# AshHarvey/ssa-gym

Hardware: AMD Instinct MI355X
Metric: env_steps_per_sec_at_20k_objects (higher is better)
Workload: dtype f64

## Files before the change

### include/ssa_hip.h

```cpp
#ifndef SSA_HIP_H
#define SSA_HIP_H

#include <stdint.h>

#ifdef __cplusplus
extern "C" {
#endif

#define SSA_ABI_VERSION 23
#define SSA_INLINE_ENVS 8

#define SSA_OK 0
#define SSA_E_INVALID (-1)
#define SSA_E_LAUNCH (-2)
#define SSA_E_UNSUPPORTED (-3)

#define SSA_ST_OK 0
#define SSA_ST_PREDICT_NAN 1
#define SSA_ST_PREDICT_LINALG 2
#define SSA_ST_UPDATE_NAN 3
#define SSA_ST_UPDATE_LINALG 4

#define SSA_OBS_AER 0
#define SSA_OBS_XYZ 1

#define SSA_PROP_ELEMENTS 0
#define SSA_PROP_FG 1
#define SSA_PROP_J2_RK4 2

#define SSA_PROP_HYBRID 3

#define SSA_FLAG_RESAMPLE 1u

#define SSA_FLAG_REFERENCE_COV 2u

#define SSA_UPD_STRIDE 64
#define SSA_UPD_OBS_TAKEN 0
#define SSA_UPD_Z_TRUE 1
#define SSA_UPD_Y 4
#define SSA_UPD_S 7
#define SSA_UPD_SIGMAS_H 16
#define SSA_UPD_VISIBLE 55
#define SSA_UPD_ACTION 56

#define SSA_STAT_SHARDS 128
#define SSA_STAT_SHARD_WORDS 16
#define SSA_STAT_STRIDE 8
#define SSA_STAT_MAX_DPOS 0
#define SSA_STAT_CNT_LT_1E4 1
#define SSA_STAT_CNT_LT_1E7 2
#define SSA_STAT_ARGMAX_SPOS 3
#define SSA_STAT_N_FAILED 4
#define SSA_STAT_MAX_SPOS 5

typedef struct ssa_consts {
    double Q[36];
    double R[9];
    double Wm0, Wc0, Wi;
    double sum_wm_m1;
    double sum_wc;
    double scale;
    double dt;
    double obs_limit;
    double enu[9];
    double obs_itrs[3];
    int32_t obs_type;
    int32_t propagator;
    uint32_t flags;
    int32_t update_interval;
    double j2, r_eq;
    int32_t rk4_substeps;
    int32_t reserved0;
} ssa_consts;

typedef struct ssa_step_params {
    int64_t n_obj;
    int32_t n_env;
    int32_t time_offset;
    const double *x_true_in; double *x_true_out;
    const double *x_in;      double *x_out;
    const double *P_in;      double *P_out;
    int32_t *status;
    double *obs;
    double *metrics;
    double *upd;
    const double *trans;
    const int32_t *env_time;
    const int32_t *actions;
    const double *z_noise;
    int64_t zn_stride_env, zn_stride_time, zn_stride_obj;
    int32_t n_time;
    uint32_t launch_mask;
    double *stats;
    int32_t *work;
    void *stat_ws;
    uint64_t *stat_shards;
    uint64_t *stat_shards_prev;
    double *stats_prev;
    double *aer_out;
    uint64_t *stat_shards_clear;
    int32_t aer_cols;
    int32_t action0;
    double *obs_mirror;
    int32_t inline_time[SSA_INLINE_ENVS];
    int32_t inline_action[SSA_INLINE_ENVS];
    uint64_t *spos_tiles;
    uint64_t *spos_tiles_prev;
    double *fail_log;
    uint32_t *fail_count;
    int32_t fail_cap;
    int32_t reserved1;
    const int32_t *obj_ids;
    const double *metrics_prev;
} ssa_step_params;
#define SSA_FAIL_STRIDE 8
#define SSA_FAIL_ENV 0
#define SSA_FAIL_OBJ 1
#define SSA_FAIL_STATUS 2
#define SSA_FAIL_TIME 3
#define SSA_FAIL_ERR 4

int ssa_env_step_f64(const ssa_consts *c_host, const ssa_step_params *p_host, void *stream);
#define SSA_PROFILE_SLOTS 1024
#define SSA_LAUNCH_DEFER_FOLD 8u
#define SSA_LAUNCH_INLINE_ACTION 16u
#define SSA_LAUNCH_FOLD_INSIDE 32u
#define SSA_LAUNCH_MIRROR_F32 128u
#define SSA_LAUNCH_INLINE_ENVS 64u
#define SSA_LAUNCH_STATS_FROM_METRICS 256u
int ssa_env_step_profiled_f64(const ssa_consts *c_host, const ssa_step_params *p_host, void *stream, int32_t slot);
int ssa_env_step_profile_ms(int32_t slot, float *kernel_ms);
typedef struct ssa_rollout_params {
    int32_t n_steps;
    int32_t history;
    int32_t slot_out;
    int32_t reserved;
    double *x_true_ring;
    double *x_ring;
    double *P_ring;
    double *obs_ring;
    double *metrics_ring;
    double *upd_ring;
    double *stats_ring;
    const int32_t *actions;
    uint64_t *stat_shards;
    uint64_t *spos_tiles;
} ssa_rollout_params;
int ssa_env_rollout_f64(const ssa_consts *c_host, const ssa_step_params *first, const ssa_rollout_params *r, void *stream);

int ssa_stats_fold_f64(uint64_t *stat_shards, double *stats, int32_t n_env, void *stream);
int ssa_stats_fold_spos_f64(uint64_t *stat_shards, const uint64_t *spos_tiles, double *stats, int64_t n_obj, int32_t n_env, void *stream);
int32_t ssa_stats_from_metrics_waves(int64_t n_obj, int32_t n_env);
int ssa_stats_fold_metrics_f64(const double *metrics, uint64_t *stat_shards, const uint64_t *spos_tiles, double *stats, int64_t n_obj,
                               void *stream);
int64_t ssa_env_step_work_bytes(int64_t n_obj, int32_t n_env);

int ssa_reward_stats_f64(const double *metrics, const int32_t *status, double *stats, void *workspace,
                         int64_t n_obj, int32_t n_env, void *stream);
int64_t ssa_reward_stats_workspace_bytes(int32_t n_env);

int ssa_propagate_f64(const double *x_in, double *x_out, int64_t n, double dt, int32_t propagator, void *stream);
int ssa_propagate_j2_f64(const double *x_in, double *x_out, int64_t n, double dt, double j2, double r_eq,
                         int32_t substeps, void *stream);
int ssa_kepler_elements_f64(const double *x_in, double *coe, int64_t n, double dt, void *stream);
int ssa_robust_cholesky6_f64(const double *A, double *U, int32_t *rung, int64_t n, void *stream);
int ssa_ladder_probe_f64(const double *A, double scale, int32_t *rung, int32_t *mask, double *U, int64_t n, void *stream);
int ssa_sigma_points_f64(const double *x, const double *P, double scale, double *sig, int32_t *fail,
                         int64_t n, void *stream);
int ssa_hx_aer_f64(const double *x, int64_t x_stride, const double *M, const ssa_consts *c_host, double *z,
                   int64_t n, void *stream);
int ssa_mean_z_uvw_f64(const double *sigmas, const ssa_consts *c_host, double *zp, int64_t n, void *stream);
int ssa_residual_z_aer_f64(const double *a, const double *b, double *c, int64_t n, void *stream);
int ssa_visible_mask_f64(const double *x_true, const double *M, const ssa_consts *c_host, uint8_t *mask,
                         double *el, int64_t n, void *stream);
int ssa_observe_f64(const double *x_true, const double *x, const double *P, double *obs, double *metrics,
                    int64_t n, void *stream);
int ssa_aer_obs_f64(const double *x, const double *P, const double *M, const ssa_consts *c_host, double *out,
                    int64_t n, void *stream);

int ssa_agent_scores_f64(const double *x_true, const double *x_cur, const double *P_cur, const double *P_prev,
                         const double *M, const ssa_consts *c_host, double *scores, uint8_t *mask, int64_t n,
                         void *stream);
int ssa_visible_mask_at_f64(const double *x_true, const double *trans, const int32_t *env_time, int32_t time_offset, int32_t n_time,
                            const ssa_consts *c_host, uint8_t *mask, double *el, int64_t n, void *stream);
int ssa_agent_scores_at_f64(const double *x_true, const double *x_cur, const double *P_cur, const double *P_prev, const double *trans,
                            const int32_t *env_time, int32_t time_offset, int32_t n_time, const ssa_consts *c_host, double *scores,
                            uint8_t *mask, int64_t n, void *stream);
int ssa_masked_argmax_f64(const double *score, const uint8_t *mask, int64_t n, int64_t *out, void *stream);
int ssa_masked_argmax_ws_f64(const double *score, const uint8_t *mask, int64_t n, int64_t *out, void *workspace, int64_t workspace_bytes,
                             void *stream);
int64_t ssa_masked_argmax_workspace_bytes(int64_t n);

#define SSA_AGENT_NAIVE_GREEDY 0
#define SSA_AGENT_VISIBLE_GREEDY 1
#define SSA_AGENT_SHANNON 2
#define SSA_AGENT_POS_ERROR 3
#define SSA_AGENT_VEL_ERROR 4
int ssa_agent_select_f64(const ssa_consts *c_host, int32_t kind, const double *x_true, const double *x_cur,
                         const double *P_cur, const double *P_prev, const double *trans, const int32_t *env_time,
                         int32_t time_offset, int32_t n_time, const int32_t *fallback, void *workspace,
                         int32_t *action_out, int64_t *pick_out, int64_t n_obj, int32_t n_env, void *stream);
int ssa_agent_select_ids_f64(const ssa_consts *c_host, int32_t kind, const double *x_true, const double *x_cur,
                             const double *P_cur, const double *P_prev, const double *trans, const int32_t *env_time,
                             int32_t time_offset, int32_t n_time, const int32_t *fallback, void *workspace,
                             int32_t *action_out, int64_t *pick_out, int64_t n_obj, int32_t n_env, const int32_t *obj_ids, void *stream);
int64_t ssa_agent_select_workspace_bytes(int64_t n_obj, int32_t n_env);

int ssa_nees_f64(const double *x_true, const double *x, const double *P, double *nees, int64_t n, void *stream);
int ssa_nis_f64(const double *y, const double *S, double *nis, int64_t n, void *stream);
int ssa_chi2_contained_f64(const double *v, int64_t n, double lo, double hi, int64_t *counts, void *stream);

typedef struct ssa_closed_loop_params {
    int32_t n_steps;
    int32_t history;
    int32_t slot_out;
    int32_t agent;
    double *x_true_ring, *x_ring, *P_ring, *obs_ring, *metrics_ring;
    double *upd_out;
    double *stats_out;
    int32_t *actions;
    const int32_t *fallback;
    int64_t *picks;
    int32_t *error;
    void *workspace;
    int64_t workspace_bytes;
    int64_t wait_ticks;
    uint32_t flags;
    uint32_t reserved;
    const int32_t *slot_of;
} ssa_closed_loop_params;
#define SSA_LOOP_ARGMAX_SPOS 1u
#define SSA_LOOP_DEBUG_WITHHOLD 2u
int ssa_env_closed_loop_f64(const ssa_consts *c_host, const ssa_step_params *first, const ssa_closed_loop_params *r, void *stream);
int64_t ssa_closed_loop_workspace_bytes(int64_t n_obj, int32_t n_env);

#define SSA_LOOK_NSCORE 3
#define SSA_LOOK_TRACE_GAIN 0
#define SSA_LOOK_POS_TRACE_GAIN 1
#define SSA_LOOK_INFO_GAIN 2
typedef struct ssa_lookahead_out {
    double *score;
    int32_t *status;
    uint8_t *visible;
    double *x_prior;
    double *P_prior;
    double *P_post;
} ssa_lookahead_out;
int ssa_lookahead_f64(const ssa_consts *c_host, const ssa_step_params *p_host, const ssa_lookahead_out *out, void *stream);

#define SSA_MAX_SENSORS 8
typedef struct ssa_sensor_params {
    int32_t n_sensor;
    int32_t reserved;
    int32_t action[SSA_MAX_SENSORS];
    double enu[SSA_MAX_SENSORS][9];
    double obs_itrs[SSA_MAX_SENSORS][3];
    double obs_limit[SSA_MAX_SENSORS];
    double R[SSA_MAX_SENSORS][9];
    int64_t zn_stride_sensor;
    double *upd;
} ssa_sensor_params;
int ssa_env_step_sensors_f64(const ssa_consts *c_host, const ssa_step_params *p_host, const ssa_sensor_params *s_host, void *stream);

typedef struct ssa_sensor_envs_params {
    const int32_t *actions;
    double *upd;
    int32_t inline_action[SSA_INLINE_ENVS][SSA_MAX_SENSORS];
} ssa_sensor_envs_params;
int ssa_env_step_sensors_envs_f64(const ssa_consts *c, const ssa_step_params *p, const ssa_sensor_params *sites,
                                  const ssa_sensor_envs_params *envs, void *stream);

int ssa_lookahead_sensors_f64(const ssa_consts *c_host, const ssa_step_params *p_host, const ssa_sensor_params *s_host,
                              const ssa_lookahead_out *out, void *stream);
int ssa_lookahead_sensors_envs_f64(const ssa_consts *c, const ssa_step_params *p, const ssa_sensor_params *sites,
                                   const ssa_lookahead_out *out, void *stream);

typedef struct ssa_rollout_sensors_params {
    const int32_t *actions;
    double *upd_ring;
} ssa_rollout_sensors_params;
int ssa_env_rollout_sensors_f64(const ssa_consts *c_host, const ssa_step_params *first, const ssa_rollout_params *r,
                                const ssa_sensor_params *sites, const ssa_rollout_sensors_params *rs, void *stream);
// ... 63 lines not shown
```

### profiles/pmc_counters_reduce.py

```python
import csv, glob, json, os, sys
ROOT = os.path.dirname(os.path.dirname(os.path.abspath(__file__)))
out = {"kernel": None, "workload": "20 000 objects = 5000 wavefronts, profiles/pmc_workload.py", "counters": {}}
for d in sys.argv[1:]:
    fs = glob.glob(os.path.join(ROOT, d, '*', '*counter_collection.csv'))
    if not fs:
        out["counters"][os.path.basename(d)] = "pass produced no counter file (counter not available on this build?)"
        continue
    acc = {}
    for r in csv.DictReader(open(fs[0])):
        if 'step_fast_kernel' not in r['Kernel_Name']:
            continue
        if out["kernel"] is None:
            out["kernel"] = r['Kernel_Name'].split('(')[0]
        acc.setdefault(r['Counter_Name'], []).append(float(r['Counter_Value']))
    for k, v in acc.items():
        v = v[20:] if len(v) > 40 else v
        out["counters"][k] = {"mean_per_launch": sum(v) / len(v), "per_wavefront": sum(v) / len(v) / 5000.0, "launches": len(v)}
print(json.dumps(out, indent=1))
```

### profiles/pmc_reduce.py

```python
import csv, glob, json, os, sys
ROOT = os.path.dirname(os.path.dirname(os.path.abspath(__file__)))
def per_kernel(d, counter):
    f = glob.glob(os.path.join(ROOT, d, '*', '*counter_collection.csv'))[0]
    acc = {}
    for r in csv.DictReader(open(f)):
        if r['Counter_Name'] != counter: continue
        k = r['Kernel_Name']
        key = 'step' if 'step_fast_kernel' in k else 'propagate' if 'propagate_kernel' in k else 'observe' if 'observe_kernel' in k else None
        if key: acc.setdefault(key, []).append(float(r['Counter_Value']))
    return acc
fe, wr = per_kernel(sys.argv[1], 'FETCH_SIZE'), per_kernel(sys.argv[2], 'WRITE_SIZE')
n = 1 << 20
known = {'propagate': (48 * n, 48 * n), 'observe': (384 * n, 128 * n)}
out = {}
for k in ('propagate', 'observe'):
    f = sum(fe[k][-3:]) / 3 * 1024; w = sum(wr[k][-3:]) / 3 * 1024
    out['calib_' + k] = {'fetch_counter_bytes': f, 'fetch_known_bytes': known[k][0], 'fetch_ratio': f / known[k][0],
                         'write_counter_bytes': w, 'write_known_bytes': known[k][1], 'write_ratio': w / known[k][1]}
fs = fe['step'][20:]; ws = wr['step'][20:]
f = sum(fs) / len(fs) * 1024; w = sum(ws) / len(ws) * 1024
cf = out['calib_observe']['fetch_ratio']; cw = out['calib_observe']['write_ratio']
out['step_raw'] = {'fetch_counter_bytes': f, 'write_counter_bytes': w, 'launches': len(fs)}
key = '%s_%s' % (os.environ.get('PROP', 'hybrid'), os.environ.get('M', '20000'))
out[key] = round(f / cf + w / cw)
out['algorithmic_bytes'] = 896 * int(os.environ.get('M', '20000'))
print(json.dumps(out, indent=1))
dst = os.path.join(ROOT, 'profiles', 'traffic.json')
old = json.load(open(dst)) if os.path.exists(dst) else {}
old[key] = out[key]
old.setdefault('other_configurations', {})[key] = {'step_raw': out['step_raw'], 'calib_observe': out['calib_observe'], 'calib_propagate': out['calib_propagate']}
if not isinstance(old.get('collected'), dict):
    old['collected'] = {}
old['collected'][key] = os.environ.get('TAG', 'unlabelled')
old['algorithmic_bytes_20000'] = 896 * 20000
json.dump(old, open(dst, 'w'), indent=1)
```

### ssa-gym_amd/_lib.py

```python
import ctypes as C
import os

from . import _build

c_dp = C.c_void_p


class ssa_consts(C.Structure):
    _fields_ = [
        ("Q", C.c_double * 36), ("R", C.c_double * 9),
        ("Wm0", C.c_double), ("Wc0", C.c_double), ("Wi", C.c_double),
        ("sum_wm_m1", C.c_double), ("sum_wc", C.c_double), ("scale", C.c_double),
        ("dt", C.c_double), ("obs_limit", C.c_double),
        ("enu", C.c_double * 9), ("obs_itrs", C.c_double * 3),
        ("obs_type", C.c_int32), ("propagator", C.c_int32), ("flags", C.c_uint32),
        ("update_interval", C.c_int32),
        ("j2", C.c_double), ("r_eq", C.c_double), ("rk4_substeps", C.c_int32), ("reserved0", C.c_int32),
    ]


class ssa_step_params(C.Structure):
    _fields_ = [
        ("n_obj", C.c_int64), ("n_env", C.c_int32), ("time_offset", C.c_int32),
        ("x_true_in", c_dp), ("x_true_out", c_dp), ("x_in", c_dp), ("x_out", c_dp),
        ("P_in", c_dp), ("P_out", c_dp), ("status", c_dp), ("obs", c_dp), ("metrics", c_dp),
        ("upd", c_dp), ("trans", c_dp), ("env_time", c_dp), ("actions", c_dp), ("z_noise", c_dp),
        ("zn_stride_env", C.c_int64), ("zn_stride_time", C.c_int64), ("zn_stride_obj", C.c_int64),
        ("n_time", C.c_int32), ("launch_mask", C.c_uint32), ("stats", c_dp), ("work", c_dp), ("stat_ws", c_dp),
        ("stat_shards", c_dp), ("stat_shards_prev", c_dp), ("stats_prev", c_dp), ("aer_out", c_dp),
        ("stat_shards_clear", c_dp), ("aer_cols", C.c_int32), ("action0", C.c_int32), ("obs_mirror", c_dp),
        ("inline_time", C.c_int32 * 8), ("inline_action", C.c_int32 * 8),
        ("spos_tiles", c_dp), ("spos_tiles_prev", c_dp),
        ("fail_log", c_dp), ("fail_count", c_dp), ("fail_cap", C.c_int32), ("reserved1", C.c_int32),
        ("obj_ids", c_dp), ("metrics_prev", c_dp),
    ]


class ssa_rollout_params(C.Structure):
    _fields_ = [
        ("n_steps", C.c_int32), ("history", C.c_int32), ("slot_out", C.c_int32), ("reserved", C.c_int32),
        ("x_true_ring", c_dp), ("x_ring", c_dp), ("P_ring", c_dp), ("obs_ring", c_dp), ("metrics_ring", c_dp),
        ("upd_ring", c_dp), ("stats_ring", c_dp), ("actions", c_dp), ("stat_shards", c_dp), ("spos_tiles", c_dp),
    ]


class ssa_closed_loop_params(C.Structure):
    _fields_ = [
        ("n_steps", C.c_int32), ("history", C.c_int32), ("slot_out", C.c_int32), ("agent", C.c_int32),
        ("x_true_ring", c_dp), ("x_ring", c_dp), ("P_ring", c_dp), ("obs_ring", c_dp), ("metrics_ring", c_dp),
        ("upd_out", c_dp), ("stats_out", c_dp), ("actions", c_dp), ("fallback", c_dp), ("picks", c_dp), ("error", c_dp),
        ("workspace", c_dp), ("workspace_bytes", C.c_int64),
        ("wait_ticks", C.c_int64), ("flags", C.c_uint32), ("reserved", C.c_uint32), ("slot_of", c_dp),
    ]


class ssa_lookahead_out(C.Structure):
    _fields_ = [
        ("score", c_dp), ("status", c_dp), ("visible", c_dp), ("x_prior", c_dp), ("P_prior", c_dp), ("P_post", c_dp),
    ]


class ssa_sensor_params(C.Structure):
    _fields_ = [
        ("n_sensor", C.c_int32), ("reserved", C.c_int32), ("action", C.c_int32 * 8),
        ("enu", (C.c_double * 9) * 8), ("obs_itrs", (C.c_double * 3) * 8), ("obs_limit", C.c_double * 8), ("R", (C.c_double * 9) * 8),
        ("zn_stride_sensor", C.c_int64), ("upd", c_dp),
    ]


class ssa_rollout_sensors_params(C.Structure):
    _fields_ = [("actions", c_dp), ("upd_ring", c_dp)]


class ssa_rollout_sensors_envs_params(C.Structure):
    _fields_ = [("actions", c_dp), ("stats_out", c_dp), ("upd_out", c_dp)]


class ssa_sensor_envs_params(C.Structure):
    _fields_ = [("actions", c_dp), ("upd", c_dp), ("inline_action", (C.c_int32 * 8) * 8)]


class ssa_forecast_params(C.Structure):
    _fields_ = [("n_steps", C.c_int32), ("reserved", C.c_int32), ("out", ssa_lookahead_out)]


class ssa_screen_params(C.Structure):
    _fields_ = [
        ("n", C.c_int64), ("n_time", C.c_int32), ("n_site", C.c_int32), ("step", C.c_double), ("min_alt", C.c_double),
        ("first", C.c_int32), ("max_gap", C.c_int32), ("elements", c_dp), ("trans", c_dp), ("sites", c_dp),
        ("accept", c_dp), ("worst_gap", c_dp), ("flags", c_dp),
    ]


E_INVALID, E_LAUNCH, E_UNSUPPORTED = -1, -2, -3
ABI_VERSION = 23
ST_OK, ST_PREDICT_NAN, ST_PREDICT_LINALG, ST_UPDATE_NAN, ST_UPDATE_LINALG = range(5)
OBS_AER, OBS_XYZ = 0, 1
PROP_ELEMENTS, PROP_FG, PROP_J2_RK4, PROP_HYBRID = 0, 1, 2, 3
FLAG_RESAMPLE = 1
FLAG_REFERENCE_COV = 2
UPD_STRIDE, UPD_OBS_TAKEN, UPD_Z_TRUE, UPD_Y, UPD_S, UPD_SIGMAS_H, UPD_VISIBLE, UPD_ACTION = 64, 0, 1, 4, 7, 16, 55, 56
STAT_SHARDS = 128
STAT_SHARD_WORDS = 16
PROFILE_SLOTS = 1024
LAUNCH_DEFER_FOLD = 8
LAUNCH_INLINE_ACTION = 16
LAUNCH_FOLD_INSIDE = 32
LAUNCH_INLINE_ENVS = 64
LAUNCH_MIRROR_F32 = 128
LAUNCH_STATS_FROM_METRICS = 256
INLINE_ENVS = 8
LOOP_ARGMAX_SPOS, LOOP_DEBUG_WITHHOLD = 1, 2
FAIL_STRIDE, FAIL_ENV, FAIL_OBJ, FAIL_STATUS, FAIL_TIME, FAIL_ERR = 8, 0, 1, 2, 3, 4
AGENT_NAIVE_GREEDY, AGENT_VISIBLE_GREEDY, AGENT_SHANNON, AGENT_POS_ERROR, AGENT_VEL_ERROR = range(5)
MAX_SENSORS = 8
LOOK_NSCORE, LOOK_TRACE_GAIN, LOOK_POS_TRACE_GAIN, LOOK_INFO_GAIN = 3, 0, 1, 2
STAT_STRIDE, STAT_MAX_DPOS, STAT_CNT_LT_1E4, STAT_CNT_LT_1E7, STAT_ARGMAX_SPOS, STAT_N_FAILED, STAT_MAX_SPOS = 8, 0, 1, 2, 3, 4, 5

SIGNATURES = {
    "ssa_abi_version": (C.c_int, []),
    "ssa_build_info": (C.c_char_p, []),
    "ssa_env_step_f64": (C.c_int, [C.POINTER(ssa_consts), C.POINTER(ssa_step_params), c_dp]),
    "ssa_env_step_profiled_f64": (C.c_int, [C.POINTER(ssa_consts), C.POINTER(ssa_step_params), c_dp, C.c_int32]),
    "ssa_env_step_profile_ms": (C.c_int, [C.c_int32, C.POINTER(C.c_float)]),
    "ssa_stats_fold_f64": (C.c_int, [c_dp, c_dp, C.c_int32, c_dp]),
    "ssa_stats_fold_spos_f64": (C.c_int, [c_dp, c_dp, c_dp, C.c_int64, C.c_int32, c_dp]),
    "ssa_stats_from_metrics_waves": (C.c_int32, [C.c_int64, C.c_int32]),
    "ssa_stats_fold_metrics_f64": (C.c_int, [c_dp, c_dp, c_dp, c_dp, C.c_int64, c_dp]),
    "ssa_ladder_probe_f64": (C.c_int, [c_dp, C.c_double, c_dp, c_dp, c_dp, C.c_int64, c_dp]),
    "ssa_env_rollout_f64": (C.c_int, [C.POINTER(ssa_consts), C.POINTER(ssa_step_params), C.POINTER(ssa_rollout_params), c_dp]),
    "ssa_env_closed_loop_f64": (C.c_int, [C.POINTER(ssa_consts), C.POINTER(ssa_step_params), C.POINTER(ssa_closed_loop_params), c_dp]),
    "ssa_lookahead_f64": (C.c_int, [C.POINTER(ssa_consts), C.POINTER(ssa_step_params), C.POINTER(ssa_lookahead_out), c_dp]),
    "ssa_env_step_sensors_f64": (C.c_int, [C.POINTER(ssa_consts), C.POINTER(ssa_step_params), C.POINTER(ssa_sensor_params), c_dp]),
    "ssa_env_step_sensors_envs_f64": (C.c_int, [C.POINTER(ssa_consts), C.POINTER(ssa_step_params), C.POINTER(ssa_sensor_params),
                                                C.POINTER(ssa_sensor_envs_params), c_dp]),
    "ssa_lookahead_sensors_f64": (C.c_int, [C.POINTER(ssa_consts), C.POINTER(ssa_step_params), C.POINTER(ssa_sensor_params),
                                            C.POINTER(ssa_lookahead_out), c_dp]),
    "ssa_lookahead_sensors_envs_f64": (C.c_int, [C.POINTER(ssa_consts), C.POINTER(ssa_step_params), C.POINTER(ssa_sensor_params),
                                                 C.POINTER(ssa_lookahead_out), c_dp]),
    "ssa_forecast_sensors_f64": (C.c_int, [C.POINTER(ssa_consts), C.POINTER(ssa_step_params), C.POINTER(ssa_sensor_params),
                                           C.POINTER(ssa_forecast_params), c_dp]),
    "ssa_forecast_sensors_envs_f64": (C.c_int, [C.POINTER(ssa_consts), C.POINTER(ssa_step_params), C.POINTER(ssa_sensor_params),
                                                C.POINTER(ssa_forecast_params), c_dp]),
    "ssa_env_rollout_sensors_f64": (C.c_int, [C.POINTER(ssa_consts), C.POINTER(ssa_step_params), C.POINTER(ssa_rollout_params),
                                              C.POINTER(ssa_sensor_params), C.POINTER(ssa_rollout_sensors_params), c_dp]),
    "ssa_env_rollout_sensors_envs_f64": (C.c_int, [C.POINTER(ssa_consts), C.POINTER(ssa_step_params), C.POINTER(ssa_rollout_params),
                                                   C.POINTER(ssa_sensor_params), C.POINTER(ssa_rollout_sensors_envs_params), c_dp]),
    "ssa_closed_loop_workspace_bytes": (C.c_int64, [C.c_int64, C.c_int32]),
    "ssa_env_step_work_bytes": (C.c_int64, [C.c_int64, C.c_int32]),
    "ssa_reward_stats_f64": (C.c_int, [c_dp, c_dp, c_dp, c_dp, C.c_int64, C.c_int32, c_dp]),
    "ssa_reward_stats_workspace_bytes": (C.c_int64, [C.c_int32]),
    "ssa_propagate_f64": (C.c_int, [c_dp, c_dp, C.c_int64, C.c_double, C.c_int32, c_dp]),
    "ssa_propagate_j2_f64": (C.c_int, [c_dp, c_dp, C.c_int64, C.c_double, C.c_double, C.c_double, C.c_int32, c_dp]),
    "ssa_kepler_elements_f64": (C.c_int, [c_dp, c_dp, C.c_int64, C.c_double, c_dp]),
    "ssa_robust_cholesky6_f64": (C.c_int, [c_dp, c_dp, c_dp, C.c_int64, c_dp]),
    "ssa_sigma_points_f64": (C.c_int, [c_dp, c_dp, C.c_double, c_dp, c_dp, C.c_int64, c_dp]),
    "ssa_hx_aer_f64": (C.c_int, [c_dp, C.c_int64, c_dp, C.POINTER(ssa_consts), c_dp, C.c_int64, c_dp]),
    "ssa_mean_z_uvw_f64": (C.c_int, [c_dp, C.POINTER(ssa_consts), c_dp, C.c_int64, c_dp]),
    "ssa_residual_z_aer_f64": (C.c_int, [c_dp, c_dp, c_dp, C.c_int64, c_dp]),
    "ssa_visible_mask_f64": (C.c_int, [c_dp, c_dp, C.POINTER(ssa_consts), c_dp, c_dp, C.c_int64, c_dp]),
    "ssa_observe_f64": (C.c_int, [c_dp, c_dp, c_dp, c_dp, c_dp, C.c_int64, c_dp]),
    "ssa_agent_scores_f64": (C.c_int, [c_dp, c_dp, c_dp, c_dp, c_dp, C.POINTER(ssa_consts), c_dp, c_dp, C.c_int64, c_dp]),
    "ssa_visible_mask_at_f64": (C.c_int, [c_dp, c_dp, c_dp, C.c_int32, C.c_int32, C.POINTER(ssa_consts), c_dp, c_dp, C.c_int64, c_dp]),
    "ssa_agent_scores_at_f64": (C.c_int, [c_dp, c_dp, c_dp, c_dp, c_dp, c_dp, C.c_int32, C.c_int32, C.POINTER(ssa_consts), c_dp, c_dp, C.c_int64, c_dp]),
    "ssa_masked_argmax_f64": (C.c_int, [c_dp, c_dp, C.c_int64, c_dp, c_dp]),
    "ssa_masked_argmax_ws_f64": (C.c_int, [c_dp, c_dp, C.c_int64, c_dp, c_dp, C.c_int64, c_dp]),
    "ssa_masked_argmax_workspace_bytes": (C.c_int64, [C.c_int64]),
    "ssa_assign_sensors_f64": (C.c_int, [c_dp, C.c_int64, C.c_int32, C.c_int32, c_dp, c_dp, c_dp, c_dp, C.c_int64, c_dp]),
    "ssa_assign_sensors_workspace_bytes": (C.c_int64, [C.c_int64, C.c_int32]),
    "ssa_assign_sensors_envs_f64": (C.c_int, [c_dp, C.c_int64, C.c_int32, C.c_int32, C.c_int32, c_dp, c_dp, c_dp, c_dp, C.c_int64, c_dp]),
    "ssa_assign_sensors_envs_workspace_bytes": (C.c_int64, [C.c_int64, C.c_int32, C.c_int32]),
    "ssa_match_sensors_f64": (C.c_int, [c_dp, C.c_int64, C.c_int32, C.c_int32, c_dp, c_dp, c_dp, c_dp, C.c_int64, c_dp]),
    "ssa_match_sensors_envs_f64": (C.c_int, [c_dp, C.c_int64, C.c_int32, C.c_int32, C.c_int32, c_dp, c_dp, c_dp, c_dp, C.c_int64, c_dp]),
    "ssa_peer_push_f64": (C.c_int, [c_dp, C.c_int64, c_dp, c_dp, C.c_int32, c_dp, C.c_uint64, c_dp, C.c_int64, c_dp, c_dp, c_dp]),
    "ssa_peer_wait": (C.c_int, [c_dp, C.c_int32, c_dp, C.c_uint64, C.c_int64, c_dp, c_dp]),
    "ssa_aer_obs_f64": (C.c_int, [c_dp, c_dp, c_dp, C.POINTER(ssa_consts), c_dp, C.c_int64, c_dp]),
    "ssa_agent_select_f64": (C.c_int, [C.POINTER(ssa_consts), C.c_int32, c_dp, c_dp, c_dp, c_dp, c_dp, c_dp, C.c_int32, C.c_int32,
                                       c_dp, c_dp, c_dp, c_dp, C.c_int64, C.c_int32, c_dp]),
    "ssa_agent_select_ids_f64": (C.c_int, [C.POINTER(ssa_consts), C.c_int32, c_dp, c_dp, c_dp, c_dp, c_dp, c_dp, C.c_int32, C.c_int32,
                                           c_dp, c_dp, c_dp, c_dp, C.c_int64, C.c_int32, c_dp, c_dp]),
    "ssa_agent_select_workspace_bytes": (C.c_int64, [C.c_int64, C.c_int32]),
    "ssa_nees_f64": (C.c_int, [c_dp, c_dp, c_dp, c_dp, C.c_int64, c_dp]),
    "ssa_nis_f64": (C.c_int, [c_dp, c_dp, c_dp, C.c_int64, c_dp]),
    "ssa_chi2_contained_f64": (C.c_int, [c_dp, C.c_int64, C.c_double, C.c_double, c_dp, c_dp]),
    "ssa_catalogue_screen_f64": (C.c_int, [C.POINTER(ssa_screen_params), c_dp]),
}

_lib = None


class SsaHipError(RuntimeError):
    pass


def library_path():
    return _build.LIB


def load():
    global _lib
    if _lib is not None:
        return _lib
    path = library_path()
    if not os.path.exists(path):
        raise SsaHipError(
            "libssa_hip.so is not built (%s). The ssa-gym hot path has no CPU fallback: run "
            "`python -c 'import __graft_entry__ as g; g.build()'` (needs hipcc)." % path)
    import torch
    lib = C.CDLL(path)
    for name, (res, args) in SIGNATURES.items():
        fn = getattr(lib, name)
        fn.restype = res
        fn.argtypes = args
    if lib.ssa_abi_version() != ABI_VERSION:
        raise SsaHipError("libssa_hip.so ABI %d != binding %d: rebuild" % (lib.ssa_abi_version(), ABI_VERSION))
    _lib = lib
    return lib


def check(rc, what):
    if rc != 0:
        raise SsaHipError("%s failed with code %d" % (what, rc))
```

### ssa-gym_amd/csrc/ssa_kernels.hip

```cpp
#include <hip/hip_runtime.h>
#include <cstdio>
#include <cstddef>
#include <cstdlib>
#include <hip/hip_ext.h>
#include <stdint.h>
#include <type_traits>

#include "../../include/ssa_hip.h"
#include "ssa_math.hpp"
#include "ssa_conics.hpp"
#include "ssa_screen.hpp"

namespace ssa {

__device__ __noinline__ Vec6 kepler_general_v(Vec6 x, double tof)
{
    Vec6 o;
    kepler_general_impl(x.v, tof, o.v, nullptr);
    return o;
}
template <int TAG>
__device__ __noinline__ Vec6 kepler_general_tagged(Vec6 x, double tof)
{
    Vec6 o;
    kepler_general_impl(x.v, tof, o.v, nullptr);
    return o;
}
template <int TAG>
__device__ __noinline__ Vec6 kepler_general_fast_tagged(Vec6 x, double tof) { return kepler_general_fast_impl<TAG>(x, tof); }
template <int TAG>
__device__ __noinline__ Vec6 kepler_beyond_series_tagged(Vec6 x, double tof)
{
    Vec6 o;
    const bool ok = kepler_conic_lean<TAG, false>(x.v, tof, o.v);
    if (__any(!ok)) {
        if (!ok) o = kepler_general_fast_tagged<TAG>(x, tof);
    }
    return o;
}
SSA_DEV bool kepler_hybrid_fast(const double* s, double tof, double* o)
{
    const double rr = dot3(s, s), vv = dot3(s + 3, s + 3), rv = dot3(s, s + 3);
    const double c1 = vv - MU * rsqrt_nr(rr);
    const double ex = c1 * s[0] - rv * s[3], ey = c1 * s[1] - rv * s[4], ez = c1 * s[2] - rv * s[5];
    const double e2 = (ex * ex + ey * ey + ez * ez) * (1.0 / (MU * MU));
    bool handled;
    const bool ok = kepler_uv_fast(s, tof, o, handled);
    return ok && (e2 < (1.0 - 1e-2) * (1.0 - 1e-2));
}

__device__ __noinline__ Vec8 kepler_general_diag_v(Vec6 x, double tof, Vec6* out)
{
    Vec8 d;
    Vec6 o;
    kepler_general_impl(x.v, tof, o.v, d.v);
    *out = o;
    return d;
}

struct StepK {
    ssa_consts c;
    ssa_step_params p;
};

constexpr int OBJ_PER_WAVE = 4;
constexpr double X_FAILED_POS = 1e20, X_FAILED_VEL = 1e12;

struct alignas(16) Tiles {
    double P[OBJ_PER_WAVE * 36];
    double Q[36];
    double Z[8];
    int St[OBJ_PER_WAVE];
    int Oid[OBJ_PER_WAVE];
    double X[OBJ_PER_WAVE * 6];
    double pad1[8];
    double T[OBJ_PER_WAVE * 6];
    double UA[OBJ_PER_WAVE * 36];
    double D[408];
    double M[OBJ_PER_WAVE * 12];
    double Obs[OBJ_PER_WAVE * 12];
    double Met[OBJ_PER_WAVE * 4];
};
static_assert(offsetof(Tiles, P) == 0 && offsetof(Tiles, X) == 1536 && offsetof(Tiles, T) == 1792, "LDS-DMA image of the tile (tile_dma_issue)");
SSA_DEV int dbase(int g) { return g * 96 + (g & 1) * 4 + (g >> 1) * 16; }
static_assert(sizeof(Tiles) <= 7680, "Tiles must fit 20 wavefronts per CU (see above)");

struct TileRegs { double2 main, aux; int st; bool dma; };
SSA_DEV double2 load16(const double* src) { return *reinterpret_cast<const double2*>(src); }
SSA_DEV void tile_issue_from(TileRegs& r, const double* P_in, const double* x_in, const double* x_true_in, const int32_t* status,
                            int lane, int64_t base, int cnt)
{
    const double2 zero = make_double2(0.0, 0.0);
    r.main = zero;
    r.aux = zero;
    r.st = SSA_ST_PREDICT_NAN;
    r.dma = false;
    if (cnt <= 0) return;
    const double* Pin = P_in + base * 36;
    if (lane < cnt * 18) r.main = load16(Pin + 2 * lane);
    const bool sX = lane >= 32, sT = lane >= 48;
    const int i = lane - (sT ? 48 : sX ? 32 : 0);
    const int lim = sX ? cnt * 3 : cnt * 18 - 64;
    const double* src = sT ? x_true_in + base * 6 : sX ? x_in + base * 6 : Pin + 128;
    if (i < lim) r.aux = load16(src + 2 * i);
    if (lane >= 60 && lane - 60 < cnt) r.st = status[base + (lane - 60)];
}
SSA_DEV void tile_issue(TileRegs& r, const ssa_step_params& p, int lane, int64_t base, int cnt)
{
    tile_issue_from(r, p.P_in, p.x_in, p.x_true_in, p.status, lane, base, cnt);
}
SSA_DEV void tile_commit(Tiles& t, const TileRegs& r, int lane)
{
    reinterpret_cast<double2*>(t.P)[lane] = r.main;
    const bool sX = lane >= 32, sT = lane >= 48;
    const int i = lane - (sT ? 48 : sX ? 32 : 0);
    double* dst = sT ? t.T : sX ? t.X : t.P + 128;
    if (i < (sX ? 12 : 8)) reinterpret_cast<double2*>(dst)[i] = r.aux;
    if (lane >= 60) t.St[lane - 60] = r.st;
}
SSA_DEV int64_t tile_total(const ssa_step_params& p, bool one_env) { return one_env ? p.n_obj : (int64_t)p.n_env * p.n_obj; }
typedef const __attribute__((address_space(1))) void* GlobalVoidPtr;
typedef __attribute__((address_space(3))) void* LdsVoidPtr;
SSA_DEV void glds16(const double* src, double* lds_base)
{
    __builtin_amdgcn_global_load_lds((GlobalVoidPtr)src, (LdsVoidPtr)lds_base, 16, 0, 0);
}
SSA_DEV void tile_dma_issue(Tiles& t, TileRegs& r, const double* P_in, const double* x_in, const double* x_true_in, const int32_t* status,
                            int lane, int64_t base, bool whole, const ssa_step_params& p, bool one_env)
{
    r.dma = whole;
    if (!whole) {
        tile_issue_from(r, P_in, x_in, x_true_in, status, lane, base, (int)(tile_total(p, one_env) - base));
        return;
    }
    r.st = SSA_ST_PREDICT_NAN;
    const double* Pin = P_in + base * 36;
    glds16(Pin + 2 * lane, t.P);
    if (lane < 8) glds16(Pin + 128 + 2 * lane, t.P + 128);
    if (lane >= 32 && lane < 44) glds16(x_in + base * 6 - 64 + 2 * lane, t.P + 128);
    if (lane >= 48 && lane < 60) glds16(x_true_in + base * 6 - 96 + 2 * lane, t.P + 128);
    if (lane >= 60) r.st = status[base + (lane - 60)];
}
SSA_DEV void tile_dma_wait(Tiles& t, const TileRegs& r, int lane)
{
    asm volatile("s_waitcnt vmcnt(0)" ::: "memory");
    if (lane >= 60) t.St[lane - 60] = r.st;
}
typedef double v2d __attribute__((ext_vector_type(2)));
template <bool NT>
SSA_DEV void store16(double* dst, const double* src)
{
    if (NT) __builtin_nontemporal_store(*reinterpret_cast<const v2d*>(src), reinterpret_cast<v2d*>(dst));
    else *reinterpret_cast<v2d*>(dst) = *reinterpret_cast<const v2d*>(src);
}
SSA_DEV int64_t env_row0(const ssa_step_params& p, int64_t base)
{
    return p.n_env > 1 ? (int64_t)((uint32_t)base / (uint32_t)p.n_obj) * p.n_obj : 0;
}
template <bool NT>
SSA_DEV void store_tile(const Tiles& t, const ssa_step_params& p, int lane, int64_t base, int cnt)
{
#define SSA_SKIP(b) 0
    if (cnt == OBJ_PER_WAVE) {
        if (!SSA_SKIP(1)) {
            store16<NT>(p.P_out + base * 36 + 2 * lane, t.P + 2 * lane);
            if (lane < 8) store16<NT>(p.P_out + base * 36 + 128 + 2 * lane, t.P + 128 + 2 * lane);
        }
        if (!SSA_SKIP(4)) {
            if ((unsigned)(lane - 8) < 12u) store16<NT>(p.x_out + base * 6 - 16 + 2 * lane, t.X - 16 + 2 * lane);
            if ((unsigned)(lane - 20) < 12u) store16<NT>(p.x_true_out + base * 6 - 40 + 2 * lane, t.T - 40 + 2 * lane);
        }
        if (!SSA_SKIP(2) && lane >= 32 && lane < 56) {
            const int i = lane - 32;
            const int jj = (i * 43) >> 8;
            const int r = 2 * i - 12 * jj;
            double* dst = p.obs + base * 12 - 64 + 2 * lane;
            v2d pair;
            if (r < 6) pair = *reinterpret_cast<const v2d*>(t.X + jj * 6 + r);
            else {
                const double* d = t.P + jj * 36 + 7 * (r - 6);
                pair = v2d{d[0], d[7]};
            }
            if (NT) __builtin_nontemporal_store(pair, reinterpret_cast<v2d*>(dst));
            else *reinterpret_cast<v2d*>(dst) = pair;
            if (p.obs_mirror) {
                const int64_t at = p.obj_ids ? (env_row0(p, base) + t.Oid[jj]) * 12 + r : base * 12 - 64 + 2 * lane;
                if (p.launch_mask & SSA_LAUNCH_MIRROR_F32)
                    *reinterpret_cast<float2*>(reinterpret_cast<float*>(p.obs_mirror) + at) = make_float2((float)pair.x, (float)pair.y);
                else *reinterpret_cast<v2d*>(p.obs_mirror + at) = pair;
            }
        }
        if (!SSA_SKIP(16) && lane >= 56 && lane < 60) p.status[base - 56 + lane] = t.St[lane - 56];
        if (!SSA_SKIP(8) && lane < 16) {
            const int kk = lane >> 2, jj = lane & 3;
            const int64_t obj = base + jj;
            if (p.n_env == 1) {
                p.metrics[(int64_t)kk * p.n_obj + obj] = t.Met[jj * 4 + kk];
            } else {
                const int64_t e = (int64_t)((uint32_t)obj / (uint32_t)p.n_obj), j = obj - e * p.n_obj;
                p.metrics[(e * 4 + kk) * p.n_obj + j] = t.Met[jj * 4 + kk];
            }
        }
        return;
    }
    if (!SSA_SKIP(1) && lane < cnt * 18) store16<NT>(p.P_out + base * 36 + 2 * lane, t.P + 2 * lane);
    {
        const bool sT = lane >= 16, sP = lane >= 32, sO = lane >= 40;
        const int i = lane - (sO ? 40 : sP ? 32 : sT ? 16 : 0);
        const int lim = sO ? cnt * 6 : sP ? cnt * 18 - 64 : cnt * 3;
        double* dst = sO ? p.obs + base * 12 : sP ? p.P_out + base * 36 + 128 : sT ? p.x_true_out + base * 6 : p.x_out + base * 6;
        const double* src = sO ? t.Obs : sP ? t.P + 128 : sT ? t.T : t.X;
        const bool skip = sO ? SSA_SKIP(2) : sP ? SSA_SKIP(1) : SSA_SKIP(4);
        if (!skip && i < lim) store16<NT>(dst + 2 * i, src + 2 * i);
        if (sO && p.obs_mirror && i < lim) {
            const int jj = (i * 43) >> 8;
            const int64_t at = p.obj_ids ? (env_row0(p, base) + t.Oid[jj]) * 12 + (2 * i - 12 * jj) : base * 12 + 2 * i;
            if (p.launch_mask & SSA_LAUNCH_MIRROR_F32)
                *reinterpret_cast<float2*>(reinterpret_cast<float*>(p.obs_mirror) + at) = make_float2((float)src[2 * i], (float)src[2 * i + 1]);
            else store16<false>(p.obs_mirror + at, src + 2 * i);
        }
    }
    if (!SSA_SKIP(16) && lane >= 12 && lane < 16) {
        const int i = lane - 12;
        if (i < cnt) p.status[base + i] = t.St[i];
    }
    if (!SSA_SKIP(8) && lane < 16) {
        const int kk = lane >> 2, jj = lane & 3;
        if (jj < cnt) {
            const int64_t obj = base + jj;
            if (p.n_env == 1) {
                p.metrics[(int64_t)kk * p.n_obj + obj] = t.Met[jj * 4 + kk];
            } else {
                const int64_t e = (int64_t)((uint32_t)obj / (uint32_t)p.n_obj), j = obj - e * p.n_obj;
                p.metrics[(e * 4 + kk) * p.n_obj + j] = t.Met[jj * 4 + kk];
            }
        }
    }
}

SSA_DEV void observe_rows(Tiles& t, int g, int l, bool stage_obs)
{
    if (stage_obs && l < 12) t.Obs[g * 12 + l] = (l < 6) ? t.X[g * 6 + l] : t.P[g * 36 + 7 * (l - 6)];
    if (l < 4) {
        const int off = (l & 1) * 3;
        double v;
        if (l < 2) {
            double a0 = t.X[g * 6 + off] - t.T[g * 6 + off];
            double a1 = t.X[g * 6 + off + 1] - t.T[g * 6 + off + 1];
            double a2 = t.X[g * 6 + off + 2] - t.T[g * 6 + off + 2];
            v = sqrt_fast(a0 * a0 + a1 * a1 + a2 * a2);
        } else {
            v = sqrt_fast(t.P[g * 36 + 7 * off] + t.P[g * 36 + 7 * (off + 1)] + t.P[g * 36 + 7 * (off + 2)]);
        }
        t.Met[g * 4 + l] = v;
    }
}

struct Moments { double c00, c01, c11; };
template <bool SUMS_ONLY = false>
SSA_DEV Moments moment_sums_mfma(Tiles& t, int lane)
{
    const int hi = lane >> 4, mid = (lane >> 2) & 3, lo = lane & 3;
    const double* src = &t.D[dbase(mid) + hi * 8 + lo];
    double a0[3], a1[3];
#pragma unroll
    for (int kc = 0; kc < 3; ++kc) {
        a0[kc] = src[kc * 32];
        a1[kc] = src[kc * 32 + 4];
    }
    Moments mo = {0.0, 0.0, 0.0};
#pragma unroll
    for (int kc = 0; kc < 3; ++kc) {
        if (!SUMS_ONLY) mo.c00 = __builtin_amdgcn_mfma_f64_4x4x4f64(a0[kc], a0[kc], mo.c00, 0, 0, 0);
        mo.c01 = __builtin_amdgcn_mfma_f64_4x4x4f64(a0[kc], a1[kc], mo.c01, 0, 0, 0);
        mo.c11 = __builtin_amdgcn_mfma_f64_4x4x4f64(a1[kc], a1[kc], mo.c11, 0, 0, 0);
    }
    if (lo == 2) {
        t.M[mid * 12 + hi] = mo.c01;
        if (hi < 2) t.M[mid * 12 + 4 + hi] = mo.c11;
    }
    return mo;
}

SSA_DEV double covariance_entry(const ssa_consts& C, double acc, double sa_, double ma, double sb_, double mb, double q)
{
    return C.Wi * acc - ma * sb_ - sa_ * mb + C.sum_wc * ma * mb + q;
}
SSA_DEV void covariance_finish(Tiles& t, const ssa_consts& C, int lane, const Moments& mo)
{
    const int hi = lane >> 4, mid = (lane >> 2) & 3, lo = lane & 3;
    const int hi1 = hi & 1, lo1 = lo & 1;
    const double* M = &t.M[mid * 12];
    double* P = &t.P[mid * 36];
    const double s_a = M[hi], m_a = M[6 + hi], s_b = M[lo], m_b = M[6 + lo];
    const double s_a4 = M[4 + hi1], m_a4 = M[10 + hi1], s_b4 = M[4 + lo1], m_b4 = M[10 + lo1];
    const double p00 = covariance_entry(C, mo.c00, s_a, m_a, s_b, m_b, t.Q[hi * 6 + lo]);
    const double p01 = covariance_entry(C, mo.c01, s_a, m_a, s_b4, m_b4, t.Q[hi * 6 + 4 + lo1]);
    const double p11 = covariance_entry(C, mo.c11, s_a4, m_a4, s_b4, m_b4, t.Q[(4 + hi1) * 6 + 4 + lo1]);
    if (hi <= lo) {
        P[hi * 6 + lo] = p00;
        P[lo * 6 + hi] = p00;
    }
    if (lo < 2) {
        P[hi * 6 + 4 + lo] = p01;
        P[(4 + lo) * 6 + hi] = p01;
        if (hi <= lo) {
            P[(4 + hi) * 6 + 4 + lo] = p11;
            P[(4 + lo) * 6 + 4 + hi] = p11;
        }
    }
}

struct StatAcc {
    double mx, sm;
    long long arg;
    unsigned c4, c7, nf;
    int mx_nan, sm_nan;
};
SSA_DEV void stat_merge(StatAcc& a, const StatAcc& b)
{
    a.mx = fmax(a.mx, b.mx);
    a.mx_nan |= b.mx_nan;
    a.c4 += b.c4; a.c7 += b.c7; a.nf += b.nf;
    bool take_b;
    if (a.sm_nan || b.sm_nan) take_b = b.sm_nan && (!a.sm_nan || b.arg < a.arg);
    else take_b = (b.sm > a.sm) || (b.sm == a.sm && b.arg < a.arg);
    if (take_b) { a.sm = b.sm; a.arg = b.arg; a.sm_nan = b.sm_nan; }
}
SSA_DEV StatAcc stat_shfl_down(const StatAcc& a, int off)
{
    StatAcc b;
    b.mx = __shfl_down(a.mx, off, 64);
    b.sm = __shfl_down(a.sm, off, 64);
    b.arg = __shfl_down(a.arg, off, 64);
    b.c4 = __shfl_down(a.c4, off, 64);
    b.c7 = __shfl_down(a.c7, off, 64);
    b.nf = __shfl_down(a.nf, off, 64);
    b.mx_nan = __shfl_down(a.mx_nan, off, 64);
    b.sm_nan = __shfl_down(a.sm_nan, off, 64);
    return b;
}
SSA_DEV StatAcc stat_identity()
{
    StatAcc a;
    a.mx = -1.0; a.sm = -1.0; a.arg = 0x7fffffffffffffffLL; a.c4 = a.c7 = a.nf = 0; a.mx_nan = a.sm_nan = 0;
    return a;
}
SSA_DEV StatAcc stat_wave_reduce(StatAcc a)
{
#pragma unroll
    for (int off = 32; off > 0; off >>= 1) {
        StatAcc b = stat_shfl_down(a, off);
        stat_merge(a, b);
    }
    return a;
}

SSA_DEV void wave_lds_sync()
{
    __builtin_amdgcn_fence(__ATOMIC_ACQ_REL, "wavefront");
    __builtin_amdgcn_wave_barrier();
    asm volatile("" ::: "memory");
}

SSA_DEV int ybase(int g) { return g * 104 + (g & 1) * 28 + (g >> 1) * 32; }
SSA_DEV void covariance_reference(Tiles& t, const ssa_consts& C, int lane, const double (&o)[6], double xb_l)
{
    static_assert(372 + 16 * 8 <= OBJ_PER_WAVE * 36 + 408, "y rows fit the factor tile + D");
    typedef double v2d_t __attribute__((ext_vector_type(2)));
    double* const Y = t.UA;
    {
        const int g = lane >> 4, l = lane & 15;
        const double x0 = row_bcast<0>(xb_l), x1 = row_bcast<1>(xb_l), x2 = row_bcast<2>(xb_l), x3 = row_bcast<3>(xb_l),
                     x4 = row_bcast<4>(xb_l), x5 = row_bcast<5>(xb_l);
        if (l <= 12) {
            v2d_t* dst = reinterpret_cast<v2d_t*>(&Y[ybase(g) + l * 8]);
            dst[0] = v2d_t{o[0] - x0, o[1] - x1};
            dst[1] = v2d_t{o[2] - x2, o[3] - x3};
            dst[2] = v2d_t{o[4] - x4, o[5] - x5};
            dst[3] = v2d_t{0.0, 0.0};
        }
    }
    wave_lds_sync();
// ... 281 lines not shown
    idx = ids ? (unsigned long long)t.Oid[0] : (unsigned long long)j0;
#pragma unroll
    for (int g = 1; g < OBJ_PER_WAVE; ++g) {
        const unsigned long long k = spos_key(t.Met[g * 4 + 2]);
        const unsigned long long ig = ids ? (unsigned long long)t.Oid[g] : (unsigned long long)(j0 + g);
        if (g < cnt && (k > key || (ids && k == key && ig < idx))) { key = k; idx = ig; }
    }
}
template <int CTRL>
SSA_DEV unsigned long long dpp_u64(unsigned long long v)
{
    return (unsigned long long)__builtin_amdgcn_update_dpp((long long)v, (long long)v, CTRL, 0xF, 0xF, true);
}
SSA_DEV unsigned long long lane_u64(unsigned long long v, int l)
{
    return ((unsigned long long)(unsigned)__builtin_amdgcn_readlane((int)(v >> 32), l) << 32) | (unsigned)__builtin_amdgcn_readlane((int)v, l);
}
struct OpMax { SSA_DEV unsigned long long operator()(unsigned long long a, unsigned long long b) const { return a > b ? a : b; } };
struct OpMin { SSA_DEV unsigned long long operator()(unsigned long long a, unsigned long long b) const { return a < b ? a : b; } };
struct OpAdd { SSA_DEV unsigned long long operator()(unsigned long long a, unsigned long long b) const { return a + b; } };
template <class OP>
SSA_DEV unsigned long long wave_fold_u64(unsigned long long v, OP op)
{
    v = op(v, dpp_u64<0x128>(v));
    v = op(v, dpp_u64<0x124>(v));
    v = op(v, dpp_u64<0x122>(v));
    v = op(v, dpp_u64<0x121>(v));
    return op(op(lane_u64(v, 0), lane_u64(v, 16)), op(lane_u64(v, 32), lane_u64(v, 48)));
}
template <bool COHERENT>
SSA_DEV void fold_spos_tiles(const unsigned long long* __restrict__ slots, int t_lo, int t_hi, double* __restrict__ stats, int lane)
{
    unsigned long long key = 0ull, idx = ~0ull;
    bool any = false;
    for (int tb = t_lo + lane; tb <= t_hi; tb += 64) {
        unsigned long long k, i;
        if (COHERENT) {
            k = __hip_atomic_load(slots + 2 * (int64_t)tb, __ATOMIC_RELAXED, __HIP_MEMORY_SCOPE_AGENT);
            i = __hip_atomic_load(slots + 2 * (int64_t)tb + 1, __ATOMIC_RELAXED, __HIP_MEMORY_SCOPE_AGENT);
        } else {
            const ulonglong2 v = *reinterpret_cast<const ulonglong2*>(slots + 2 * (int64_t)tb);
            k = v.x; i = v.y;
        }
        if (!any || k > key || (k == key && i < idx)) { key = k; idx = i; any = true; }
    }
    const unsigned long long top = wave_fold_u64(any ? key : 0ull, OpMax());
    const unsigned long long who = wave_fold_u64((any && key == top) ? idx : ~0ull, OpMin());
    if (lane == 0) {
        stats[SSA_STAT_ARGMAX_SPOS] = (double)(long long)who;
        stats[SSA_STAT_MAX_SPOS] = spos_of_key(top);
    }
}
SSA_DEV void env_tile_range(int64_t n_obj, int e, int& t_lo, int& t_hi)
{
    const int64_t first = (int64_t)e * n_obj;
    t_lo = (int)(first / OBJ_PER_WAVE);
    t_hi = (int)((first + n_obj - 1) / OBJ_PER_WAVE);
}
SSA_DEV void fold_stat_shards_inside(unsigned long long* __restrict__ shards, double* __restrict__ stats, int lane)
{
    unsigned long long* sh = shards + (int64_t)lane * SSA_STAT_SHARD_WORDS;
    unsigned long long* sh2 = sh + 64 * SSA_STAT_SHARD_WORDS;
    unsigned long long mx = __hip_atomic_load(sh, __ATOMIC_RELAXED, __HIP_MEMORY_SCOPE_AGENT);
    unsigned long long cn = __hip_atomic_load(sh + 1, __ATOMIC_RELAXED, __HIP_MEMORY_SCOPE_AGENT);
    unsigned long long nf = __hip_atomic_load(sh + 2, __ATOMIC_RELAXED, __HIP_MEMORY_SCOPE_AGENT);
    const unsigned long long mb = __hip_atomic_load(sh2, __ATOMIC_RELAXED, __HIP_MEMORY_SCOPE_AGENT);
    const unsigned long long cb = __hip_atomic_load(sh2 + 1, __ATOMIC_RELAXED, __HIP_MEMORY_SCOPE_AGENT);
    const unsigned long long nb = __hip_atomic_load(sh2 + 2, __ATOMIC_RELAXED, __HIP_MEMORY_SCOPE_AGENT);
#pragma unroll
    for (int q = 0; q < 3; ++q) {
        __hip_atomic_store(sh + q, 0ull, __ATOMIC_RELAXED, __HIP_MEMORY_SCOPE_AGENT);
        __hip_atomic_store(sh2 + q, 0ull, __ATOMIC_RELAXED, __HIP_MEMORY_SCOPE_AGENT);
    }
    mx = mb > mx ? mb : mx;
    cn += cb;
    nf += nb;
#pragma unroll
    for (int off = 32; off > 0; off >>= 1) {
        unsigned long long m2 = __shfl_down(mx, off, 64), c2 = __shfl_down(cn, off, 64), n2 = __shfl_down(nf, off, 64);
        mx = m2 > mx ? m2 : mx;
        cn += c2;
        nf += n2;
    }
    if (lane == 0) {
        stats[SSA_STAT_MAX_DPOS] = __longlong_as_double((long long)mx);
        stats[SSA_STAT_CNT_LT_1E4] = (double)(cn & 0xffffffffull);
        stats[SSA_STAT_CNT_LT_1E7] = (double)(cn >> 32);
        stats[SSA_STAT_ARGMAX_SPOS] = -1.0;
        stats[SSA_STAT_N_FAILED] = (double)nf;
        stats[SSA_STAT_MAX_SPOS] = __builtin_nan("");
        stats[6] = 0.0; stats[7] = 0.0;
    }
}

constexpr int STAT_SERVICE_WAVES = 32, STAT_SERVICE_ILP = 10;
static_assert(STAT_SERVICE_WAVES <= SSA_STAT_SHARDS, "one shard line per service wavefront");
SSA_DEV void stats_service_wave(const double* __restrict__ dpos, unsigned long long* __restrict__ shards, double* __restrict__ stats,
                                const unsigned long long* __restrict__ spos, int64_t n_obj, int w, int nserv, int lane)
{
    const uint32_t n = (uint32_t)n_obj;
    const uint32_t per = (n + (uint32_t)nserv - 1u) / (uint32_t)nserv;
    const uint32_t lo = (uint32_t)w * per < n ? (uint32_t)w * per : n;
    const uint32_t hi = n - lo < per ? n : lo + per;
    unsigned long long mx = 0ull, cn = 0ull;
    for (uint32_t b = lo; b < hi; b += 64u * STAT_SERVICE_ILP) {
        double v[STAT_SERVICE_ILP];
#pragma unroll
        for (int q = 0; q < STAT_SERVICE_ILP; ++q) {
            const uint32_t i = b + (uint32_t)(q * 64 + lane);
            v[q] = i < hi ? dpos[i] : 0.0;
        }
#pragma unroll
        for (int q = 0; q < STAT_SERVICE_ILP; ++q) {
            const uint32_t i = b + (uint32_t)(q * 64 + lane);
            if (i < hi) {
                const unsigned long long bits = (unsigned long long)__double_as_longlong(v[q]) & 0x7fffffffffffffffull;
                mx = bits > mx ? bits : mx;
                cn += (unsigned long long)(v[q] < 1e4) + ((unsigned long long)(v[q] < 1e7) << 32);
            }
        }
    }
    mx = wave_fold_u64(mx, OpMax());
    cn = wave_fold_u64(cn, OpAdd());
    bool last = false;
    if (lane == 0) {
        unsigned long long* sh = shards + (int64_t)w * SSA_STAT_SHARD_WORDS;
        __hip_atomic_store(sh, mx, __ATOMIC_RELAXED, __HIP_MEMORY_SCOPE_AGENT);
        __hip_atomic_store(sh + 1, cn, __ATOMIC_RELAXED, __HIP_MEMORY_SCOPE_AGENT);
        asm volatile("s_waitcnt vmcnt(0)" ::: "memory");
        const unsigned old = (unsigned)__hip_atomic_fetch_add(shards + 4, 1ull, __ATOMIC_RELAXED, __HIP_MEMORY_SCOPE_AGENT);
        if (old == (unsigned)nserv - 1u) {
            __hip_atomic_store(shards + 4, 0ull, __ATOMIC_RELAXED, __HIP_MEMORY_SCOPE_AGENT);
            last = true;
        }
    }
    if (__any(last)) {
        fold_stat_shards_inside(shards, stats, lane);
        if (spos) {
            int t_lo, t_hi;
            env_tile_range(n_obj, 0, t_lo, t_hi);
            fold_spos_tiles<false>(spos, t_lo, t_hi, stats, lane);
        }
    }
}

struct ActBase {
    static constexpr bool late = false;
    static constexpr bool all = false;
    static constexpr bool sensors = false;
    static constexpr bool look_sensors = false;
    static constexpr bool forecast = false;
    static constexpr bool envs = false;
    static constexpr bool look_envs = false;
    SSA_DEV int get() { return -1; }
    SSA_DEV void before_wait(Tiles&, int, int) {}
    SSA_DEV void mid_step(Tiles&, int) {}
    SSA_DEV const ssa_sensor_params* sites() const { return nullptr; }
};
struct ActEarly : ActBase {};
struct ActLate;
struct LoopK;
SSA_DEV void closed_loop_prescore(ActLate& a, Tiles& t, int lane, int cnt);
SSA_DEV void closed_loop_store(const LoopK* lk, Tiles& t, int lane, int kk, int64_t base, int cnt);
constexpr unsigned CL_ABORT_GEN = 0xFFFFFFFFu;
constexpr unsigned long long CL_TIMEOUT_TICKS = 200000000ull;
struct ActLate : ActBase {
    static constexpr bool late = true;
    unsigned long long* flag;
    unsigned long long* all_flags;
    int* err;
    int nflags;
    unsigned long long timeout;
    unsigned want;
    int first;
    int last;
    bool aborted;
    int agent;
    const ssa_consts* C;
    const double* M;
    int* vis;
    SSA_DEV void before_wait(Tiles& t, int lane, int cnt) { closed_loop_prescore(*this, t, lane, cnt); }
    const LoopK* lk;
    int pend;
    int64_t base;
    int cnt;
    SSA_DEV void mid_step(Tiles& t, int lane)
    {
        if (pend < 0) return;
        closed_loop_store(lk, t, lane, pend, base, cnt);
        pend = -1;
    }
    SSA_DEV void abort_all()
    {
        const int lane = threadIdx.x;
        for (int i = lane; i < nflags; i += 64)
            __hip_atomic_store(all_flags + (int64_t)i * 16, (unsigned long long)CL_ABORT_GEN << 32, __ATOMIC_RELAXED, __HIP_MEMORY_SCOPE_AGENT);
        if (lane == 0 && err) __hip_atomic_store(err, 1, __ATOMIC_RELAXED, __HIP_MEMORY_SCOPE_SYSTEM);
    }
    SSA_DEV int get()
    {
        if (want == 0u) { last = first; return first; }
        const unsigned long long t0 = wall_clock64();
        unsigned lo, hi;
        for (;;) {
            const unsigned long long v = __hip_atomic_load(flag, __ATOMIC_RELAXED, __HIP_MEMORY_SCOPE_AGENT);
            lo = __builtin_amdgcn_readfirstlane((unsigned)v);
            hi = __builtin_amdgcn_readfirstlane((unsigned)(v >> 32));
            if (hi >= want) break;
            if (wall_clock64() - t0 > timeout) {
                abort_all();
                hi = CL_ABORT_GEN;
                break;
            }
            __builtin_amdgcn_s_sleep(2);
        }
        if (hi == CL_ABORT_GEN) {
            aborted = true;
            return -2;
        }
        last = (int)lo;
        return (int)lo;
    }
};
struct ActAll : ActBase {
    static constexpr bool all = true;
    const ssa_lookahead_out* o;
};
struct ActSensors : ActBase {
    static constexpr bool sensors = true;
    const ssa_sensor_params* s;
    SSA_DEV const ssa_sensor_params* sites() const { return s; }
    SSA_DEV const int32_t* actions(const ssa_sensor_params* sp) const { return sp->action; }
    SSA_DEV int action(const ssa_sensor_params* sp, int k) const { return sp->action[k]; }
    SSA_DEV double* records(const ssa_sensor_params* sp) const { return sp->upd; }
};
struct ActSchedule : ActBase {
    static constexpr bool sensors = true;
    const ssa_sensor_params* s;
    const int32_t* row;
    double* upd;
    SSA_DEV const ssa_sensor_params* sites() const { return s; }
    typedef int row_t __attribute__((ext_vector_type(SSA_MAX_SENSORS)));
    typedef const __attribute__((address_space(4))) int32_t* WordPtr;
    SSA_DEV row_t actions(const ssa_sensor_params*) const
    {
        typedef const __attribute__((address_space(4))) row_t* RowPtr;
        return *(RowPtr)__builtin_assume_aligned(row, sizeof(row_t));
    }
    SSA_DEV int action(const ssa_sensor_params*, int k) const { return ((WordPtr)row)[k]; }
    SSA_DEV double* records(const ssa_sensor_params*) const { return upd; }
};
SSA_DEV ConstPtr<int32_t> vector_sensors_inline_rows();
struct ActSensorEnvs : ActBase {
    static constexpr bool sensors = true, envs = true;
    const ssa_sensor_params* s;
    const ssa_sensor_envs_params* v;
    int env;
    ConstPtr<int32_t> row;
    double* upd;
    SSA_DEV const ssa_sensor_params* sites() const { return s; }
    SSA_DEV void enter(uint32_t mask, int n_env, int64_t n_obj, int64_t base)
    {
        env = (n_env > 1) ? __builtin_amdgcn_readfirstlane((int)((uint32_t)base / (uint32_t)n_obj)) : 0;
        const ConstPtr<int32_t> rows = (mask & SSA_LAUNCH_INLINE_ENVS) ? vector_sensors_inline_rows() : (ConstPtr<int32_t>)v->actions;
        row = rows + (int64_t)env * SSA_MAX_SENSORS;
        upd = v->upd ? v->upd + (int64_t)env * s->n_sensor * SSA_UPD_STRIDE : nullptr;
    }
    typedef int row_t __attribute__((ext_vector_type(SSA_MAX_SENSORS)));
    SSA_DEV row_t actions(const ssa_sensor_params*) const { return *(ConstPtr<row_t>)__builtin_assume_aligned(row, sizeof(row_t)); }
    SSA_DEV int action(const ssa_sensor_params*, int k) const { return row[k]; }
    SSA_DEV double* records(const ssa_sensor_params*) const { return upd; }
};
struct ActScheduleEnvs : ActBase {
    static constexpr bool sensors = true, envs = true;
    const ssa_sensor_params* s;
    const ssa_rollout_sensors_envs_params* v;
    int kk;
    int env;
    ConstPtr<int32_t> row;
    double* upd;
    SSA_DEV const ssa_sensor_params* sites() const { return s; }
    SSA_DEV void enter(uint32_t, int n_env, int64_t n_obj, int64_t base)
    {
        env = (n_env > 1) ? __builtin_amdgcn_readfirstlane((int)((uint32_t)base / (uint32_t)n_obj)) : 0;
        const int64_t ke = (int64_t)kk * n_env + env;
        row = (ConstPtr<int32_t>)v->actions + ke * SSA_MAX_SENSORS;
        upd = v->upd_out ? v->upd_out + ke * s->n_sensor * SSA_UPD_STRIDE : nullptr;
    }
    typedef int row_t __attribute__((ext_vector_type(SSA_MAX_SENSORS)));
    SSA_DEV row_t actions(const ssa_sensor_params*) const { return *(ConstPtr<row_t>)__builtin_assume_aligned(row, sizeof(row_t)); }
    SSA_DEV int action(const ssa_sensor_params*, int k) const { return row[k]; }
    SSA_DEV double* records(const ssa_sensor_params*) const { return upd; }
};
template <class ACT>
SSA_DEV int sensor_index(const ACT& a, const ssa_sensor_params* s, int64_t jid)
{
    int sid = -1;
    const auto act = a.actions(s);
#pragma unroll
    for (int k = SSA_MAX_SENSORS - 1; k >= 0; --k)
        if (k < s->n_sensor && act[k] >= 0 && (int64_t)act[k] == jid) sid = k;
    return sid;
}
struct ActLookSensors : ActBase {
    static constexpr bool all = true, look_sensors = true;
    const ssa_lookahead_out* o;
    const ssa_sensor_params* s;
    SSA_DEV const ssa_sensor_params* sites() const { return s; }
};
struct ActForecastSensors : ActBase {
    static constexpr bool all = true, look_sensors = true, forecast = true;
    const ssa_lookahead_out* o;
    const ssa_sensor_params* s;
    int h;
    SSA_DEV const ssa_sensor_params* sites() const { return s; }
    SSA_DEV void slab(ssa_lookahead_out& os, int64_t m, int S) const
    {
        const int64_t rs = (int64_t)h * S * m, rp = (int64_t)h * m;
        os.score += rs * SSA_LOOK_NSCORE;
        os.status += rs;
        os.visible += rs;
        if (os.P_post) os.P_post += rs * 36;
        if (os.x_prior) os.x_prior += rp * 6;
        if (os.P_prior) os.P_prior += rp * 36;
    }
};
struct ActLookSensorEnvs : ActBase {
    static constexpr bool all = true, look_sensors = true, look_envs = true;
    const ssa_lookahead_out* o;
    const ssa_sensor_params* s;
    int env;
    SSA_DEV const ssa_sensor_params* sites() const { return s; }
    SSA_DEV void enter(int n_env, int64_t n_obj, int64_t base)
    {
        env = (n_env > 1) ? __builtin_amdgcn_readfirstlane((int)((uint32_t)base / (uint32_t)n_obj)) : 0;
    }
    SSA_DEV void slab(ssa_lookahead_out& os, int64_t m, int S) const
    {
        const int64_t rs = (int64_t)env * S * m, rp = (int64_t)env * m;
        os.score += rs * SSA_LOOK_NSCORE;
        os.status += rs;
        os.visible += rs;
        if (os.P_post) os.P_post += rs * 36;
        if (os.x_prior) os.x_prior += rp * 6;
        if (os.P_prior) os.P_prior += rp * 36;
    }
};
SSA_DEV ConstPtr<int32_t> forecast_envs_inline_time();
struct ActForecastSensorEnvs : ActBase {
    static constexpr bool all = true, look_sensors = true, forecast = true, look_envs = true;
    const ssa_lookahead_out* o;
    const ssa_sensor_params* s;
    int h;
    int n_env;
    int env;
    SSA_DEV const ssa_sensor_params* sites() const { return s; }
    SSA_DEV void enter(int n_env_, int64_t n_obj, int64_t base)
    {
        env = (n_env_ > 1) ? __builtin_amdgcn_readfirstlane((int)((uint32_t)base / (uint32_t)n_obj)) : 0;
    }
    SSA_DEV int time_word(uint32_t mask, const int32_t* mem) const
    {
        const ConstPtr<int32_t> src = (mask & SSA_LAUNCH_INLINE_ENVS) ? forecast_envs_inline_time() : (ConstPtr<int32_t>)mem;
        return src[env];
    }
    SSA_DEV void slab(ssa_lookahead_out& os, int64_t m, int S) const
    {
        const int64_t he = (int64_t)h * n_env + env;
        const int64_t rs = he * S * m, rp = he * m;
        os.score += rs * SSA_LOOK_NSCORE;
        os.status += rs;
        os.visible += rs;
        if (os.P_post) os.P_post += rs * 36;
        if (os.x_prior) os.x_prior += rp * 6;
        if (os.P_prior) os.P_prior += rp * 36;
    }
};
template <class T> SSA_DEV const T* kernarg_opaque(const T* q)
{
    typedef const __attribute__((address_space(4))) T* KP;
    KP k = (KP)q;
    asm volatile("" : "+s"(k));
    return (const T*)k;
}
SSA_DEV double logdet_chol(const double (&A)[21]);
template <int PPL> SSA_DEV int pp_at(int idx) { return PPL == 0 ? idx : (idx / 3) * 9 + 6 + idx % 3; }
template <int PPL = 0>
SSA_DEV void lookahead_store(const Tiles& t, const ssa_lookahead_out& o, int g, int l, int64_t orow, int st, bool vis, bool taken)
{
    const double* Pm = &t.P[g * 36];
    const double* Pp = &t.UA[g * 117];
    const bool lin = st == SSA_ST_UPDATE_LINALG;
    for (int idx = l; idx < 36; idx += 16) {
        const int a = idx / 6, b = idx - 6 * a;
        const double pm = Pm[idx];
        const double pp = taken ? Pp[pp_at<PPL>(idx)] : (lin ? ((a == b) ? (a < 3 ? X_FAILED_POS : X_FAILED_VEL) : 0.0) : pm);
        if (o.P_prior) o.P_prior[orow * 36 + idx] = pm;
        if (o.P_post) o.P_post[orow * 36 + idx] = pp;
    }
    if (o.x_prior && l < 6) o.x_prior[orow * 6 + l] = t.X[g * 6 + l];
    double ld = 0.0;
    if (taken && l < 2) {
        const double* src = (l == 0) ? Pm : Pp;
        double A[21];
#pragma unroll
        for (int r = 0; r < 6; ++r)
#pragma unroll
            for (int c = r; c < 6; ++c) A[tri(r, c)] = (PPL == 0 || l == 0) ? src[r * 6 + c] : src[pp_at<PPL>(r * 6 + c)];
        ld = logdet_chol(A);
    }
    const double ld_post = __shfl_down(ld, 1, 64);
    if (l == 0) {
        const double nan = __builtin_nan("");
        double sc[SSA_LOOK_NSCORE] = {nan, nan, nan};
        if (taken) {
            double trm = 0.0, trp = 0.0, pos_m = 0.0, pos_p = 0.0;
#pragma unroll
            for (int r = 0; r < 6; ++r) {
                trm += Pm[7 * r];
                trp += Pp[pp_at<PPL>(7 * r)];
                if (r == 2) { pos_m = trm; pos_p = trp; }
            }
            sc[SSA_LOOK_TRACE_GAIN] = trm - trp;
            sc[SSA_LOOK_POS_TRACE_GAIN] = pos_m - pos_p;
            sc[SSA_LOOK_INFO_GAIN] = 0.5 * (ld - ld_post);
        }
#pragma unroll
        for (int k = 0; k < SSA_LOOK_NSCORE; ++k) o.score[orow * SSA_LOOK_NSCORE + k] = sc[k];
        o.status[orow] = st;
        o.visible[orow] = vis ? 1 : 0;
    }
}

template <int PROP, int TILE, class ACT>
SSA_DEV void process_wave(Tiles& t, const ssa_consts& C, const ssa_step_params& p, int lane, int64_t obj_in, bool valid,
                          int64_t base, int cnt, TileRegs& pf, int64_t next_base, int next_cnt, int tile, ACT& asrc)
{
    constexpr bool INL = (TILE != 2) && !ACT::late;
    constexpr bool SEG = (TILE == 0);
    constexpr bool FOLD_OK = (TILE == 0);
    constexpr bool FROM_METRICS = (TILE == 0) && !ACT::late && !ACT::all && !ACT::sensors && !ACT::look_sensors;
    constexpr bool ALL = ACT::all;
    constexpr bool SENS = ACT::sensors;
    constexpr bool LSENS = ACT::look_sensors;
    constexpr bool FCAST = ACT::forecast;
    constexpr bool ENVS = ACT::envs;
    constexpr bool LENVS = ACT::look_envs;
    constexpr bool ISSUE_LAST = LSENS && PROP != 0;
    constexpr bool PASS_ARGS = LSENS && !(TILE == 1 && PROP == 0);
    int g = lane >> 4, l = lane & 15;
    int64_t obj = obj_in;
    double q_in = 0.0;
    if (TILE == 0 && lane < 36) q_in = C.Q[lane];
    struct { uint32_t mask; const int32_t *actions, *env_time, *obj_ids; int n_env, time_offset, update_interval; } hw =
        {p.launch_mask, p.actions, p.env_time, p.obj_ids, p.n_env, p.time_offset, C.update_interval};
    if (TILE == 0 && !ALL) {
        asm volatile("" : "+s"(hw.mask), "+s"(hw.actions), "+s"(hw.env_time), "+s"(hw.obj_ids), "+s"(hw.n_env), "+s"(hw.time_offset),
                          "+s"(hw.update_interval)
                     : "s"(p.P_out), "s"(p.x_out), "s"(p.x_true_out), "s"(p.obs), "s"(p.metrics), "s"(p.stat_shards), "s"(p.upd), "s"(p.aer_out),
                       "s"(p.n_obj));
    } else if (TILE == 0) {
        asm volatile("" : "+s"(hw.mask), "+s"(hw.env_time), "+s"(hw.obj_ids), "+s"(hw.n_env), "+s"(hw.time_offset), "+s"(hw.update_interval));
    }

    if constexpr (ENVS) asrc.enter(hw.mask, hw.n_env, p.n_obj, base);
    int e = (valid && hw.n_env > 1) ? (int)((uint32_t)obj / (uint32_t)p.n_obj) : 0;
    if constexpr (ENVS) e = asrc.env;
    if constexpr (LENVS) {
        asrc.enter(hw.n_env, p.n_obj, base);
        e = asrc.env;
    }
    const int64_t j = valid ? obj - (int64_t)e * p.n_obj : 0;
    int act, tix;
    int id0 = 0, id1 = 0, id2 = 0, id3 = 0;
    if (ACT::late) {
        act = -1;
        tix = valid ? p.env_time[0] + p.time_offset : 0;
    } else if (SEG) {
        const ConstPtr<int32_t> t_src = segment_word_src<true>(hw.mask, hw.env_time), a_src = segment_word_src<false>(hw.mask, hw.actions);
        int t0 = *t_src, a0 = -1;
        if constexpr (ENVS) t0 = t_src[asrc.env];
        if constexpr (LENVS) t0 = t_src[asrc.env];
        if (!ALL && !SENS) a0 = *a_src;
        if (hw.obj_ids) {
            const v4i w = *(ConstPtr<v4i>)(hw.obj_ids + base);
            id0 = w.x; id1 = w.y; id2 = w.z; id3 = w.w;
        }
        asm volatile("" : "+s"(t0), "+s"(a0), "+s"(id0), "+s"(id1), "+s"(id2), "+s"(id3));
        if (!ENVS && !LENVS && hw.n_env > 1) {
            t0 = segment_lane_word(t_src, e);
            if (!ALL && !SENS) a0 = segment_lane_word(a_src, e);
        }
        act = valid ? a0 : -1;
        tix = valid ? t0 + hw.time_offset : 0;
    } else if (ALL) {
        act = -1;
        if constexpr (FCAST && LENVS) tix = valid ? asrc.time_word(hw.mask, hw.env_time) + p.time_offset : 0;
        else tix = valid ? env_time_of<INL>(p, e) + p.time_offset : 0;
    } else if (SENS) {
        act = -1;
        if constexpr (ENVS) tix = valid ? env_time_of<INL>(p, asrc.env) + p.time_offset : 0;
        else tix = valid ? env_time_of<INL>(p, 0) + p.time_offset : 0;
    } else if (p.n_env > 1) {
        act = valid ? env_action<INL>(p, e) : -1;
        tix = valid ? env_time_of<INL>(p, e) + p.time_offset : 0;
    } else {
        const int a0 = env_action<INL>(p, 0), t0 = env_time_of<INL>(p, 0);
        act = valid ? a0 : -1;
        tix = valid ? t0 + p.time_offset : 0;
    }
    const bool interval_ok = (hw.update_interval <= 1) || (tix % hw.update_interval == 0);
    int64_t jid = j;
    if (hw.obj_ids) {
        int4 ids;
        if (TILE == 0) ids = make_int4(id0, id1, id2, id3);
        else ids = *reinterpret_cast<const int4*>(hw.obj_ids + base);
        const int mine = (g == 0) ? ids.x : (g == 1) ? ids.y : (g == 2) ? ids.z : ids.w;
        jid = valid ? (int64_t)mine : 0;
        if (l == 0) t.Oid[g] = mine;
    }
    int sid = -1;
    if constexpr (SENS) {
        sid = valid ? sensor_index(asrc, asrc.sites(), jid) : -1;
        act = (sid >= 0) ? (int)jid : -1;
    }
    bool my_update = ALL ? (valid && interval_ok) : SENS ? (sid >= 0 && interval_ok)
                                                         : (!ACT::late && valid && act >= 0 && (int64_t)act == jid && interval_ok);
    const bool may_update = ACT::late ? (valid && interval_ok) : my_update;
    if (!ACT::late && !ALL && __any(my_update)) __builtin_amdgcn_s_setprio(3);
    int tmod = 0;
    double upd_in = 0.0;
    if (may_update && l < (ALL ? 9 : 12)) {
        tmod = time_row(tix, p.n_time);
        const int64_t aobj = ACT::late ? jid : (int64_t)act;
        const double* src = (l < 9) ? p.trans + (int64_t)tmod * 9 + l
                                    : p.z_noise + (int64_t)e * p.zn_stride_env + (int64_t)tmod * p.zn_stride_time + aobj * p.zn_stride_obj + (l - 9);
        if constexpr (SENS) {
            if (l >= 9) src += (int64_t)sid * asrc.sites()->zn_stride_sensor;
        }
        upd_in = *src;
    }

    if (TILE == 0 && pf.dma) tile_dma_wait(t, pf, lane);
    else if (TILE != 2) tile_commit(t, pf, lane);
    if (lane < 8) t.Z[lane] = 0.0;
    if (TILE == 0) {
        if (lane < 36) t.Q[lane] = q_in;
    } else if (TILE != 2 && lane < 36) t.Q[lane] = C.Q[lane];
    wave_lds_sync();

    const int st_in = t.St[g];
    const bool active = valid && st_in == SSA_ST_OK;

    const int rung = robust_chol_row_lds(t, C.scale, g, l);
    asrc.mid_step(t, lane);
    if (may_update && l < 12) t.Obs[g * 12 + l] = upd_in;
    wave_lds_sync();
    const bool chol_fail = (rung == 16);
    const bool is_sigma = (l <= 12);
    const bool is_pm = (l >= 1 && l <= 12);
    double s[6];
    {
        const int krow = (l >= 7) ? l - 7 : l - 1;
        const double sgn = (l >= 7) ? -1.0 : 1.0;
        const bool use_filter = active && !chol_fail && l != 13;
        const double* base = use_filter ? &t.X[g * 6] : &t.T[g * 6];
        const double* urow = (use_filter && is_pm) ? &t.UA[g * 36 + krow * 6] : &t.Z[0];
#pragma unroll
        for (int c = 0; c < 6; ++c) s[c] = fma(sgn, urow[c], base[c]);
    }
    double o[6];
    {
        bool kep_ok;
        if (PROP == 2) {
            const J2Params jq = {C.j2, C.r_eq, C.rk4_substeps};
            kep_ok = propagate_j2_rk4(s, C.dt, jq, o);
        } else {
            if (PROP == 3) kep_ok = kepler_hybrid_fast(s, C.dt, o);
            else kep_ok = kepler_step_fast<PROP == 2 ? 1 : PROP, 1>(s, C.dt, o);
        }
        if (PROP == 3) {
            if (__any(!kep_ok)) {
                bool served = kep_ok;
                if (!ACT::late) {
                    if (!kep_ok) served = kepler_conic_lean<1, true>(s, C.dt, o);
                }
                if (__any(!served)) {
                    __builtin_amdgcn_s_setprio(3);
                    if (!served) {
                        Vec6 si;
#pragma unroll
                        for (int c = 0; c < 6; ++c) si.v[c] = s[c];
                        Vec6 oo = kepler_beyond_series_tagged<1>(si, C.dt);
#pragma unroll
                        for (int c = 0; c < 6; ++c) o[c] = oo.v[c];
                    }
                }
            }
        } else if (PROP != 0) {
            if (__any(!kep_ok)) {
                asm volatile("");
                if (!kep_ok) {
#pragma unroll
                    for (int c = 0; c < 6; ++c) o[c] = __builtin_nan("");
                }
            }
        } else if (__any(!kep_ok)) {
            bool served = kep_ok;
            if (!ACT::late) {
                if (!kep_ok) served = kepler_conic_lean<2, true>(s, C.dt, o);
            }
            if (__any(!served)) {
                if (!served) {
                    Vec6 si;
#pragma unroll
                    for (int c = 0; c < 6; ++c) si.v[c] = s[c];
                    Vec6 oo = kepler_beyond_series_tagged<2>(si, C.dt);
#pragma unroll
                    for (int c = 0; c < 6; ++c) o[c] = oo.v[c];
                }
            }
        }
    }
    wave_lds_sync();
    asm volatile("" : "+v"(lane));
    g = lane >> 4;
    l = lane & 15;
    obj = base + g;
    e = (valid && p.n_env > 1) ? (int)((uint32_t)obj / (uint32_t)p.n_obj) : 0;
    if constexpr (ENVS) e = asrc.env;
    if constexpr (FCAST && LENVS) e = asrc.env;
    if (TILE == 1 && !ISSUE_LAST) tile_issue(pf, p, lane, next_base, next_cnt);

    {
        typedef double v2d_t __attribute__((ext_vector_type(2)));
        double d[6];
#pragma unroll
        for (int c = 0; c < 6; ++c) d[c] = o[c] - row_bcast<0>(o[c]);
        if (is_pm) {
            v2d_t* dst = reinterpret_cast<v2d_t*>(&t.D[dbase(g) + (l - 1) * 8]);
            dst[0] = v2d_t{d[0], d[1]};
            dst[1] = v2d_t{d[2], d[3]};
            dst[2] = v2d_t{d[4], d[5]};
            dst[3] = v2d_t{1.0, 0.0};
        } else if (l == 0 || l == 13) {
            v2d_t* dst = reinterpret_cast<v2d_t*>(l == 0 ? &t.X[g * 6] : &t.T[g * 6]);
            dst[0] = v2d_t{o[0], o[1]};
            dst[1] = v2d_t{o[2], o[3]};
            dst[2] = v2d_t{o[4], o[5]};
        }
    }
    wave_lds_sync();
    Moments mo = {0.0, 0.0, 0.0};
    if (C.flags & SSA_FLAG_REFERENCE_COV) mo = moment_sums_mfma<true>(t, lane);
    else mo = moment_sums_mfma(t, lane);
    wave_lds_sync();
    double xb_l = 0.0;
    if (l < 6) {
        const double s0 = t.X[g * 6 + l];
        const double ssum = C.Wi * t.M[g * 12 + l];
        const double mp = C.sum_wm_m1 * s0 + ssum;
        xb_l = s0 + mp;
        t.M[g * 12 + l] = ssum;
        t.M[g * 12 + 6 + l] = mp;
        t.X[g * 6 + l] = xb_l;
    }
    const bool nan_x = ((__ballot(l < 6 && xb_l != xb_l) >> (g * 16)) & 0xFFFFull) != 0;
    wave_lds_sync();
    if (C.flags & SSA_FLAG_REFERENCE_COV) covariance_reference(t, C, lane, o, xb_l);
    else covariance_finish(t, C, lane, mo);
    wave_lds_sync();

    int st_new = st_in;
    if (active) {
        if (chol_fail) st_new = SSA_ST_PREDICT_LINALG;
        else if (nan_x) st_new = SSA_ST_PREDICT_NAN;
    }
    if (C.flags & SSA_FLAG_RESAMPLE) {
        const int rg = robust_chol_row_lds(t, C.scale, g, l);
        wave_lds_sync();
        if (active && st_new == SSA_ST_OK && rg == 16) st_new = SSA_ST_PREDICT_LINALG;
    }
    const int st_pred = st_new;

    if (ACT::late) {
        asrc.before_wait(t, lane, cnt);
        act = asrc.get();
        my_update = valid && act >= 0 && (int64_t)act == (p.obj_ids ? (int64_t)t.Oid[g] : obj) && interval_ok;
        if (__any(my_update)) __builtin_amdgcn_s_setprio(3);
    }
    int look_s = 0;
look_pass:
    if constexpr (LSENS) st_new = st_pred;
    bool look_vis = false, look_taken = false;
    const ssa_sensor_params* SP = PASS_ARGS ? kernarg_opaque(asrc.sites()) : asrc.sites();
    if constexpr (ENVS) sid = valid ? sensor_index(asrc, SP, p.obj_ids ? (int64_t)t.Oid[g] : obj - (int64_t)asrc.env * p.n_obj) : -1;
    else if constexpr (SENS) sid = valid ? sensor_index(asrc, SP, p.obj_ids ? (int64_t)t.Oid[g] : obj) : -1;
    if (__any(my_update)) {
    bool upd_go = false, taken = false, visible = false, attempted = false;
    double z[3] = {0.0, 0.0, 0.0}, y_row[3] = {0.0, 0.0, 0.0};
    double* rec = nullptr;
    double* const STG = &t.UA[g * 117];
    double* const W = &t.D[330];
    static_assert(offsetof(Tiles, D) == offsetof(Tiles, UA) + sizeof(double) * OBJ_PER_WAVE * 36, "UA and D contiguous");
    static_assert(4 * 117 <= OBJ_PER_WAVE * 36 + 330 && 330 + 57 <= 408, "update staging fits");
    if (my_update) {
        if constexpr (SENS) rec = asrc.records(SP) ? asrc.records(SP) + (int64_t)sid * SSA_UPD_STRIDE : nullptr;
        else rec = (!ALL && p.upd) ? p.upd + (int64_t)e * SSA_UPD_STRIDE : nullptr;
        attempted = (st_new == SSA_ST_OK);
        if (attempted) {
            const double* M = &t.Obs[g * 12];
            double sf[6], xb[6];
#pragma unroll
            for (int c = 0; c < 6; ++c) {
                sf[c] = o[c];
                xb[c] = t.X[g * 6 + c];
            }
            if ((C.flags & SSA_FLAG_RESAMPLE) && (!LSENS || look_s == 0)) {
                const int krow = is_pm ? (l - 1) % 6 : 0;
                const double sgn = (l >= 1 && l <= 6) ? 1.0 : ((l >= 7 && l <= 12) ? -1.0 : 0.0);
#pragma unroll
                for (int c = 0; c < 6; ++c)
                    if (l != 13) sf[c] = xb[c] + sgn * t.UA[g * 36 + krow * 6 + c];
            }
            if constexpr (LSENS) {
                if (look_s == 0) {
                    if (l <= 12) {
#pragma unroll
                        for (int c = 0; c < 6; ++c) STG[l * 9 + c] = sf[c];
                    }
                } else {
#pragma unroll
                    for (int c = 0; c < 6; ++c) sf[c] = (l <= 12) ? STG[l * 9 + c] : t.T[g * 6 + c];
                }
            } else if (l <= 12) {
#pragma unroll
                for (int c = 0; c < 6; ++c) STG[l * 9 + c] = sf[c] - xb[c];
            }
            double enu_vec[3];
            double el_mine;
            double lim = 0.0;
            {
                double Mm[9], aer[3];
#pragma unroll
                for (int i = 0; i < 9; ++i) Mm[i] = M[i];
                if constexpr (SENS) {
                    for (;;) {
                        const int su = __builtin_amdgcn_readfirstlane(sid);
                        if (sid == su) {
                            hx_aer_enu(sf, Mm, SP->enu[su], SP->obs_itrs[su], aer, enu_vec);
                            lim = SP->obs_limit[su];
                            break;
                        }
                    }
                } else if constexpr (LSENS) {
                    hx_aer_enu(sf, Mm, SP->enu[look_s], SP->obs_itrs[look_s], aer, enu_vec);
                    lim = SP->obs_limit[look_s];
                } else hx_aer_enu(sf, Mm, C.enu, C.obs_itrs, aer, enu_vec);
                el_mine = aer[1];
                if (C.obs_type == SSA_OBS_AER) { z[0] = aer[0]; z[1] = aer[1]; z[2] = aer[2]; }
                else { z[0] = sf[0]; z[1] = sf[1]; z[2] = sf[2]; }
            }
            if constexpr (SENS || LSENS) visible = row_bcast<13>(el_mine) >= lim;
            else visible = row_bcast<13>(el_mine) >= C.obs_limit;
            if (rec && l == 13) {
#pragma unroll
                for (int c = 0; c < 3; ++c) rec[SSA_UPD_Z_TRUE + c] = z[c];
            }
            if (visible) {
                double zp[3];
                const double wl = (l == 0) ? C.Wc0 : (is_pm ? C.Wi : 0.0);
                if (C.obs_type == SSA_OBS_AER) {
                    double um[3];
#pragma unroll
                    for (int c = 0; c < 3; ++c) {
                        double u0 = row_bcast<0>(enu_vec[c]);
                        double du = is_pm ? (enu_vec[c] - u0) : 0.0;
                        um[c] = u0 + (C.sum_wm_m1 * u0 + C.Wi * row_allsum(du));
                    }
                    uvw2aer(um, zp);
                } else {
#pragma unroll
                    for (int c = 0; c < 3; ++c) {
                        double u0 = row_bcast<0>(z[c]);
                        double du = is_pm ? (z[c] - u0) : 0.0;
                        zp[c] = u0 + (C.sum_wm_m1 * u0 + C.Wi * row_allsum(du));
                    }
                }
                double rz[3];
                {
                    double zin[3];
                    if (l == 13) {
                        const double* zn = &t.Obs[g * 12 + 9];
#pragma unroll
                        for (int c = 0; c < 3; ++c) zin[c] = z[c] + zn[c];
                    } else {
#pragma unroll
                        for (int c = 0; c < 3; ++c) zin[c] = z[c];
                    }
                    if (C.obs_type == SSA_OBS_AER) residual_z_aer_wrapped(zin, zp, rz);
                    else {
#pragma unroll
                        for (int c = 0; c < 3; ++c) rz[c] = zin[c] - zp[c];
                    }
                }
                upd_go = true;
                if (l <= 12) {
#pragma unroll
                    for (int c = 0; c < 3; ++c) STG[l * 9 + 6 + c] = rz[c];
                }
                if (l == 13) {
#pragma unroll
                    for (int c = 0; c < 3; ++c) y_row[c] = rz[c];
                }
            }
        }
    }
    {
        unsigned long long pend = __ballot(upd_go);
        while (pend) {
            const int gu = (__ffsll((long long)pend) - 1) >> 4;
            pend &= ~(0xFFFFull << (gu * 16));
            const double* Rm = C.R;
            if constexpr (SENS) Rm = SP->R[__builtin_amdgcn_readlane(sid, gu * 16)];
            if constexpr (LSENS) Rm = SP->R[look_s];
            if (g == gu && l == 13) {
#pragma unroll
                for (int c = 0; c < 3; ++c) W[54 + c] = y_row[c];
            }
            wave_lds_sync();
            {
                const int kk = lane >> 4, blk = (lane >> 2) & 3, ij = lane & 3;
                const double* SG = &t.UA[gu * 117];
                const int acol = (blk < 2) ? 4 * blk + ij : 8;
                double acc = 0.0;
#pragma unroll
                for (int cch = 0; cch < 4; ++cch) {
                    const int k = (cch < 3) ? 4 * cch + kk : 12;
                    const double* row = &SG[k * 9];
                    double av = row[acol];
                    if constexpr (LSENS) {
                        if (acol < 6) av = av - t.X[gu * 6 + acol];
                    }
                    double bv = row[6 + (ij < 3 ? ij : 2)] * ((cch == 0 && kk == 0) ? C.Wc0 : C.Wi);
                    if (cch == 3 && kk != 0) { av = 0.0; bv = 0.0; }
                    acc = __builtin_amdgcn_mfma_f64_4x4x4f64(av, bv, acc, 0, 0, 0);
                }
                const int ri = 4 * blk + kk;
                if (ij < 3 && ri < 6) W[9 + ri * 3 + ij] = acc;
                if (ij < 3 && ri >= 6 && ri < 9 && ri - 6 <= ij) {
                    const int a = ri - 6;
                    W[a * 3 + ij] = acc + Rm[a * 3 + ij];
                    W[ij * 3 + a] = acc + Rm[ij * 3 + a];
                }
            }
            wave_lds_sync();
            bool inv_ok;
            double SI[9];
            {
                double S[9];
#pragma unroll
                for (int c = 0; c < 9; ++c) S[c] = W[c];
                inv_ok = inv3(S, SI);
            }
            bool nan_u = false;
            if (inv_ok) {
                if (lane < 18) {
                    const int a = lane / 3, b = lane - 3 * a;
                    W[36 + lane] = W[9 + a * 3] * SI[b] + W[9 + a * 3 + 1] * SI[3 + b] + W[9 + a * 3 + 2] * SI[6 + b];
                }
                wave_lds_sync();
                if constexpr (ALL) {
                    if (lane < 36) {
                        const int a = lane / 6, b = lane - 6 * a;
                        double corr = 0.0;
#pragma unroll
                        for (int u = 0; u < 3; ++u) {
                            const double sk = W[u * 3] * W[36 + b * 3] + W[u * 3 + 1] * W[36 + b * 3 + 1] + W[u * 3 + 2] * W[36 + b * 3 + 2];
                            corr = fma(W[36 + a * 3 + u], sk, corr);
                        }
                        t.UA[gu * 117 + (LSENS ? pp_at<1>(lane) : lane)] = t.P[gu * 36 + lane] - corr;
                    }
                } else {
                double xn = 0.0;
                if (lane < 6) xn = t.X[gu * 6 + lane] + (W[36 + lane * 3] * W[54] + W[36 + lane * 3 + 1] * W[55] + W[36 + lane * 3 + 2] * W[56]);
                nan_u = __ballot(lane < 6 && xn != xn) != 0;
                if (lane < 36) {
                    const int a = lane / 6, b = lane - 6 * a;
                    double corr = 0.0;
#pragma unroll
                    for (int u = 0; u < 3; ++u) {
                        const double sk = W[u * 3] * W[36 + b * 3] + W[u * 3 + 1] * W[36 + b * 3 + 1] + W[u * 3 + 2] * W[36 + b * 3 + 2];
                        corr = fma(W[36 + a * 3 + u], sk, corr);
                    }
                    t.P[gu * 36 + lane] = t.P[gu * 36 + lane] - corr;
                }
                if (lane < 6) t.X[gu * 6 + lane] = xn;
                }
            }
            if (g == gu) {
                if (!inv_ok) st_new = SSA_ST_UPDATE_LINALG;
                else {
                    taken = true;
                    if (nan_u) st_new = SSA_ST_UPDATE_NAN;
                    if (rec) {
                        if (l < 3) rec[SSA_UPD_Y + l] = W[54 + l];
                        if (l < 9) rec[SSA_UPD_S + l] = W[l];
                        if (is_sigma) {
#pragma unroll
                            for (int c = 0; c < 3; ++c) rec[SSA_UPD_SIGMAS_H + l * 3 + c] = z[c];
                        }
                    }
                }
            }
            wave_lds_sync();
        }
    }
    if (my_update && rec && l == 0) {
        rec[SSA_UPD_OBS_TAKEN] = taken ? 1.0 : 0.0;
        rec[SSA_UPD_VISIBLE] = visible ? 1.0 : 0.0;
        if constexpr (ENVS) rec[SSA_UPD_ACTION] = attempted ? (double)(p.obj_ids ? (int64_t)t.Oid[g] : obj - (int64_t)asrc.env * p.n_obj) : -1.0;
        else if constexpr (SENS) rec[SSA_UPD_ACTION] = attempted ? (double)(p.obj_ids ? (int64_t)t.Oid[g] : obj) : -1.0;
        else rec[SSA_UPD_ACTION] = attempted ? (double)(ACT::late ? act : env_action<INL, SEG>(p, e)) : -1.0;
    }
    if constexpr (ALL) {
        look_vis = visible;
        look_taken = taken;
    }
    asm volatile("" : "+v"(lane));
    g = lane >> 4;
    l = lane & 15;
    obj = base + g;
    e = (valid && p.n_env > 1) ? (int)((uint32_t)obj / (uint32_t)p.n_obj) : 0;
    if constexpr (ENVS) e = asrc.env;
    if constexpr (FCAST && LENVS) e = asrc.env;
    if (TILE == 1 && !ISSUE_LAST) tile_issue(pf, p, lane, next_base, next_cnt);
    }
    if (!ALL && valid && p.upd && obj == (int64_t)e * p.n_obj && l == 0) {
      const int a_env = ACT::late ? act : env_action<INL, SEG>(p, e);
      if (!(a_env >= 0 && interval_ok && (int64_t)a_env < p.n_obj)) {
        double* rec = p.upd + (int64_t)e * SSA_UPD_STRIDE;
        rec[SSA_UPD_OBS_TAKEN] = 0.0;
        rec[SSA_UPD_VISIBLE] = 0.0;
        rec[SSA_UPD_ACTION] = -1.0;
      }
    }
    if constexpr (ENVS) {
        if (asrc.records(SP) && valid && obj == (int64_t)asrc.env * p.n_obj && l == 0) {
            for (int k = 0; k < SP->n_sensor; ++k) {
                const int a = asrc.action(SP, k);
                bool owns = a >= 0 && (int64_t)a < p.n_obj && interval_ok;
                for (int q = 0; q < k; ++q)
                    if (asrc.action(SP, q) == a) owns = false;
                if (!owns) {
                    double* rec = asrc.records(SP) + (int64_t)k * SSA_UPD_STRIDE;
                    rec[SSA_UPD_OBS_TAKEN] = 0.0;
                    rec[SSA_UPD_VISIBLE] = 0.0;
                    rec[SSA_UPD_ACTION] = -1.0;
                }
            }
        }
    } else if constexpr (SENS) {
        if (asrc.records(SP) && valid && obj == 0 && l == 0) {
            for (int k = 0; k < SP->n_sensor; ++k) {
                const int a = asrc.action(SP, k);
                bool owns = a >= 0 && (int64_t)a < p.n_obj && interval_ok;
                for (int q = 0; q < k; ++q)
                    if (asrc.action(SP, q) == a) owns = false;
                if (!owns) {
                    double* rec = asrc.records(SP) + (int64_t)k * SSA_UPD_STRIDE;
                    rec[SSA_UPD_OBS_TAKEN] = 0.0;
                    rec[SSA_UPD_VISIBLE] = 0.0;
                    rec[SSA_UPD_ACTION] = -1.0;
                }
            }
        }
    }

    wave_lds_sync();
    if (valid && (ALL ? st_pred : st_new) != SSA_ST_OK && st_in == SSA_ST_OK) {
        for (int idx = l; idx < 36; idx += 16) {
            int a = idx / 6, b = idx - a * 6;
            t.P[g * 36 + idx] = (a == b) ? (a < 3 ? X_FAILED_POS : X_FAILED_VEL) : 0.0;
        }
        if (l < 6) t.X[g * 6 + l] = (l < 3) ? X_FAILED_POS : X_FAILED_VEL;
        if (!ALL && p.fail_log && l == 0) {
            if (ACT::late) asm volatile("s_waitcnt vmcnt(0)" ::: "memory");
            const double* xt = p.x_true_in + obj * 6;
            const double* xf = p.x_in + obj * 6;
            const double* Pd = p.P_in + obj * 36;
            const double a0 = xf[0] - xt[0], a1 = xf[1] - xt[1], a2 = xf[2] - xt[2];
            const double b0 = xf[3] - xt[3], b1 = xf[4] - xt[4], b2 = xf[5] - xt[5];
            const unsigned at = atomicAdd(p.fail_count, 1u);
            if ((int)at < p.fail_cap) {
                double* rec = p.fail_log + (int64_t)at * SSA_FAIL_STRIDE;
                rec[SSA_FAIL_ENV] = (double)e;
                rec[SSA_FAIL_OBJ] = p.obj_ids ? (double)t.Oid[g] : (double)(obj - (int64_t)e * p.n_obj);
                rec[SSA_FAIL_STATUS] = (double)st_new;
                rec[SSA_FAIL_TIME] = (double)((ACT::late ? p.env_time[0] : env_time_of<INL, SEG>(p, e)) + p.time_offset);
                rec[SSA_FAIL_ERR + 0] = sqrt(a0 * a0 + a1 * a1 + a2 * a2);
                rec[SSA_FAIL_ERR + 1] = sqrt(b0 * b0 + b1 * b1 + b2 * b2);
                rec[SSA_FAIL_ERR + 2] = sqrt(Pd[0] + Pd[7] + Pd[14]);
                rec[SSA_FAIL_ERR + 3] = sqrt(Pd[21] + Pd[28] + Pd[35]);
            }
        }
    }
    if constexpr (FCAST) {
        if (valid && st_in != SSA_ST_OK) {
            const bool at_entry = p.status[obj] != SSA_ST_OK;
            for (int idx = l; idx < 36; idx += 16) {
                const int a = idx / 6, b = idx - a * 6;
                t.P[g * 36 + idx] = at_entry ? p.P_in[obj * 36 + idx] : ((a == b) ? (a < 3 ? X_FAILED_POS : X_FAILED_VEL) : 0.0);
            }
            if (l < 6) t.X[g * 6 + l] = at_entry ? p.x_in[obj * 6 + l] : ((l < 3) ? X_FAILED_POS : X_FAILED_VEL);
        }
        if (l == 0) t.St[g] = st_pred;
    } else {
    if (valid && st_in != SSA_ST_OK) {
        if (ACT::late) asm volatile("s_waitcnt vmcnt(0)" ::: "memory");
        for (int idx = l; idx < 36; idx += 16) t.P[g * 36 + idx] = p.P_in[obj * 36 + idx];
        if (l < 6) t.X[g * 6 + l] = p.x_in[obj * 6 + l];
    }
    if (l == 0) t.St[g] = st_new;
    }
    wave_lds_sync();
    if constexpr (LSENS) {
        const bool last = look_s + 1 >= SP->n_sensor;
        if (TILE == 1 && ISSUE_LAST && last) tile_issue(pf, p, lane, next_base, next_cnt);
        ssa_lookahead_out os = PASS_ARGS ? *kernarg_opaque(asrc.o) : *asrc.o;
        if constexpr (FCAST) asrc.slab(os, p.n_obj, SP->n_sensor);
        if constexpr (LENVS && !FCAST) asrc.slab(os, p.n_obj, SP->n_sensor);
        if (look_s > 0) os.x_prior = os.P_prior = nullptr;
        if constexpr (LENVS) {
            if (valid) lookahead_store<1>(t, os, g, l, (int64_t)look_s * p.n_obj + (p.obj_ids ? (int64_t)t.Oid[g] : obj - (int64_t)asrc.env * p.n_obj),
                                          st_new, look_vis, look_taken);
        } else {
        if (valid) lookahead_store<1>(t, os, g, l, (int64_t)look_s * p.n_obj + (p.obj_ids ? (int64_t)t.Oid[g] : obj), st_new, look_vis, look_taken);
        }
        if (!last) {
            ++look_s;
            wave_lds_sync();
            goto look_pass;
        }
        return;
    } else if constexpr (ALL) {
        if (valid) lookahead_store(t, *asrc.o, g, l, (int64_t)e * p.n_obj + (p.obj_ids ? (int64_t)t.Oid[g] : obj - (int64_t)e * p.n_obj),
                                   st_new, look_vis, look_taken);
        return;
    }
    observe_rows(t, g, l, cnt != OBJ_PER_WAVE);
    if (p.aer_out && p.stat_shards) {
        if (l < 4 && valid) aer_obs_tile<INL, SEG>(t, p, C, g, l, e, p.obj_ids ? (int64_t)e * p.n_obj + t.Oid[g] : obj);
    }
    wave_lds_sync();
    if (!ACT::late) {
        if (p.spos_tiles && p.stat_shards && lane == 0) {
            unsigned long long key, idx;
            spos_tile_best(t, cnt, obj - (int64_t)e * p.n_obj, key, idx, p.obj_ids != nullptr);
            unsigned long long* slot = (unsigned long long*)p.spos_tiles + 2 * (int64_t)tile;
            __hip_atomic_store(slot, key, __ATOMIC_RELAXED, __HIP_MEMORY_SCOPE_AGENT);
            __hip_atomic_store(slot + 1, idx, __ATOMIC_RELAXED, __HIP_MEMORY_SCOPE_AGENT);
        }
        store_tile<TILE != 1>(t, p, lane, base, cnt);
        const bool one_env = p.n_env == 1 || ((uint32_t)base / (uint32_t)p.n_obj == (uint32_t)(base + cnt - 1) / (uint32_t)p.n_obj);
        if (FROM_METRICS && (p.launch_mask & SSA_LAUNCH_STATS_FROM_METRICS)) {
            const unsigned long long failed = __ballot(valid && st_new != 0) & 0x0001000100010001ull;
            if (failed && lane == 63) {
                unsigned long long* sh = (unsigned long long*)p.stat_shards + (int64_t)(tile & (SSA_STAT_SHARDS - 1)) * SSA_STAT_SHARD_WORDS;
                atomicAdd(sh + 2, (unsigned long long)__popcll(failed));
            }
        } else if (p.stat_shards && one_env) {
            const double dp = t.Met[g * 4 + 0];
            const bool rv = g < cnt;
            const unsigned long long rowbit = 0x0001000100010001ull;
            const unsigned c4 = (unsigned)__popcll(__ballot(rv && dp < 1e4) & rowbit);
            const unsigned c7 = (unsigned)__popcll(__ballot(rv && dp < 1e7) & rowbit);
            const unsigned nfl = (unsigned)__popcll(__ballot(rv && t.St[g] != 0) & rowbit);
            unsigned long long mx = rv ? ((unsigned long long)__double_as_longlong(dp) & 0x7fffffffffffffffull) : 0ull;
#define SSA_XROW(CTRL, ROWMASK)                                                                                          \
            {                                                                                                            \
                const unsigned long long m2 = ((unsigned long long)(unsigned)__builtin_amdgcn_update_dpp(0, (int)(mx >> 32), CTRL, ROWMASK, 0xF, false) << 32) | \
                                              (unsigned)__builtin_amdgcn_update_dpp(0, (int)(mx & 0xffffffffull), CTRL, ROWMASK, 0xF, false);                 \
                mx = m2 > mx ? m2 : mx;                                                                                  \
            }
            SSA_XROW(0x142, 0xA)
            SSA_XROW(0x143, 0xC)
#undef SSA_XROW
            bool i_fold = false;
            if (lane == 63) {
                const int64_t e_tile = (p.n_env > 1) ? (int64_t)((uint32_t)base / (uint32_t)p.n_obj) : 0;
                unsigned long long* sh = (unsigned long long*)p.stat_shards + ((e_tile * SSA_STAT_SHARDS) + (tile & (SSA_STAT_SHARDS - 1))) * SSA_STAT_SHARD_WORDS;
                atomicMax(sh, mx);
                atomicAdd(sh + 1, (unsigned long long)c4 | ((unsigned long long)c7 << 32));
                if (nfl) atomicAdd(sh + 2, (unsigned long long)nfl);
                if (FOLD_OK && (p.launch_mask & SSA_LAUNCH_FOLD_INSIDE)) {
                    asm volatile("s_waitcnt vmcnt(0)" ::: "memory");
                    i_fold = stat_tile_counted(p, e_tile, tile);
                }
            }
            if (FOLD_OK && (p.launch_mask & SSA_LAUNCH_FOLD_INSIDE) && __any(i_fold)) {
                const int64_t e_tile = (p.n_env > 1) ? (int64_t)((uint32_t)base / (uint32_t)p.n_obj) : 0;
                fold_stat_shards_inside((unsigned long long*)p.stat_shards + e_tile * SSA_STAT_SHARDS * SSA_STAT_SHARD_WORDS,
                                        p.stats + e_tile * SSA_STAT_STRIDE, lane);
                if (p.spos_tiles) {
                    int t_lo, t_hi;
                    env_tile_range(p.n_obj, (int)e_tile, t_lo, t_hi);
                    fold_spos_tiles<true>((const unsigned long long*)p.spos_tiles, t_lo, t_hi, p.stats + e_tile * SSA_STAT_STRIDE, lane);
                }
            }
        } else if (p.stat_shards) {
          unsigned fold_envs = 0u;
          const int64_t e_first = (p.n_env > 1) ? (int64_t)((uint32_t)base / (uint32_t)p.n_obj) : 0;
          if (lane == 0) {
            int64_t e_cur = -1;
            unsigned long long mx = 0ull, cnts = 0ull, nf = 0ull;
            int64_t j_run = base - e_first * p.n_obj, e_run = e_first;
            for (int gg = 0; gg <= cnt; ++gg) {
                while (j_run >= p.n_obj) { j_run -= p.n_obj; ++e_run; }
                const int64_t eg = (gg < cnt) ? e_run : -2;
                ++j_run;
                if (eg != e_cur) {
                    if (e_cur >= 0) {
                        unsigned long long* sh = (unsigned long long*)p.stat_shards + ((e_cur * SSA_STAT_SHARDS) + (tile & (SSA_STAT_SHARDS - 1))) * SSA_STAT_SHARD_WORDS;
                        atomicMax(sh, mx);
                        atomicAdd(sh + 1, cnts);
                        if (nf) atomicAdd(sh + 2, nf);
                        if (FOLD_OK && (p.launch_mask & SSA_LAUNCH_FOLD_INSIDE)) {
                            asm volatile("s_waitcnt vmcnt(0)" ::: "memory");
                            if (stat_tile_counted(p, e_cur, tile)) fold_envs |= 1u << (unsigned)(e_cur - e_first);
                        }
                    }
                    e_cur = eg; mx = 0ull; cnts = 0ull; nf = 0ull;
                }
                if (gg < cnt) {
                    const double dp = t.Met[gg * 4 + 0];
                    unsigned long long bits = (unsigned long long)__double_as_longlong(dp) & 0x7fffffffffffffffull;
                    mx = bits > mx ? bits : mx;
                    cnts += (unsigned long long)(dp < 1e4) + ((unsigned long long)(dp < 1e7) << 32);
                    nf += t.St[gg] != 0;
                }
            }
          }
          if (FOLD_OK && (p.launch_mask & SSA_LAUNCH_FOLD_INSIDE)) {
              fold_envs = (unsigned)__builtin_amdgcn_readfirstlane((int)fold_envs);
              for (int i = 0; i < OBJ_PER_WAVE; ++i)
                  if (fold_envs & (1u << i))
                      fold_stat_shards_inside((unsigned long long*)p.stat_shards + (e_first + i) * SSA_STAT_SHARDS * SSA_STAT_SHARD_WORDS,
                                              p.stats + (e_first + i) * SSA_STAT_STRIDE, lane);
          }
        }
        if (tile == 0) {
            if (p.stat_shards_clear) {
                unsigned long long* z = (unsigned long long*)p.stat_shards_clear;
                for (int i = lane; i < p.n_env * SSA_STAT_SHARDS * 4; i += 64) z[(i >> 2) * SSA_STAT_SHARD_WORDS + (i & 3)] = 0ull;
            }
        }
    }
}

SSA_DEV void fold_stat_shards(unsigned long long* __restrict__ shards, double* __restrict__ stats, int e, int lane,
                              const unsigned long long* __restrict__ spos = nullptr, int64_t n_obj = 0)
{
    static_assert(SSA_STAT_SHARDS == 128, "two shards per lane");
    unsigned long long* sh = shards + ((int64_t)e * SSA_STAT_SHARDS + lane) * SSA_STAT_SHARD_WORDS;
    unsigned long long* sh2 = sh + 64 * SSA_STAT_SHARD_WORDS;
    unsigned long long mx = sh[0], cn = sh[1], nf = sh[2];
    const unsigned long long mb = sh2[0], cb = sh2[1], nb = sh2[2];
    sh[0] = 0ull; sh[1] = 0ull; sh[2] = 0ull;
    sh2[0] = 0ull; sh2[1] = 0ull; sh2[2] = 0ull;
    mx = mb > mx ? mb : mx;
    cn += cb;
    nf += nb;
#pragma unroll
    for (int off = 32; off > 0; off >>= 1) {
        unsigned long long m2 = __shfl_down(mx, off, 64), c2 = __shfl_down(cn, off, 64), n2 = __shfl_down(nf, off, 64);
        mx = m2 > mx ? m2 : mx;
        cn += c2;
        nf += n2;
    }
    if (lane == 0 && stats) {
        double* o = stats + (int64_t)e * SSA_STAT_STRIDE;
        o[SSA_STAT_MAX_DPOS] = __longlong_as_double((long long)mx);
        o[SSA_STAT_CNT_LT_1E4] = (double)(cn & 0xffffffffull);
        o[SSA_STAT_CNT_LT_1E7] = (double)(cn >> 32);
        o[SSA_STAT_ARGMAX_SPOS] = -1.0;
        o[SSA_STAT_N_FAILED] = (double)nf;
        o[SSA_STAT_MAX_SPOS] = __builtin_nan("");
        o[6] = 0.0; o[7] = 0.0;
    }
    if (spos && stats) {
        int t_lo, t_hi;
        env_tile_range(n_obj, e, t_lo, t_hi);
        fold_spos_tiles<false>(spos, t_lo, t_hi, stats + (int64_t)e * SSA_STAT_STRIDE, lane);
    }
}
__global__ void __launch_bounds__(64) reward_fold_kernel(unsigned long long* __restrict__ shards, double* __restrict__ stats,
                                                         const unsigned long long* __restrict__ spos, int64_t n_obj)
{
    fold_stat_shards(shards, stats, blockIdx.x, threadIdx.x, spos, n_obj);
}

__global__ void __launch_bounds__(64) reward_service_kernel(const double* __restrict__ dpos, unsigned long long* __restrict__ shards,
                                                            double* __restrict__ stats, const unsigned long long* __restrict__ spos, int64_t n_obj)
{
    stats_service_wave(dpos, shards, stats, spos, n_obj, blockIdx.x, gridDim.x, threadIdx.x);
}

SSA_DEV int xcd_tile(int b, int n)
{
    const int x = b & 7, i = b >> 3, q = n >> 3, r = n & 7;
    return x * q + (x < r ? x : r) + i;
}

SSA_DEV void rotate_issue_priority(unsigned wave_slot, unsigned turn)
{
    switch ((wave_slot + turn) & 3u) {
        case 0: __builtin_amdgcn_s_setprio(0); break;
        case 1: __builtin_amdgcn_s_setprio(1); break;
        case 2: __builtin_amdgcn_s_setprio(2); break;
        default: __builtin_amdgcn_s_setprio(3); break;
    }
}

template <class K> struct TileArgs {
    int ntiles, nwork;
    const double *pre_P_in, *pre_x_in, *pre_x_true_in;
    const int32_t* pre_status;
    K k;
};
template <class K> using KernargPtr = ConstPtr<K>;
static_assert(offsetof(TileArgs<StepK>, k) == 40 && offsetof(StepK, p) == sizeof(ssa_consts), "the step's parameter block in the argument segment");
SSA_DEV ConstPtr<ssa_step_params> tile_kernel_params()
{
    return (ConstPtr<ssa_step_params>)((const char*)__builtin_amdgcn_kernarg_segment_ptr() + offsetof(TileArgs<StepK>, k) + offsetof(StepK, p));
}
struct LookK {
    StepK k;
    ssa_lookahead_out o;
};
struct SensK {
    StepK k;
    ssa_sensor_params s;
};
struct LookSensK {
    LookK k;
    ssa_sensor_params s;
};
struct VecLookSensK {
    LookK k;
    ssa_sensor_params s;
};
struct VecSensK {
    StepK k;
    ssa_sensor_params s;
    ssa_sensor_envs_params v;
};
SSA_DEV const StepK& step_of(const StepK& k) { return k; }
SSA_DEV const StepK& step_of(const LookK& k) { return k.k; }
SSA_DEV const StepK& step_of(const SensK& k) { return k.k; }
SSA_DEV const StepK& step_of(const LookSensK& k) { return k.k.k; }
SSA_DEV const StepK& step_of(const VecLookSensK& k) { return k.k.k; }
SSA_DEV ConstPtr<int32_t> vector_sensors_inline_rows()
{
    return (ConstPtr<int32_t>)((const char*)__builtin_amdgcn_kernarg_segment_ptr() + offsetof(TileArgs<VecSensK>, k) + offsetof(VecSensK, v) +
                               offsetof(ssa_sensor_envs_params, inline_action));
}
SSA_DEV const StepK& step_of(const VecSensK& k) { return k.k; }
SSA_DEV ActEarly act_of(const StepK&) { return ActEarly(); }
SSA_DEV ActAll act_of(const LookK& k) { return ActAll{{}, &k.o}; }
SSA_DEV ActSensors act_of(const SensK& k) { return ActSensors{{}, &k.s}; }
SSA_DEV ActLookSensors act_of(const LookSensK& k) { return ActLookSensors{{}, &k.k.o, &k.s}; }
SSA_DEV ActLookSensorEnvs act_of(const VecLookSensK& k) { return ActLookSensorEnvs{{}, &k.k.o, &k.s, 0}; }
SSA_DEV ActSensorEnvs act_of(const VecSensK& k) { return ActSensorEnvs{{}, &k.s, &k.v, 0, nullptr, nullptr}; }
enum : unsigned {
    WALK_STEP = 1,
    WALK_ONE_ENV = 2,
    WALK_ACT_SEGMENT = 4,
    WALK_BASE_PER_TILE = 8
};
#define SSA_TILE_KERNEL(NAME, K, WALK)                                                                                                        \
    template <int PROP, bool MULTI>                                                                                                           \
    __global__ void __launch_bounds__(64, SSA_STEP_WAVES) NAME(int ntiles, int nwork, const double* pre_P_in, const double* pre_x_in,         \
                                                               const double* pre_x_true_in, const int32_t* pre_status, const K k_arg)         \
    {                                                                                                                                         \
        __shared__ Tiles t;                                                                                                                   \
        int lane = threadIdx.x;                                                                                                               \
        const int unit = (int)blockIdx.x;                                                                                                     \
        if (((WALK) & WALK_STEP) && unit >= nwork) {                                                                                          \
            const ssa_step_params& p = step_of(k_arg).p;                                                                                      \
            if (!MULTI && !((WALK) & WALK_ONE_ENV) && (p.launch_mask & SSA_LAUNCH_STATS_FROM_METRICS))                                        \
                stats_service_wave(p.metrics_prev, (unsigned long long*)p.stat_shards_prev, p.stats_prev,                                     \
                                   (const unsigned long long*)p.spos_tiles_prev, p.n_obj, unit - nwork, (int)gridDim.x - nwork, lane);        \
            else                                                                                                                              \
                fold_stat_shards((unsigned long long*)p.stat_shards_prev, p.stats_prev, unit - nwork, lane,                                   \
                                 (const unsigned long long*)p.spos_tiles_prev, p.n_obj);                                                      \
            return;                                                                                                                           \
        }                                                                                                                                     \
        const int64_t total = ((WALK) & WALK_ONE_ENV) ? step_of(k_arg).p.n_obj : (int64_t)step_of(k_arg).p.n_env * step_of(k_arg).p.n_obj;    \
        TileRegs pf;                                                                                                                          \
        int tile = xcd_tile(unit, nwork);                                                                                                     \
        if (!MULTI) {                                                                                                                         \
            const int64_t base = (int64_t)tile * OBJ_PER_WAVE;                                                                                \
            const bool whole = tile < ntiles;                                  \
                   \
            tile_dma_issue(t, pf, pre_P_in, pre_x_in, pre_x_true_in, pre_status, lane, base, whole, step_of(k_arg).p,                         \
                           ((WALK) & WALK_ONE_ENV) != 0);                                                                                     \
            int cnt = OBJ_PER_WAVE;                                                                                                           \
            asm volatile("" : "+s"(cnt));                                                                                                     \
            if (!whole) cnt = (int)(tile_total(step_of(k_arg).p, ((WALK) & WALK_ONE_ENV) != 0) - base);                                       \
            const K& ka = ((WALK) & WALK_ACT_SEGMENT)                                                                                         \
                              ? *(const K*)(KernargPtr<K>)((const char*)__builtin_amdgcn_kernarg_segment_ptr() + offsetof(TileArgs<K>, k))    \
                              : k_arg;                                                                                                        \
            auto act = act_of(ka);                                                                                                            \
            process_wave<PROP, 0>(t, step_of(k_arg).c, step_of(k_arg).p, lane, base + (lane >> 4), (lane >> 4) < cnt, base, cnt, pf, 0, 0,    \
                                  tile, act);                                                                                                 \
            return;                                                                                                                           \
        }                                                                                                                                     \
        {                                                                                                                                     \
            const int64_t b0 = (int64_t)tile * OBJ_PER_WAVE;                                                                                  \
            tile_issue(pf, step_of(k_arg).p, lane, b0, tile < ntiles ? (int)((total - b0) < OBJ_PER_WAVE ? (total - b0) : OBJ_PER_WAVE) : 0); \
        }                                                                                                                                     \
        constexpr size_t pre_off = ((WALK) & WALK_BASE_PER_TILE) ? 0 : offsetof(TileArgs<K>, k);                                              \
        KernargPtr<K> kp = (KernargPtr<K>)((const char*)__builtin_amdgcn_kernarg_segment_ptr() + pre_off);                                    \
        unsigned wave_slot, turn = 0;                                                                                                         \
        if ((WALK) & WALK_STEP) asm volatile("s_getreg_b32 %0, hwreg(HW_REG_HW_ID, 0, 4)" : "=s"(wave_slot));                                 \
        for (; tile < ntiles; tile += nwork) {                                                                                                \
            if ((WALK) & WALK_STEP) rotate_issue_priority(wave_slot, turn++);                                                                 \
            asm volatile("" : "+s"(kp));                                                                                                      \
            asm volatile("" : "+v"(lane));                                                                                                    \
            const K& k = *(const K*)((const char*)kp + (offsetof(TileArgs<K>, k) - pre_off));                                                 \
            const int64_t base = (int64_t)tile * OBJ_PER_WAVE;                                                                                \
            const int cnt = (int)((total - base) < OBJ_PER_WAVE ? (total - base) : OBJ_PER_WAVE);                                             \
            const int nt = tile + nwork;                                                                                                      \
            const int64_t nbase = (int64_t)nt * OBJ_PER_WAVE;                                                                                 \
            const int ncnt = nt < ntiles ? (int)((total - nbase) < OBJ_PER_WAVE ? (total - nbase) : OBJ_PER_WAVE) : 0;                        \
            auto act = act_of(k);                                                                                                             \
            process_wave<PROP, 1>(t, step_of(k).c, step_of(k).p, lane, base + (lane >> 4), (lane >> 4) < cnt, base, cnt, pf, nbase, ncnt,     \
                                  tile, act);                                                                                                 \
            wave_lds_sync();                                                                                                                  \
        }                                                                                                                                     \
    }

SSA_TILE_KERNEL(step_fast_kernel, StepK, WALK_STEP | WALK_BASE_PER_TILE)
SSA_TILE_KERNEL(lookahead_kernel, LookK, 0)
SSA_TILE_KERNEL(lookahead_sensors_kernel, LookSensK, WALK_ONE_ENV | WALK_ACT_SEGMENT)
SSA_TILE_KERNEL(step_sensors_kernel, SensK, WALK_STEP | WALK_ONE_ENV)
SSA_TILE_KERNEL(vector_sensors_kernel, VecSensK, WALK_STEP)
SSA_TILE_KERNEL(lookahead_sensor_envs_kernel, VecLookSensK, WALK_ACT_SEGMENT)
#undef SSA_TILE_KERNEL

struct RollK {
    StepK k;
    ssa_rollout_params r;
};
struct RollSensK {
    RollK k;
    ssa_sensor_params s;
    ssa_rollout_sensors_params rs;
};
SSA_DEV const RollK& roll_of(const RollK& a) { return a; }
SSA_DEV const RollK& roll_of(const RollSensK& a) { return a.k; }
SSA_DEV const StepK& step_of(const RollK& a) { return a.k; }
SSA_DEV const StepK& step_of(const RollSensK& a) { return a.k.k; }
SSA_DEV int roll_envs(const RollK& a) { return a.k.p.n_env; }
SSA_DEV int roll_envs(const RollSensK&) { return 1; }
struct Ring {
    int E, H, K_steps;
    int64_t total, sx, sP, so_, sm, su;
};
SSA_DEV Ring ring_of(const RollK& a, int E)
{
    const int H = a.r.history, K_steps = a.r.n_steps;
    const int64_t total = (int64_t)E * a.k.p.n_obj;
    return Ring{E, H, K_steps, total, total * 6, total * 36, total * 12, (int64_t)E * 4 * a.k.p.n_obj, (int64_t)E * SSA_UPD_STRIDE};
}
SSA_DEV Ring roll_plan(const RollK& a) { return ring_of(a, roll_envs(a)); }
SSA_DEV Ring roll_plan(const RollSensK& a) { return ring_of(a.k, roll_envs(a)); }
SSA_DEV ssa_step_params roll_source(const RollK& a, const Ring& g)
{
    const int si0 = (a.r.slot_out + g.H - 1) % g.H;
    ssa_step_params p0 = a.k.p;
    p0.x_true_in = a.r.x_true_ring + si0 * g.sx;
    p0.x_in = a.r.x_ring + si0 * g.sx;
    p0.P_in = a.r.P_ring + si0 * g.sP;
    return p0;
}
SSA_DEV ssa_step_params roll_source(const RollSensK& a, const Ring& g) { return roll_source(a.k, g); }
SSA_DEV ActEarly ring_act(const RollK&, ssa_step_params&, int, int, bool) { return ActEarly(); }
SSA_DEV ActSchedule ring_act(const RollSensK& a, ssa_step_params& pk, int kk, int so, bool owns)
{
    pk.upd = nullptr;
    pk.actions = nullptr;
    return ActSchedule{{}, &a.s, a.rs.actions + (int64_t)kk * SSA_MAX_SENSORS,
                       (a.rs.upd_ring && owns) ? a.rs.upd_ring + (int64_t)so * a.s.n_sensor * SSA_UPD_STRIDE : nullptr};
}
template <class K>
SSA_DEV auto roll_act(const Ring& g, const K& ka, ssa_step_params& pk, int kk, int ntiles)
{
    const int E = g.E, H = g.H, K_steps = g.K_steps;
    const int64_t sx = g.sx, sP = g.sP, so_ = g.so_, sm = g.sm, su = g.su;
    const StepK& k = roll_of(ka).k;
    const ssa_rollout_params& r = roll_of(ka).r;
    const int so = (r.slot_out + kk) % H, si = (so + H - 1) % H;
    pk = k.p;
    pk.time_offset = k.p.time_offset + kk;
    pk.x_true_in = r.x_true_ring + si * sx;  pk.x_true_out = r.x_true_ring + so * sx;
    pk.x_in = r.x_ring + si * sx;            pk.x_out = r.x_ring + so * sx;
    pk.P_in = r.P_ring + si * sP;            pk.P_out = r.P_ring + so * sP;
    pk.obs = r.obs_ring + so * so_;
    pk.metrics = r.metrics_ring + so * sm;
    pk.upd = (r.upd_ring && kk >= K_steps - H) ? r.upd_ring + so * su : nullptr;
    pk.actions = r.actions + (int64_t)kk * E;
    pk.stat_shards = r.stat_shards + (int64_t)kk * E * SSA_STAT_SHARDS * SSA_STAT_SHARD_WORDS;
    pk.spos_tiles = r.spos_tiles ? r.spos_tiles + (int64_t)kk * ntiles * 2 : nullptr;
    pk.aer_out = nullptr;
    return ring_act(ka, pk, kk, so, kk >= K_steps - H);
}
#define SSA_RESIDENT_KERNEL(NAME, K)                                                                                                          \
    template <int PROP>                                                                                                                       \
    __global__ void __launch_bounds__(64, SSA_STEP_WAVES) NAME(const K a, int ntiles, int nwork)                                              \
    {                                                                                                                                         \
        __shared__ Tiles t;                                                                                                                   \
        int lane = threadIdx.x;                                                                                                               \
        const auto plan = roll_plan(a);                                                                                                       \
        const int K_steps = plan.K_steps;                                                                                                     \
        const int64_t total = plan.total;                                                                                                     \
        TileRegs pf;                                                                                                                          \
        typedef const __attribute__((address_space(4))) K* RollArgPtr;                                                                        \
        RollArgPtr kp = (RollArgPtr)__builtin_amdgcn_kernarg_segment_ptr();                                                                   \
        for (int tile = xcd_tile((int)blockIdx.x, nwork); tile < ntiles; tile += nwork) {                                                     \
            const int64_t base = (int64_t)tile * OBJ_PER_WAVE;                                                                                \
            const int cnt = (int)((total - base) < OBJ_PER_WAVE ? (total - base) : OBJ_PER_WAVE);                                             \
            {                                                                                                                                 \
                const ssa_step_params p0 = roll_source(a, plan);                                                                              \
                wave_lds_sync();                                                     \
                tile_issue(pf, p0, lane, base, cnt);                                                                                          \
                tile_commit(t, pf, lane);                                                                                                     \
                if (lane < 36) t.Q[lane] = step_of(a).c.Q[lane];                  \
            }                                                                                                                                 \
            unsigned wave_slot;                                                        \
            asm volatile("s_getreg_b32 %0, hwreg(HW_REG_HW_ID, 0, 4)" : "=s"(wave_slot));                                                     \
            for (int kk = 0; kk < K_steps; ++kk) {                                                                                            \
                rotate_issue_priority(wave_slot, (unsigned)kk);                                                                               \
                asm volatile("" : "+s"(kp));                  \
                asm volatile("" : "+v"(lane));                                                                                                \
                const K& ka = *(const K*)kp;                                                                                                  \
                ssa_step_params pk;                                                                                                           \
                auto act = roll_act(plan, ka, pk, kk, ntiles);                                                                                \
                process_wave<PROP, 2>(t, step_of(ka).c, pk, lane, base + (lane >> 4), (lane >> 4) < cnt, base, cnt, pf, 0, 0, tile, act);     \
                wave_lds_sync();                                                                                                              \
            }                                                                                                                                 \
        }                                                                                                                                     \
    }
SSA_RESIDENT_KERNEL(rollout_kernel, RollK)
SSA_RESIDENT_KERNEL(rollout_sensors_kernel, RollSensK)

struct ForeSensK {
    StepK k;
    ssa_sensor_params s;
    ssa_forecast_params f;
};
SSA_DEV const StepK& step_of(const ForeSensK& a) { return a.k; }
struct ForePlan {
    int K_steps;
    int64_t total;
};
SSA_DEV ForePlan roll_plan(const ForeSensK& a) { return ForePlan{a.f.n_steps, a.k.p.n_obj}; }
SSA_DEV ssa_step_params roll_source(const ForeSensK& a, ForePlan) { return a.k.p; }
SSA_DEV ActForecastSensors roll_act(ForePlan, const ForeSensK& ka, ssa_step_params& pk, int h, int)
{
    pk = ka.k.p;
    pk.time_offset = ka.k.p.time_offset + h;
    return ActForecastSensors{{}, &ka.f.out, &ka.s, h};
}
SSA_RESIDENT_KERNEL(forecast_sensors_kernel, ForeSensK)
struct VecForeSensK {
    StepK k;
    ssa_sensor_params s;
    ssa_forecast_params f;
};
SSA_DEV ConstPtr<int32_t> forecast_envs_inline_time()
{
    return (ConstPtr<int32_t>)((const char*)__builtin_amdgcn_kernarg_segment_ptr() + offsetof(VecForeSensK, k) + offsetof(StepK, p) +
                               offsetof(ssa_step_params, inline_time));
}
SSA_DEV const StepK& step_of(const VecForeSensK& a) { return a.k; }
SSA_DEV ForePlan roll_plan(const VecForeSensK& a) { return ForePlan{a.f.n_steps, (int64_t)a.k.p.n_env * a.k.p.n_obj}; }
SSA_DEV ssa_step_params roll_source(const VecForeSensK& a, ForePlan) { return a.k.p; }
SSA_DEV ActForecastSensorEnvs roll_act(ForePlan, const VecForeSensK& ka, ssa_step_params& pk, int h, int)
{
    pk = ka.k.p;
    pk.time_offset = ka.k.p.time_offset + h;
    return ActForecastSensorEnvs{{}, &ka.f.out, &ka.s, h, ka.k.p.n_env, 0};
}
SSA_RESIDENT_KERNEL(forecast_sensor_envs_kernel, VecForeSensK)
struct VecRollSensK {
// ... 1403 lines not shown
static inline unsigned nblk(int64_t n, int bs) { return (unsigned)((n + bs - 1) / bs); }


constexpr int PEER_SPLIT = 8;
__global__ void __launch_bounds__(256) peer_push_kernel(const double* __restrict__ src, int64_t n_words, double* const* __restrict__ dst,
                                                        unsigned long long* const* __restrict__ flag,
                                                        const unsigned long long* __restrict__ seq_base, unsigned long long seq_off,
                                                        const unsigned long long* __restrict__ prev_flags, long long timeout_ticks,
                                                        int32_t* __restrict__ error, unsigned int* __restrict__ tickets)
{
    const int r = blockIdx.x, sl = blockIdx.y, t = threadIdx.x;
    const unsigned long long seq = seq_base[0] + seq_off;
    if (prev_flags && seq >= 2ull) {
        if (t == 0) {
            const long long t0 = (long long)wall_clock64();
            while (__hip_atomic_load(&prev_flags[r], __ATOMIC_ACQUIRE, __HIP_MEMORY_SCOPE_SYSTEM) < seq - 1ull) {
                if ((long long)wall_clock64() - t0 > timeout_ticks) {
                    if (error) atomicMax(error, 1 + r);
                    break;
                }
                __builtin_amdgcn_s_sleep(8);
            }
        }
        __syncthreads();
    }
    double* __restrict__ d = dst[r];
    int64_t chunk = (n_words + gridDim.y - 1) / gridDim.y;
    chunk += chunk & 1;
    const int64_t lo = (int64_t)sl * chunk, hi = (lo + chunk < n_words) ? lo + chunk : n_words;
    if (lo < hi) {
        const bool wide = ((reinterpret_cast<uintptr_t>(d) | reinterpret_cast<uintptr_t>(src)) & 15) == 0;
        if (wide) {
            const double2* __restrict__ s2 = reinterpret_cast<const double2*>(src + lo);
            double2* __restrict__ d2 = reinterpret_cast<double2*>(d + lo);
            const int64_t n2 = (hi - lo) >> 1;
            for (int64_t i = t; i < n2; i += blockDim.x) d2[i] = s2[i];
            if (((hi - lo) & 1) && t == 0) d[hi - 1] = src[hi - 1];
        } else {
            for (int64_t i = lo + t; i < hi; i += blockDim.x) d[i] = src[i];
        }
    }
    __threadfence_system();
    __syncthreads();
    if (t == 0 && atomicInc(&tickets[r], gridDim.y - 1) == gridDim.y - 1) {
        __threadfence_system();
        __hip_atomic_store(flag[r], seq, __ATOMIC_RELEASE, __HIP_MEMORY_SCOPE_SYSTEM);
    }
}
__global__ void __launch_bounds__(64) peer_wait_kernel(const unsigned long long* __restrict__ flags, int32_t n_src,
                                                       const unsigned long long* __restrict__ seq_base, unsigned long long seq_off,
                                                       long long timeout_ticks, int32_t* __restrict__ error)
{
    const unsigned long long want = seq_base[0] + seq_off;
    const long long t0 = (long long)wall_clock64();
    for (int r = threadIdx.x; r < n_src; r += 64) {
        while (__hip_atomic_load(&flags[r], __ATOMIC_ACQUIRE, __HIP_MEMORY_SCOPE_SYSTEM) < want) {
            if ((long long)wall_clock64() - t0 > timeout_ticks) {
                if (error) atomicMax(error, 1 + r);
                break;
            }
            __builtin_amdgcn_s_sleep(8);
        }
    }
}

}

using namespace ssa;

template <class F> static void with_prop(int prop, F&& f)
{
    if (prop == SSA_PROP_FG) f(std::integral_constant<int, SSA_PROP_FG>());
    else if (prop == SSA_PROP_ELEMENTS) f(std::integral_constant<int, SSA_PROP_ELEMENTS>());
    else if (prop == SSA_PROP_HYBRID) f(std::integral_constant<int, SSA_PROP_HYBRID>());
    else f(std::integral_constant<int, SSA_PROP_J2_RK4>());
}
template <class F> static void with_prop(int prop, bool multi, F&& f)
{
    with_prop(prop, [&](auto P) {
        if (multi) f(P, std::true_type());
        else f(P, std::false_type());
    });
}

extern "C" {

int ssa_abi_version(void) { return SSA_ABI_VERSION; }
const char* ssa_build_info(void) { return "libssa_hip gfx950 fp64 (" __DATE__ " " __TIME__ ")"; }

static int device_cu_count()
{
    static int cached = 0;
    if (cached <= 0) {
        int dev = 0, n = 0;
        if (hipGetDevice(&dev) != hipSuccess || hipDeviceGetAttribute(&n, hipDeviceAttributeMultiprocessorCount, dev) != hipSuccess || n <= 0) n = 256;
        cached = n;
    }
    return cached;
}
static int post_parts(int64_t n_obj, int32_t n_env)
{
    (void)n_env;
    int64_t want = (n_obj + POST_T - 1) / POST_T;
    if (want < 1) want = 1;
    if (want > 256) want = 256;
    return (int)want;
}
static bool consts_ok(const ssa_consts* c)
{
    if (c->obs_type != SSA_OBS_AER && c->obs_type != SSA_OBS_XYZ) return false;
    if (c->propagator != SSA_PROP_FG && c->propagator != SSA_PROP_ELEMENTS && c->propagator != SSA_PROP_J2_RK4 && c->propagator != SSA_PROP_HYBRID) return false;
    return c->propagator != SSA_PROP_J2_RK4 || (c->rk4_substeps >= 1 && c->rk4_substeps <= 4096);
}
struct TileGrid {
    int64_t ntiles, per_wave;
    int nwork, arg;
};
static TileGrid tile_grid(int64_t total)
{
    TileGrid g;
    g.ntiles = (total + OBJ_PER_WAVE - 1) / OBJ_PER_WAVE;
    const int64_t slots = (int64_t)device_cu_count() * 4 * SSA_STEP_WAVES;
    g.per_wave = (g.ntiles + slots - 1) / slots;
    g.nwork = (int)((g.ntiles + g.per_wave - 1) / g.per_wave);
    g.arg = g.per_wave != 1 ? (int)g.ntiles : (int)(total / OBJ_PER_WAVE);
    return g;
}
static bool ragged_envs(int64_t n_obj, int32_t n_env) { return n_env > 1 && (n_obj % OBJ_PER_WAVE) != 0; }
static bool ragged_envs(const ssa_step_params* p) { return ragged_envs(p->n_obj, p->n_env); }
static bool rows_fit(int64_t a, int64_t b, int64_t c = 1) { return a * b * c < ((int64_t)1 << 31); }
static bool row_aligned(const int32_t* row) { return row && ((uintptr_t)row % (SSA_MAX_SENSORS * sizeof(int32_t))) == 0; }
static bool inline_envs_fit(const ssa_step_params* p) { return !(p->launch_mask & SSA_LAUNCH_INLINE_ENVS) || p->n_env <= SSA_INLINE_ENVS; }
static int sites_ok(const ssa_sensor_params* sp, int between = SSA_OK)
{
    if (sp->n_sensor < 1 || sp->n_sensor > SSA_MAX_SENSORS) return SSA_E_INVALID;
    if (between != SSA_OK) return between;
    for (int k = 0; k < sp->n_sensor; ++k)
        if (!(sp->obs_limit[k] == sp->obs_limit[k])) return SSA_E_INVALID;
    return SSA_OK;
}
static int sensors_ok(const ssa_sensor_params* sp, const ssa_step_params* p) { return sites_ok(sp, p->n_env != 1 ? SSA_E_UNSUPPORTED : SSA_OK); }
static bool noise_stride_ok(const ssa_sensor_params* sp)
{
    return sp->zn_stride_sensor >= 0 && (sp->n_sensor <= 1 || sp->zn_stride_sensor != 0);
}
static ssa_sensor_params idle_sites(const ssa_sensor_params* sp)
{
    ssa_sensor_params s = *sp;
    s.upd = nullptr;
    for (int q = 0; q < SSA_MAX_SENSORS; ++q) s.action[q] = -1;
    return s;
}

static int step_launch(const ssa_consts* c, const ssa_step_params* p, void* stream, hipEvent_t ev0, hipEvent_t ev1,
                       const ssa_sensor_params* sens = nullptr, const ssa_sensor_envs_params* envs = nullptr)
{
    if (!c || !p || p->n_obj <= 0 || p->n_env <= 0) return SSA_E_INVALID;
    if (!p->x_true_in || !p->x_true_out || !p->x_in || !p->x_out || !p->P_in || !p->P_out || !p->status ||
        !p->obs || !p->metrics || !p->trans || !p->env_time || !p->z_noise || !p->stat_ws)
        return SSA_E_INVALID;
    if (sens) {
    } else if (p->launch_mask & SSA_LAUNCH_INLINE_ENVS) {
        if (!inline_envs_fit(p) || (p->launch_mask & SSA_LAUNCH_INLINE_ACTION)) return SSA_E_INVALID;
    } else if (p->launch_mask & SSA_LAUNCH_INLINE_ACTION) {
        if (p->n_env != 1) return SSA_E_INVALID;
    } else if (!p->actions) return SSA_E_INVALID;
    if ((p->launch_mask & SSA_LAUNCH_FOLD_INSIDE) &&
        (!p->stat_shards || !p->stats || (p->launch_mask & SSA_LAUNCH_DEFER_FOLD))) return SSA_E_INVALID;
    if (p->spos_tiles && !p->stat_shards) return SSA_E_INVALID;
    if (p->fail_log && (!p->fail_count || p->fail_cap <= 0)) return SSA_E_INVALID;
    if ((p->launch_mask & SSA_LAUNCH_MIRROR_F32) && !p->stat_shards) return SSA_E_UNSUPPORTED;
    if (p->obj_ids && (!p->stat_shards || ragged_envs(p))) return SSA_E_UNSUPPORTED;
    if ((p->spos_tiles || p->spos_tiles_prev) && ragged_envs(p)) return SSA_E_UNSUPPORTED;
    if (!consts_ok(c)) return SSA_E_INVALID;
    if (p->aer_cols != 0 && p->aer_cols != 1 && p->aer_cols != 4) return SSA_E_INVALID;
    StepK k;
    k.c = *c;
    k.p = *p;
    if (!rows_fit(p->n_env, p->n_obj)) return SSA_E_INVALID;
    const TileGrid g = tile_grid((int64_t)p->n_env * p->n_obj);
    const bool fast_stats = p->stat_shards != nullptr;
    const bool defer = fast_stats && (p->launch_mask & SSA_LAUNCH_DEFER_FOLD);
    if (defer && p->stat_shards_prev && (!p->stats_prev || p->stat_shards_prev == p->stat_shards)) return SSA_E_INVALID;
    const bool from_metrics = (p->launch_mask & SSA_LAUNCH_STATS_FROM_METRICS) != 0;
    if (from_metrics) {
        if (!defer || sens || p->n_env != 1 || g.per_wave != 1 || (p->launch_mask & SSA_LAUNCH_FOLD_INSIDE) || p->stat_shards_clear)
            return SSA_E_UNSUPPORTED;
        if (p->stat_shards_prev && !p->metrics_prev) return SSA_E_INVALID;
    }
    const int nfold = (defer && p->stat_shards_prev) ? (from_metrics ? STAT_SERVICE_WAVES : p->n_env) : 0;
    dim3 grid((unsigned)(g.nwork + nfold)), block(64);
    const int nparts = post_parts(p->n_obj, p->n_env);
    StatAcc* parts = (StatAcc*)p->stat_ws;
    hipStream_t s = (hipStream_t)stream;
    const unsigned mask = (p->launch_mask & 7u) ? (p->launch_mask & 7u) : 7u;
    const int prop = c->propagator;
    if ((mask & 1u) && envs) {
        VecSensK kv;
        kv.k = k;
        kv.k.p.upd = nullptr;
        kv.k.p.actions = nullptr;
        kv.s = idle_sites(sens);
        kv.v = *envs;
        with_prop(prop, g.per_wave != 1, [&](auto P, auto M) {
            hipExtLaunchKernelGGL((vector_sensors_kernel<P, M>), grid, block, 0, s, ev0, ev1, 0, g.arg, g.nwork, p->P_in, p->x_in, p->x_true_in, p->status, kv);
        });
    } else if ((mask & 1u) && sens) {
        SensK ks;
        ks.k = k;
        ks.k.p.upd = nullptr;
        ks.k.p.actions = nullptr;
        ks.k.p.launch_mask &= ~SSA_LAUNCH_INLINE_ACTION;
        ks.s = *sens;
        with_prop(prop, g.per_wave != 1, [&](auto P, auto M) {
            hipExtLaunchKernelGGL((step_sensors_kernel<P, M>), grid, block, 0, s, ev0, ev1, 0, g.arg, g.nwork, p->P_in, p->x_in, p->x_true_in, p->status, ks);
        });
    } else if (mask & 1u) {
        with_prop(prop, g.per_wave != 1, [&](auto P, auto M) {
            hipExtLaunchKernelGGL((step_fast_kernel<P, M>), grid, block, 0, s, ev0, ev1, 0, g.arg, g.nwork, p->P_in, p->x_in, p->x_true_in, p->status, k);
        });
    }
    if (fast_stats) {
        if ((p->launch_mask & SSA_LAUNCH_FOLD_INSIDE) && g.per_wave == 1) return launch_status();
        if ((mask & 6u) && !defer && p->stats)
            hipLaunchKernelGGL(reward_fold_kernel, dim3(p->n_env), dim3(64), 0, s, (unsigned long long*)p->stat_shards, p->stats,
                               (const unsigned long long*)p->spos_tiles, p->n_obj);
        return launch_status();
    }
    if (mask & 2u)
        with_prop(prop, [&](auto P) { hipLaunchKernelGGL(step_post_kernel<P>, dim3(nparts, p->n_env), dim3(POST_T), 0, s, k, parts, nparts); });
    if ((mask & 4u) && p->stats)
        hipLaunchKernelGGL(reward_final_kernel, dim3(p->n_env), dim3(64), 0, s, (const StatAcc*)parts, p->stats, nparts);
    return launch_status();
}
int32_t ssa_stats_from_metrics_waves(int64_t n_obj, int32_t n_env)
{
    if (n_obj <= 0 || n_env != 1) return 0;
    return tile_grid(n_obj).per_wave == 1 ? STAT_SERVICE_WAVES : 0;
}
int ssa_stats_fold_metrics_f64(const double* metrics, uint64_t* stat_shards, const uint64_t* spos_tiles, double* stats, int64_t n_obj,
                               void* stream)
{
    if (!metrics || !stat_shards || !stats || n_obj <= 0 || n_obj >= ((int64_t)1 << 31)) return SSA_E_INVALID;
    hipLaunchKernelGGL(reward_service_kernel, dim3(STAT_SERVICE_WAVES), dim3(64), 0, (hipStream_t)stream, metrics,
                       (unsigned long long*)stat_shards, stats, (const unsigned long long*)spos_tiles, n_obj);
    return launch_status();
}
int ssa_env_step_f64(const ssa_consts* c, const ssa_step_params* p, void* stream)
{
    return step_launch(c, p, stream, nullptr, nullptr);
}
int ssa_env_step_sensors_f64(const ssa_consts* c, const ssa_step_params* p, const ssa_sensor_params* sp, void* stream)
{
    if (!c || !p || !sp) return SSA_E_INVALID;
    const int rc = sensors_ok(sp, p);
    if (rc != SSA_OK) return rc;
    if (!noise_stride_ok(sp)) return SSA_E_INVALID;
    return step_launch(c, p, stream, nullptr, nullptr, sp);
}
int ssa_env_step_sensors_envs_f64(const ssa_consts* c, const ssa_step_params* p, const ssa_sensor_params* sp,
                                  const ssa_sensor_envs_params* envs, void* stream)
{
    if (!c || !p || !sp || !envs) return SSA_E_INVALID;
    if (sites_ok(sp) != SSA_OK || !noise_stride_ok(sp)) return SSA_E_INVALID;
    if ((p->launch_mask & SSA_LAUNCH_INLINE_ACTION) || !inline_envs_fit(p)) return SSA_E_INVALID;
    if (!(p->launch_mask & SSA_LAUNCH_INLINE_ENVS) && !row_aligned(envs->actions)) return SSA_E_INVALID;
    if (ragged_envs(p) || (p->launch_mask & SSA_LAUNCH_STATS_FROM_METRICS)) return SSA_E_UNSUPPORTED;
    return step_launch(c, p, stream, nullptr, nullptr, sp, envs);
}
static hipEvent_t g_prof_ev[SSA_PROFILE_SLOTS][2];
static bool g_prof_made[SSA_PROFILE_SLOTS];
int ssa_env_step_profiled_f64(const ssa_consts* c, const ssa_step_params* p, void* stream, int32_t slot)
{
    if (slot < 0 || slot >= SSA_PROFILE_SLOTS) return SSA_E_INVALID;
    if (!g_prof_made[slot]) {
        if (hipEventCreate(&g_prof_ev[slot][0]) != hipSuccess || hipEventCreate(&g_prof_ev[slot][1]) != hipSuccess) return SSA_E_LAUNCH;
        g_prof_made[slot] = true;
    }
    return step_launch(c, p, stream, g_prof_ev[slot][0], g_prof_ev[slot][1]);
}
int ssa_env_step_profile_ms(int32_t slot, float* kernel_ms)
{
    if (slot < 0 || slot >= SSA_PROFILE_SLOTS || !kernel_ms || !g_prof_made[slot]) return SSA_E_INVALID;
    if (hipEventSynchronize(g_prof_ev[slot][1]) != hipSuccess ||
        hipEventElapsedTime(kernel_ms, g_prof_ev[slot][0], g_prof_ev[slot][1]) != hipSuccess) return SSA_E_LAUNCH;
    return SSA_OK;
}
static int lookahead_args(const ssa_consts* c, const ssa_step_params* p, const ssa_lookahead_out* o, LookK& k)
{
    if (!c || !p || !o || p->n_obj <= 0 || p->n_env <= 0) return SSA_E_INVALID;
    if (!p->x_true_in || !p->x_in || !p->P_in || !p->status || !p->trans || !p->env_time) return SSA_E_INVALID;
    if (!o->score || !o->status || !o->visible) return SSA_E_INVALID;
    if (!inline_envs_fit(p)) return SSA_E_INVALID;
    if (p->obj_ids && ragged_envs(p)) return SSA_E_UNSUPPORTED;
    if (!consts_ok(c) || !rows_fit(p->n_env, p->n_obj)) return SSA_E_INVALID;
    k.k.c = *c;
    k.k.p = *p;
    k.o = *o;
    ssa_step_params& q = k.k.p;
    q.x_true_out = nullptr; q.x_out = nullptr; q.P_out = nullptr; q.obs = nullptr; q.metrics = nullptr; q.upd = nullptr;
    q.actions = nullptr; q.z_noise = nullptr; q.stats = nullptr; q.work = nullptr; q.stat_ws = nullptr;
    q.stat_shards = nullptr; q.stat_shards_prev = nullptr; q.stats_prev = nullptr; q.aer_out = nullptr; q.stat_shards_clear = nullptr;
    q.metrics_prev = nullptr;
    q.obs_mirror = nullptr; q.spos_tiles = nullptr; q.spos_tiles_prev = nullptr; q.fail_log = nullptr; q.fail_count = nullptr;
    q.fail_cap = 0;
    q.launch_mask = p->launch_mask & SSA_LAUNCH_INLINE_ENVS;
    return SSA_OK;
}
int ssa_lookahead_f64(const ssa_consts* c, const ssa_step_params* p, const ssa_lookahead_out* o, void* stream)
{
    LookK k;
    const int rc = lookahead_args(c, p, o, k);
    if (rc != SSA_OK) return rc;
    const TileGrid g = tile_grid((int64_t)p->n_env * p->n_obj);
    dim3 grid((unsigned)g.nwork), block(64);
    hipStream_t s = (hipStream_t)stream;
    with_prop(c->propagator, g.per_wave != 1, [&](auto P, auto M) {
        hipLaunchKernelGGL((lookahead_kernel<P, M>), grid, block, 0, s, g.arg, g.nwork, p->P_in, p->x_in, p->x_true_in, p->status, k);
    });
    return launch_status();
}
static int lookahead_sensors_args(const ssa_consts* c, const ssa_step_params* p, const ssa_sensor_params* sp, const ssa_lookahead_out* o,
                                  bool envs, LookK& k, ssa_sensor_params& sites)
{
    if (!c || !p || !sp || !o) return SSA_E_INVALID;
    int rc = envs ? sites_ok(sp) : sensors_ok(sp, p);
    if (rc != SSA_OK) return rc;
    rc = lookahead_args(c, p, o, k);
    if (rc != SSA_OK) return rc;
    if (!rows_fit(p->n_env, sp->n_sensor, p->n_obj)) return SSA_E_INVALID;
    if (ragged_envs(p)) return SSA_E_UNSUPPORTED;
    sites = idle_sites(sp);
    return SSA_OK;
}
int ssa_lookahead_sensors_f64(const ssa_consts* c, const ssa_step_params* p, const ssa_sensor_params* sp, const ssa_lookahead_out* o,
                              void* stream)
{
    LookSensK k;
    const int rc = lookahead_sensors_args(c, p, sp, o, false, k.k, k.s);
    if (rc != SSA_OK) return rc;
    const TileGrid g = tile_grid(p->n_obj);
    dim3 grid((unsigned)g.nwork), block(64);
    hipStream_t s = (hipStream_t)stream;
    with_prop(c->propagator, g.per_wave != 1, [&](auto P, auto M) {
        hipLaunchKernelGGL((lookahead_sensors_kernel<P, M>), grid, block, 0, s, g.arg, g.nwork, p->P_in, p->x_in, p->x_true_in, p->status, k);
    });
    return launch_status();
}
int ssa_lookahead_sensors_envs_f64(const ssa_consts* c, const ssa_step_params* p, const ssa_sensor_params* sp, const ssa_lookahead_out* o,
                                   void* stream)
{
    VecLookSensK k;
    const int rc = lookahead_sensors_args(c, p, sp, o, true, k.k, k.s);
    if (rc != SSA_OK) return rc;
    const TileGrid g = tile_grid((int64_t)p->n_env * p->n_obj);
    dim3 grid((unsigned)g.nwork), block(64);
    hipStream_t s = (hipStream_t)stream;
    with_prop(c->propagator, g.per_wave != 1, [&](auto P, auto M) {
        hipLaunchKernelGGL((lookahead_sensor_envs_kernel<P, M>), grid, block, 0, s, g.arg, g.nwork, p->P_in, p->x_in, p->x_true_in, p->status, k);
    });
    return launch_status();
}
int ssa_forecast_sensors_f64(const ssa_consts* c, const ssa_step_params* p, const ssa_sensor_params* sp, const ssa_forecast_params* f,
                             void* stream)
{
    if (!f) return SSA_E_INVALID;
    LookK lk;
    ForeSensK k;
    const int rc = lookahead_sensors_args(c, p, sp, &f->out, false, lk, k.s);
    if (rc != SSA_OK) return rc;
    if (f->n_steps < 1) return SSA_E_INVALID;
    k.k = lk.k;
    k.k.p.launch_mask = 0;
    k.f = *f;
    const TileGrid g = tile_grid(p->n_obj);
    hipStream_t s = (hipStream_t)stream;
    with_prop(c->propagator, [&](auto P) { hipLaunchKernelGGL(forecast_sensors_kernel<P>, dim3(g.nwork), dim3(64), 0, s, k, (int)g.ntiles, g.nwork); });
    return launch_status();
}
int ssa_forecast_sensors_envs_f64(const ssa_consts* c, const ssa_step_params* p, const ssa_sensor_params* sp, const ssa_forecast_params* f,
                                  void* stream)
{
    if (!f) return SSA_E_INVALID;
    LookK lk;
    VecForeSensK k;
    const int rc = lookahead_sensors_args(c, p, sp, &f->out, true, lk, k.s);
    if (rc != SSA_OK) return rc;
    if (f->n_steps < 1) return SSA_E_INVALID;
    k.k = lk.k;
    k.f = *f;
    const TileGrid g = tile_grid((int64_t)p->n_env * p->n_obj);
    hipStream_t s = (hipStream_t)stream;
    with_prop(c->propagator, [&](auto P) { hipLaunchKernelGGL(forecast_sensor_envs_kernel<P>, dim3(g.nwork), dim3(64), 0, s, k, (int)g.ntiles, g.nwork); });
    return launch_status();
}
static int rollout_args(const ssa_consts* c, const ssa_step_params* p, const ssa_rollout_params* r, bool sens, RollK& rk, bool ids_per_env = false)
{
    if (!c || !p || !r || p->n_obj <= 0 || p->n_env <= 0 || r->n_steps < 1 || r->history < 2) return SSA_E_INVALID;
    if (r->slot_out < 0 || r->slot_out >= r->history) return SSA_E_INVALID;
    if (!r->x_true_ring || !r->x_ring || !r->P_ring || !r->obs_ring || !r->metrics_ring || !r->stats_ring || (!sens && !r->actions) ||
        !r->stat_shards)
        return SSA_E_INVALID;
    if (!p->status || !p->trans || !p->env_time || !p->z_noise) return SSA_E_INVALID;
// ... 492 lines not shown
```

### ssa-gym_amd/engine.py

```python
import ctypes as C

import numpy as np
import torch

from . import _lib, device

f64 = torch.float64


class _Snapshot(tuple):
    order = None


class HotPathEngine:
    def __init__(self, consts, n_obj, n_env, trans, z_noise, history, device_name="cuda",
                 zn_stride_env=None, zn_stride_time=None, zn_stride_obj=3):
        _lib.load()
        if not torch.cuda.is_available():
            raise _lib.SsaHipError("no GPU visible: the ssa-gym hot path runs on MI355X only (no CPU fallback)")
        self.consts = consts
        self.m, self.E, self.H = int(n_obj), int(n_env), int(history)
        if self.H < 2:
            raise ValueError("history depth must be >= 2")
        self.dev = torch.device(device_name)
        N = self.m * self.E
        d = self.dev
        self.x_true = torch.zeros((self.H, N, 6), dtype=f64, device=d)
        self.x_filter = torch.zeros((self.H, N, 6), dtype=f64, device=d)
        self.P_filter = torch.zeros((self.H, N, 6, 6), dtype=f64, device=d)
        self.obs = torch.zeros((self.H, N, 12), dtype=f64, device=d)
        self.metrics = torch.full((self.H, self.E, 4, self.m), float("nan"), dtype=f64, device=d)
        self.stats = torch.zeros((self.H, self.E, _lib.STAT_STRIDE), dtype=f64, device=d)
        self.upd = torch.zeros((self.H, self.E, _lib.UPD_STRIDE), dtype=f64, device=d)
        self.status = torch.zeros(N, dtype=torch.int32, device=d)
        self.trans = device.as_dev(np.asarray(trans, dtype=np.float64).reshape(-1, 9), d)
        self.n_time = self.trans.shape[0]
        self.z_noise = z_noise if isinstance(z_noise, torch.Tensor) else device.as_dev(z_noise, d)
        self.zn_stride_time = self.m * 3 if zn_stride_time is None else int(zn_stride_time)
        self.zn_stride_env = self.n_time * self.m * 3 if zn_stride_env is None else int(zn_stride_env)
        self.time_actions = torch.zeros(2 * self.E, dtype=torch.int32, device=d)
        self.time_actions[self.E:] = -1
        self.env_time0 = self.time_actions[:self.E]
        self.actions = self.time_actions[self.E:]
        self._p = _lib.ssa_step_params()
        self._p.n_obj, self._p.n_env = self.m, self.E
        self._p.status = self.status.data_ptr()
        self._p.trans = self.trans.data_ptr()
        self._p.env_time = self.env_time0.data_ptr()
        need = (self.E - 1) * self.zn_stride_env + (self.n_time - 1) * self.zn_stride_time + (self.m - 1) * int(zn_stride_obj) + 3
        if min(self.zn_stride_env, self.zn_stride_time, int(zn_stride_obj)) < 0 or self.z_noise.numel() < need \
                or self.z_noise.dtype != torch.float64 or not self.z_noise.is_contiguous():
            raise _lib.SsaHipError("z_noise: %d contiguous float64 values needed for (n_env=%d, n_time=%d, n_obj=%d) with strides "
                                   "(%d, %d, %d), got %s of %d" % (need, self.E, self.n_time, self.m, self.zn_stride_env,
                                                                   self.zn_stride_time, int(zn_stride_obj), self.z_noise.dtype,
                                                                   self.z_noise.numel()))
        self._p.z_noise = self.z_noise.data_ptr()
        self._p.zn_stride_env, self._p.zn_stride_time = self.zn_stride_env, self.zn_stride_time
        self._p.zn_stride_obj = int(zn_stride_obj)
        self._p.n_time = self.n_time
        self._lib = _lib.load()
        self._stats_ws = device.stats_workspace(self.E, d)
        self.work = torch.zeros(self._lib.ssa_env_step_work_bytes(self.m, self.E) // 4, dtype=torch.int32, device=d)
        self._p.work, self._p.stat_ws, self._p.launch_mask = self.work.data_ptr(), self._stats_ws.data_ptr(), 0
        self.fail_log_host = torch.zeros((N, _lib.FAIL_STRIDE), dtype=f64).pin_memory()
        self.fail_log = self.fail_log_host.numpy()
        self.fail_count = torch.zeros(1, dtype=torch.int32, device=d)
        self._p.fail_log, self._p.fail_count, self._p.fail_cap = self.fail_log_host.data_ptr(), self.fail_count.data_ptr(), N
        self._shard_sets = torch.zeros((2, self.E, _lib.STAT_SHARDS, _lib.STAT_SHARD_WORDS), dtype=torch.int64, device=d)
        self.stat_shards = self._shard_sets[0]
        self._shard_cur = 0
        self._fold_pending = None
        self.stats_from_metrics = int(self._lib.ssa_stats_from_metrics_waves(self.m, self.E)) > 0
        self._shard_ptr = [self._shard_sets[0].data_ptr(), self._shard_sets[1].data_ptr()]
        self.ntiles = (N + 3) // 4
        self.supports_argmax = self.E == 1 or self.m % 4 == 0
        self._spos_sets = None
        self._actions_ptr = self.actions.data_ptr()
        self._order = None
        self._roll_shards = self._roll_spos = None
        self._roll_sched = self.upd_sensors = None
        self._roll_envs_out = None
        self._loop_ws = self._agent_ws = None
        self._look = self._look_s = None
        self._fore = None
        self._assign_ws = None
        self._assign_row = None
        self._sensor_envs = None
        self._look_se = None
        self._assign_envs_ws = None
        self._fore_e = None
        self._pcache = {}
        self._cref = C.byref(self.consts)
        self._pref = C.byref(self._p)
        self._sx, self._sP, self._so = N * 6 * 8, N * 36 * 8, N * 12 * 8
        self._sm, self._ss, self._su = self.E * 4 * self.m * 8, self.E * _lib.STAT_STRIDE * 8, self.E * _lib.UPD_STRIDE * 8
        self._bx_t, self._bx, self._bP = self.x_true.data_ptr(), self.x_filter.data_ptr(), self.P_filter.data_ptr()
        self._bo, self._bm, self._bs, self._bu = (self.obs.data_ptr(), self.metrics.data_ptr(), self.stats.data_ptr(),
                                                  self.upd.data_ptr())

    def set_layout(self, order):
        if order is None and self._order is None:
            return
        if order is not None:
            order = np.asarray(order, dtype=np.int64)
            if self.E == 1:
                order = order.reshape(-1)
            if order.shape != ((self.m,) if self.E == 1 else (self.E, self.m)) or \
                    not np.array_equal(np.sort(order.reshape(self.E, self.m), axis=1), np.broadcast_to(np.arange(self.m), (self.E, self.m))):
                raise _lib.SsaHipError("set_layout: `order` must be a permutation of 0 .. n_obj - 1 (one per env)")
            if self.E > 1 and self.m % 4:
                raise _lib.SsaHipError("a storage layout with several envs needs n_obj % 4 == 0 (whole tiles per env)")
        self._order = None
        self._p.obj_ids = 0
        self._pcache.clear()
        if order is None:
            return
        self._order = order.copy()
        self._obj_ids = torch.full((4 * self.ntiles,), -1, dtype=torch.int32, device=self.dev)
        self._p.obj_ids = self._obj_ids.data_ptr()
        self._upload_layout()

    def _upload_layout(self):
        N = self.m * self.E
        rows = (self._order.reshape(self.E, self.m) + (np.arange(self.E, dtype=np.int64) * self.m)[:, None]).reshape(-1)
        self._obj_ids[:N].copy_(torch.as_tensor(self._order.reshape(-1).astype(np.int32)))
        self._order_idx = torch.as_tensor(rows).to(self.dev)
        self._slot_of = torch.as_tensor(np.argsort(rows)).to(self.dev)
        self._slot_of32 = self._slot_of.to(torch.int32)

    def set_env_layout(self, e, order):
        if self._order is None or self.E == 1:
            raise _lib.SsaHipError("set_env_layout: set_layout([n_env][n_obj]) first")
        order = np.asarray(order, dtype=np.int64).reshape(-1)
        if order.shape[0] != self.m or not np.array_equal(np.sort(order), np.arange(self.m)):
            raise _lib.SsaHipError("set_env_layout: `order` must be a permutation of 0 .. n_obj - 1")
        self._order[e] = order
        self._upload_layout()

    def _reorder(self, idx, slots):
        N = self.m * self.E
        for sl in slots:
            for tns in (self.x_true, self.x_filter, self.P_filter, self.obs):
                tns[sl].copy_(tns[sl].index_select(0, idx))
            mt = self.metrics[sl].reshape(self.E, 4, self.m).permute(1, 0, 2).reshape(4, N).index_select(1, idx)
            self.metrics[sl].copy_(mt.reshape(4, self.E, self.m).permute(1, 0, 2).reshape(self.metrics[sl].shape))
        self.status.copy_(self.status.index_select(0, idx))

    def caller_rows(self, tensor):
        return tensor if self._order is None else tensor.index_select(0, self._slot_of)

    def to_caller_order(self):
        if self._order is None:
            return
        self.flush_stats()
        self._reorder(self._slot_of, range(self.H))
        self.set_layout(None)

    def load_state(self, slot, x_true, x_filter, P_filter):
        N = self.m * self.E
        self.flush_stats()
        self.x_true[slot].copy_(device.as_dev(np.asarray(x_true).reshape(N, 6), self.dev))
        self.x_filter[slot].copy_(device.as_dev(np.asarray(x_filter).reshape(N, 6), self.dev))
        self.P_filter[slot].copy_(device.as_dev(np.asarray(P_filter).reshape(N, 6, 6), self.dev))
        self.status.zero_()
        self.fail_count.zero_()
        for e in range(self.E):
            sl = slice(e * self.m, (e + 1) * self.m)
            device.observe(self.x_true[slot, sl], self.x_filter[slot, sl], self.P_filter[slot, sl],
                           obs=self.obs[slot, sl], metrics=self.metrics[slot, e])
        device.reward_stats(self.metrics[slot], self.status, self.m, self.E, out=self.stats[slot])
        if self._order is not None:
            self._reorder(self._order_idx, [slot])

    def load_env_state(self, slot, e, x_true, x_filter, P_filter):
        sl = slice(e * self.m, (e + 1) * self.m)
        self.x_true[slot, sl].copy_(device.as_dev(np.asarray(x_true).reshape(self.m, 6), self.dev))
        self.x_filter[slot, sl].copy_(device.as_dev(np.asarray(x_filter).reshape(self.m, 6), self.dev))
        self.P_filter[slot, sl].copy_(device.as_dev(np.ascontiguousarray(np.broadcast_to(P_filter, (self.m, 6, 6))), self.dev))
        self.status[sl].zero_()
        device.observe(self.x_true[slot, sl], self.x_filter[slot, sl], self.P_filter[slot, sl],
                       obs=self.obs[slot, sl], metrics=self.metrics[slot, e])
        device.reward_stats(self.metrics[slot, e:e + 1], self.status[sl], self.m, 1, out=self.stats[slot, e:e + 1])
        if self._order is not None:
            idx = torch.as_tensor(self._order.reshape(self.E, self.m)[e]).to(self.dev)
            for tns in (self.x_true, self.x_filter, self.P_filter, self.obs):
                tns[slot, sl].copy_(tns[slot, sl].index_select(0, idx))
            self.metrics[slot, e].copy_(self.metrics[slot, e].reshape(4, self.m).index_select(1, idx).reshape(self.metrics[slot, e].shape))

    def env_caller_rows(self, e, tensor):
        if self._order is None:
            return tensor
        idx = self._slot_of[e * self.m:(e + 1) * self.m] - e * self.m
        return tensor.index_select(0, idx)

    def snapshot(self, slot):
        snap = _Snapshot((self.x_true[slot].clone(), self.x_filter[slot].clone(), self.P_filter[slot].clone(),
                          self.obs[slot].clone(), self.metrics[slot].clone(), self.stats[slot].clone()))
        snap.order = None if self._order is None else self._order.copy()
        return snap

    def restore(self, slot, snap):
        order = getattr(snap, "order", None)
        if (order is None) != (self._order is None) or (order is not None and not np.array_equal(order, self._order)):
            self.flush_stats()
            self.set_layout(order)
        self.flush_stats()
        xt, x, P, obs, met, st = snap[:6]
        self.x_true[slot].copy_(xt)
        self.x_filter[slot].copy_(x)
        self.P_filter[slot].copy_(P)
        self.obs[slot].copy_(obs)
        self.metrics[slot].copy_(met)
        self.stats[slot].copy_(st)
        self.status.zero_()
        self.fail_count.zero_()

    def snapshot_state(self, slot):
        base = self.snapshot(slot)
        snap = _Snapshot(tuple(base) + (self.status.clone(), self.fail_count.clone()))
        snap.order = base.order
        return snap

    def restore_state(self, slot, snap):
        self.restore(slot, snap)
        self.status.copy_(snap[6])
        self.fail_count.copy_(snap[7])

    def _spos_ptr(self, k):
        if self._spos_sets is None:
            self._spos_sets = torch.zeros((2, self.ntiles, 2), dtype=torch.int64, device=self.dev)
        return self._spos_sets[k].data_ptr()

    def _step_params(self, slot_in, slot_out, aer_out, stats_out, upd_out, shard_set, shards_out=0, shards_clear=0, aer_cols=4, obs_mirror=0,
                     argmax=False):
        key = (slot_in, slot_out, aer_out, stats_out, upd_out, shard_set, shards_out, shards_clear, aer_cols, obs_mirror, argmax)
        ent = self._pcache.get(key)
        if ent is None:
            p = _lib.ssa_step_params()
            C.memmove(C.byref(p), C.byref(self._p), C.sizeof(p))
            p.x_true_in, p.x_true_out = self._bx_t + slot_in * self._sx, self._bx_t + slot_out * self._sx
            p.x_in, p.x_out = self._bx + slot_in * self._sx, self._bx + slot_out * self._sx
            p.P_in, p.P_out = self._bP + slot_in * self._sP, self._bP + slot_out * self._sP
            p.obs = self._bo + slot_out * self._so
            p.metrics = self._bm + slot_out * self._sm
            p.upd = upd_out if upd_out else self._bu + slot_out * self._su
            p.stats = stats_out if stats_out else self._bs + slot_out * self._ss
            p.aer_out = aer_out
            p.stat_shards = self._shard_sets[shard_set].data_ptr() if shard_set >= 0 else 0
            p.stat_shards_prev, p.stats_prev, p.launch_mask = 0, 0, 0
            p.stat_shards_clear, p.metrics_prev = 0, 0
            p.spos_tiles = self._spos_ptr(shard_set) if (argmax and shard_set >= 0) else 0
            p.spos_tiles_prev = 0
            p.aer_cols = int(aer_cols)
            p.obs_mirror = obs_mirror
            if shards_out:
                p.stat_shards, p.stats, p.stat_shards_clear = shards_out, 0, shards_clear
            ent = (p, C.byref(p), int(p.stats or 0), int(p.metrics))
            if len(self._pcache) > 4096:
                self._pcache.clear()
            self._pcache[key] = ent
        return ent

    def launch_step(self, slot_in, slot_out, time_offset, actions_ptr=None, stream=None, aer_out=0, stats_out=0, upd_out=0,
                    fast_stats=False, defer_fold=False, profile_slot=None, shards_out=0, shards_clear=0, aer_cols=4, action=None,
                    obs_mirror=0, fold_inside=False, env_words=None, argmax_spos=False, mirror_f32=False, sensors=None, sensor_envs=None):
        s = torch.cuda.current_stream().cuda_stream if stream is None else stream
        if shards_out:
            fast_stats, defer_fold = True, False
        defer = bool(defer_fold and fast_stats)
        from_metrics = defer and self.stats_from_metrics and not fold_inside and sensors is None
        if self._fold_pending is not None and (not defer or bool(self._fold_pending[3]) != from_metrics):
            self.flush_stats(s)
        argmax = bool(argmax_spos and fast_stats and not shards_out)
        if argmax and not self.supports_argmax:
            raise _lib.SsaHipError("argmax_spos on the one-launch paths needs whole tiles per env (n_env == 1 or n_obj % 4 == 0)")
        p, pref, stats_ptr, metrics_ptr = self._step_params(slot_in, slot_out, aer_out, stats_out, upd_out, self._shard_cur if fast_stats else -1,
                                               shards_out, shards_clear, aer_cols, obs_mirror, argmax)
        p.time_offset = int(time_offset)
        p.actions = self._actions_ptr if actions_ptr is None else actions_ptr
        inline = _lib.LAUNCH_MIRROR_F32 if mirror_f32 else 0
        if env_words is not None:
            if self.E > _lib.INLINE_ENVS:
                raise _lib.SsaHipError("env_words: at most %d envs travel in the parameter block" % _lib.INLINE_ENVS)
            p.inline_time[:self.E] = env_words[0]
            p.inline_action[:self.E] = env_words[1]
            inline |= _lib.LAUNCH_INLINE_ENVS
        elif action is not None:
            p.action0, inline = int(action), inline | _lib.LAUNCH_INLINE_ACTION
        if fold_inside and fast_stats and not defer and not shards_out:
            inline |= _lib.LAUNCH_FOLD_INSIDE
        if from_metrics:
            inline |= _lib.LAUNCH_STATS_FROM_METRICS
        if defer and self._fold_pending is not None:
            p.launch_mask = _lib.LAUNCH_DEFER_FOLD | inline
            p.stat_shards_prev = self._shard_ptr[self._fold_pending[0]]
            p.stats_prev = self._fold_pending[1]
            p.spos_tiles_prev = self._spos_ptr(self._fold_pending[0]) if self._fold_pending[2] else 0
            p.metrics_prev = self._fold_pending[3]
        else:
            p.launch_mask = (_lib.LAUNCH_DEFER_FOLD if defer else 0) | inline
            p.stat_shards_prev, p.stats_prev, p.spos_tiles_prev, p.metrics_prev = 0, 0, 0, 0
        if sensors is not None:
            if profile_slot is not None:
                raise _lib.SsaHipError("profile_slot: the step of a sensor network is not profiled by event pairs")
            if sensor_envs is not None:
                rc = self._lib.ssa_env_step_sensors_envs_f64(self._cref, pref, C.byref(sensors), C.byref(sensor_envs), s)
            else:
                rc = self._lib.ssa_env_step_sensors_f64(self._cref, pref, C.byref(sensors), s)
        elif profile_slot is None:
            rc = self._lib.ssa_env_step_f64(self._cref, pref, s)
        else:
            rc = self._lib.ssa_env_step_profiled_f64(self._cref, pref, s, int(profile_slot))
        if rc:
            raise _lib.SsaHipError("%s failed with code %d" % ("ssa_env_step_sensors_envs_f64" if sensor_envs is not None else
                                                               "ssa_env_step_sensors_f64" if sensors is not None else "ssa_env_step_f64", rc))
        if defer:
            self._fold_pending = (self._shard_cur, stats_ptr, argmax, metrics_ptr if from_metrics else 0)
            self._shard_cur ^= 1

    def _check_sensor_noise(self, sensors, envs=False):
        S = int(sensors.n_sensor)
        need = (S - 1) * int(sensors.zn_stride_sensor) + (self.n_time - 1) * self.zn_stride_time + (self.m - 1) * int(self._p.zn_stride_obj) + 3
        if envs:
            need += (self.E - 1) * self.zn_stride_env
        if self.z_noise.numel() < need:
            raise _lib.SsaHipError("z_noise: %d values needed for %d sensors, got %d" % (need, S, self.z_noise.numel()))

    def launch_step_sensors(self, slot_in, slot_out, time_offset, sensors, actions, upd_out, stream=None, **kw):
        if self.E != 1:
            raise _lib.SsaHipError("a sensor network's step covers one env (n_env == 1)")
        S = int(sensors.n_sensor)
        if len(actions) != S:
            raise _lib.SsaHipError("launch_step_sensors: %d actions for %d sensors" % (len(actions), S))
        self._check_sensor_noise(sensors)
        for k in range(S):
            sensors.action[k] = int(actions[k])
        sensors.upd = int(upd_out)
        self.launch_step(slot_in, slot_out, time_offset, stream=stream, sensors=sensors, **kw)

    def _sensor_envs_block(self):
        if self._sensor_envs is None:
            W = _lib.MAX_SENSORS
            self._sensor_envs = (_lib.ssa_sensor_envs_params(), torch.full((self.E, W), -1, dtype=torch.int32, device=self.dev),
                                 np.full((self.E, W), -1, dtype=np.int32))
        return self._sensor_envs

    def action_table(self):
        return self._sensor_envs_block()[1]

    def launch_step_sensors_envs(self, slot_in, slot_out, time_offset, sensors, actions=None, upd_out=0, stream=None, env_words=None, **kw):
        S = int(sensors.n_sensor)
        if actions is None:
            if env_words is not None:
                raise _lib.SsaHipError("launch_step_sensors_envs: actions=None reads the rows and the time words from device memory (no env_words)")
        else:
            a = np.asarray(actions, dtype=np.int64)
            if a.shape != (self.E, S):
                raise _lib.SsaHipError("launch_step_sensors_envs: actions must be [%d][%d] (envs x sensors), got %s" % (self.E, S, a.shape))
        if self.E > 1 and self.m % 4:
            raise _lib.SsaHipError("a sensor network in several envs needs n_obj % 4 == 0 (whole tiles per env)")
        self._check_sensor_noise(sensors, envs=True)
        v, table, rows_np = self._sensor_envs_block()
        v.upd = int(upd_out)
        if actions is None:
            v.actions = table.data_ptr()
            self.launch_step(slot_in, slot_out, time_offset, stream=stream, sensors=sensors, sensor_envs=v, env_words=None, **kw)
            return
        a = np.clip(a, -1, 2 ** 31 - 1)
        if env_words is not None:
            if self.E > _lib.INLINE_ENVS:
                raise _lib.SsaHipError("env_words: at most %d envs travel in the parameter block" % _lib.INLINE_ENVS)
            v.actions = 0
            rows = a.tolist()
            for e in range(self.E):
                v.inline_action[e][:S] = rows[e]
            words = ([int(t) for t in env_words], [-1] * self.E)
        else:
            rows_np[:, :S] = a
            table.copy_(torch.from_numpy(rows_np))
            v.actions = table.data_ptr()
            words = None
        self.launch_step(slot_in, slot_out, time_offset, stream=stream, sensors=sensors, sensor_envs=v, env_words=words, **kw)

    LOOKAHEAD_PARTS = ("x_prior", "P_prior", "P_post")

    def _lookahead_out(self, name, attr, lead, prior_lead, out):
        want = tuple(out)
        bad = [k for k in want if k not in self.LOOKAHEAD_PARTS]
        if bad:
            raise ValueError("%s: unknown output(s) %s (choose from %s)" % (name, bad, self.LOOKAHEAD_PARTS))
        look = getattr(self, attr)
        if look is None or tuple(look["status"].shape) != lead:
            look = {"score": torch.empty(lead + (_lib.LOOK_NSCORE,), dtype=f64, device=self.dev),
                    "status": torch.empty(lead, dtype=torch.int32, device=self.dev),
                    "visible": torch.empty(lead, dtype=torch.uint8, device=self.dev)}
            setattr(self, attr, look)
        shapes = {"x_prior": prior_lead + (6,), "P_prior": prior_lead + (6, 6), "P_post": lead + (6, 6)}
        for k in want:
            if k not in look:
                look[k] = torch.empty(shapes[k], dtype=f64, device=self.dev)
        o = _lib.ssa_lookahead_out()
        o.score, o.status, o.visible = (look[k].data_ptr() for k in ("score", "status", "visible"))
        for k in self.LOOKAHEAD_PARTS:
            setattr(o, k, look[k].data_ptr() if k in want else 0)
        return o, {k: look[k] for k in ("score", "status", "visible") + want}

    def _lookahead_params(self, slot_in, time_offset):
        p = _lib.ssa_step_params()
        C.memmove(C.byref(p), C.byref(self._p), C.sizeof(p))
        sl = int(slot_in) % self.H
        p.x_true_in, p.x_in, p.P_in = self._bx_t + sl * self._sx, self._bx + sl * self._sx, self._bP + sl * self._sP
        p.time_offset, p.launch_mask = int(time_offset), 0
        return p

    def launch_lookahead(self, slot_in, time_offset, out=(), stream=None, env_times=None):
        N = self.m * self.E
        o, res = self._lookahead_out("launch_lookahead", "_look", (N,), (N,), out)
        s = torch.cuda.current_stream().cuda_stream if stream is None else stream
        p = self._lookahead_params(slot_in, time_offset)
        if env_times is not None:
            if self.E > _lib.INLINE_ENVS:
                raise _lib.SsaHipError("env_times: at most %d envs travel in the parameter block" % _lib.INLINE_ENVS)
            p.inline_time[:self.E] = [int(v) for v in env_times]
            p.launch_mask = _lib.LAUNCH_INLINE_ENVS
        rc = self._lib.ssa_lookahead_f64(self._cref, C.byref(p), C.byref(o), s)
        if rc:
            raise _lib.SsaHipError("ssa_lookahead_f64 failed with code %d" % rc)
        return res

    def launch_lookahead_sensors(self, slot_in, time_offset, sensors, out=(), stream=None):
        if self.E != 1:
            raise _lib.SsaHipError("the lookahead of a sensor network covers one env (n_env == 1)")
        o, res = self._lookahead_out("launch_lookahead_sensors", "_look_s", (int(sensors.n_sensor), self.m), (self.m,), out)
        s = torch.cuda.current_stream().cuda_stream if stream is None else stream
        p = self._lookahead_params(slot_in, time_offset)
        rc = self._lib.ssa_lookahead_sensors_f64(self._cref, C.byref(p), C.byref(sensors), C.byref(o), s)
        if rc:
            raise _lib.SsaHipError("ssa_lookahead_sensors_f64 failed with code %d" % rc)
        return res

    def launch_lookahead_sensors_envs(self, slot_in, time_offset, sensors, out=(), stream=None, env_times=None):
        o, res = self._lookahead_out("launch_lookahead_sensors_envs", "_look_se", (self.E, int(sensors.n_sensor), self.m), (self.E, self.m), out)
        s = torch.cuda.current_stream().cuda_stream if stream is None else stream
        p = self._lookahead_params(slot_in, time_offset)
        if env_times is not None:
# ... 264 lines not shown
```

Baseline: 74460.

## Add specialized plain step kernel for the single-env from-metrics launch form

Adds a step_plain_kernel instantiation whose ACT policy compiles out the branches for multi-env indexing, observation mirroring, resampling, spos tiles, aer output, shard clearing and XYZ observations. It is chosen on the host when the launch parameters match that common single-env deferred-fold form. The goal is less runtime branching, fewer scalar loads and lower register pressure in the hot step kernel. The cost is one more kernel instantiation and a host-side form check; any configuration outside the form falls back to the generic kernel.

```diff
diff --git a/include/ssa_hip.h b/include/ssa_hip.h
--- a/include/ssa_hip.h
+++ b/include/ssa_hip.h
@@ -128,6 +128,8 @@
 #define SSA_LAUNCH_MIRROR_F32 128u
 #define SSA_LAUNCH_INLINE_ENVS 64u
 #define SSA_LAUNCH_STATS_FROM_METRICS 256u
+#define SSA_LAUNCH_GENERIC 512u
+int ssa_env_step_instance(const ssa_consts *c_host, const ssa_step_params *p_host);
 int ssa_env_step_profiled_f64(const ssa_consts *c_host, const ssa_step_params *p_host, void *stream, int32_t slot);
 int ssa_env_step_profile_ms(int32_t slot, float *kernel_ms);
 typedef struct ssa_rollout_params {
diff --git a/profiles/pmc_counters_reduce.py b/profiles/pmc_counters_reduce.py
--- a/profiles/pmc_counters_reduce.py
+++ b/profiles/pmc_counters_reduce.py
@@ -8,7 +8,7 @@
         continue
     acc = {}
     for r in csv.DictReader(open(fs[0])):
-        if 'step_fast_kernel' not in r['Kernel_Name']:
+        if 'step_fast_kernel' not in r['Kernel_Name'] and 'step_plain_kernel' not in r['Kernel_Name']:
             continue
         if out["kernel"] is None:
             out["kernel"] = r['Kernel_Name'].split('(')[0]
diff --git a/profiles/pmc_reduce.py b/profiles/pmc_reduce.py
--- a/profiles/pmc_reduce.py
+++ b/profiles/pmc_reduce.py
@@ -6,7 +6,7 @@
     for r in csv.DictReader(open(f)):
         if r['Counter_Name'] != counter: continue
         k = r['Kernel_Name']
-        key = 'step' if 'step_fast_kernel' in k else 'propagate' if 'propagate_kernel' in k else 'observe' if 'observe_kernel' in k else None
+        key = 'step' if ('step_fast_kernel' in k or 'step_plain_kernel' in k) else 'propagate' if 'propagate_kernel' in k else 'observe' if 'observe_kernel' in k else None
         if key: acc.setdefault(key, []).append(float(r['Counter_Value']))
     return acc
 fe, wr = per_kernel(sys.argv[1], 'FETCH_SIZE'), per_kernel(sys.argv[2], 'WRITE_SIZE')
diff --git a/ssa-gym_amd/_lib.py b/ssa-gym_amd/_lib.py
--- a/ssa-gym_amd/_lib.py
+++ b/ssa-gym_amd/_lib.py
@@ -109,6 +109,7 @@
 LAUNCH_INLINE_ENVS = 64
 LAUNCH_MIRROR_F32 = 128
 LAUNCH_STATS_FROM_METRICS = 256
+LAUNCH_GENERIC = 512
 INLINE_ENVS = 8
 LOOP_ARGMAX_SPOS, LOOP_DEBUG_WITHHOLD = 1, 2
 FAIL_STRIDE, FAIL_ENV, FAIL_OBJ, FAIL_STATUS, FAIL_TIME, FAIL_ERR = 8, 0, 1, 2, 3, 4
@@ -121,6 +122,7 @@
     "ssa_abi_version": (C.c_int, []),
     "ssa_build_info": (C.c_char_p, []),
     "ssa_env_step_f64": (C.c_int, [C.POINTER(ssa_consts), C.POINTER(ssa_step_params), c_dp]),
+    "ssa_env_step_instance": (C.c_int, [C.POINTER(ssa_consts), C.POINTER(ssa_step_params)]),
     "ssa_env_step_profiled_f64": (C.c_int, [C.POINTER(ssa_consts), C.POINTER(ssa_step_params), c_dp, C.c_int32]),
     "ssa_env_step_profile_ms": (C.c_int, [C.c_int32, C.POINTER(C.c_float)]),
     "ssa_stats_fold_f64": (C.c_int, [c_dp, c_dp, C.c_int32, c_dp]),
diff --git a/ssa-gym_amd/csrc/ssa_kernels.hip b/ssa-gym_amd/csrc/ssa_kernels.hip
--- a/ssa-gym_amd/csrc/ssa_kernels.hip
+++ b/ssa-gym_amd/csrc/ssa_kernels.hip
@@ -157,7 +157,7 @@
 {
     return p.n_env > 1 ? (int64_t)((uint32_t)base / (uint32_t)p.n_obj) * p.n_obj : 0;
 }
-template <bool NT>
+template <bool NT, bool PLAIN = false>
 SSA_DEV void store_tile(const Tiles& t, const ssa_step_params& p, int lane, int64_t base, int cnt)
 {
 #define SSA_SKIP(b) 0
@@ -183,7 +183,7 @@
             }
             if (NT) __builtin_nontemporal_store(pair, reinterpret_cast<v2d*>(dst));
             else *reinterpret_cast<v2d*>(dst) = pair;
-            if (p.obs_mirror) {
+            if (!PLAIN && p.obs_mirror) {
                 const int64_t at = p.obj_ids ? (env_row0(p, base) + t.Oid[jj]) * 12 + r : base * 12 - 64 + 2 * lane;
                 if (p.launch_mask & SSA_LAUNCH_MIRROR_F32)
                     *reinterpret_cast<float2*>(reinterpret_cast<float*>(p.obs_mirror) + at) = make_float2((float)pair.x, (float)pair.y);
@@ -194,7 +194,7 @@
         if (!SSA_SKIP(8) && lane < 16) {
             const int kk = lane >> 2, jj = lane & 3;
             const int64_t obj = base + jj;
-            if (p.n_env == 1) {
+            if (PLAIN || p.n_env == 1) {
                 p.metrics[(int64_t)kk * p.n_obj + obj] = t.Met[jj * 4 + kk];
             } else {
                 const int64_t e = (int64_t)((uint32_t)obj / (uint32_t)p.n_obj), j = obj - e * p.n_obj;
@@ -212,7 +212,7 @@
         const double* src = sO ? t.Obs : sP ? t.P + 128 : sT ? t.T : t.X;
         const bool skip = sO ? SSA_SKIP(2) : sP ? SSA_SKIP(1) : SSA_SKIP(4);
         if (!skip && i < lim) store16<NT>(dst + 2 * i, src + 2 * i);
-        if (sO && p.obs_mirror && i < lim) {
+        if (!PLAIN && sO && p.obs_mirror && i < lim) {
             const int jj = (i * 43) >> 8;
             const int64_t at = p.obj_ids ? (env_row0(p, base) + t.Oid[jj]) * 12 + (2 * i - 12 * jj) : base * 12 + 2 * i;
             if (p.launch_mask & SSA_LAUNCH_MIRROR_F32)
@@ -228,7 +228,7 @@
         const int kk = lane >> 2, jj = lane & 3;
         if (jj < cnt) {
             const int64_t obj = base + jj;
-            if (p.n_env == 1) {
+            if (PLAIN || p.n_env == 1) {
                 p.metrics[(int64_t)kk * p.n_obj + obj] = t.Met[jj * 4 + kk];
             } else {
                 const int64_t e = (int64_t)((uint32_t)obj / (uint32_t)p.n_obj), j = obj - e * p.n_obj;
@@ -816,12 +816,16 @@
     static constexpr bool forecast = false;
     static constexpr bool envs = false;
     static constexpr bool look_envs = false;
+    static constexpr bool plain = false;
     SSA_DEV int get() { return -1; }
     SSA_DEV void before_wait(Tiles&, int, int) {}
     SSA_DEV void mid_step(Tiles&, int) {}
     SSA_DEV const ssa_sensor_params* sites() const { return nullptr; }
 };
 struct ActEarly : ActBase {};
+struct ActPlain : ActBase {
+    static constexpr bool plain = true;
+};
 struct ActLate;
 struct LoopK;
 SSA_DEV void closed_loop_prescore(ActLate& a, Tiles& t, int lane, int cnt);
@@ -1110,6 +1114,9 @@
     constexpr bool FCAST = ACT::forecast;
     constexpr bool ENVS = ACT::envs;
     constexpr bool LENVS = ACT::look_envs;
+    constexpr bool PLAIN = ACT::plain;
+    static_assert(!PLAIN || (!ACT::late && !ALL && !SENS && !LSENS), "ActPlain: a step kernel's form");
+#define SSA_NENV (PLAIN ? 1 : p.n_env)
     constexpr bool ISSUE_LAST = LSENS && PROP != 0;
     constexpr bool PASS_ARGS = LSENS && !(TILE == 1 && PROP == 0);
     int g = lane >> 4, l = lane & 15;
@@ -1117,8 +1124,12 @@
     double q_in = 0.0;
     if (TILE == 0 && lane < 36) q_in = C.Q[lane];
     struct { uint32_t mask; const int32_t *actions, *env_time, *obj_ids; int n_env, time_offset, update_interval; } hw =
-        {p.launch_mask, p.actions, p.env_time, p.obj_ids, p.n_env, p.time_offset, C.update_interval};
-    if (TILE == 0 && !ALL) {
+        {PLAIN ? (SSA_LAUNCH_DEFER_FOLD | SSA_LAUNCH_STATS_FROM_METRICS) : p.launch_mask, p.actions, p.env_time, p.obj_ids, SSA_NENV,
+         p.time_offset, PLAIN ? 1 : C.update_interval};
+    if constexpr (PLAIN) {
+        asm volatile("" : "+s"(hw.actions), "+s"(hw.env_time), "+s"(hw.obj_ids), "+s"(hw.time_offset)
+                     : "s"(p.P_out), "s"(p.x_out), "s"(p.x_true_out), "s"(p.obs), "s"(p.metrics), "s"(p.stat_shards), "s"(p.upd), "s"(p.n_obj));
+    } else if (TILE == 0 && !ALL) {
         asm volatile("" : "+s"(hw.mask), "+s"(hw.actions), "+s"(hw.env_time), "+s"(hw.obj_ids), "+s"(hw.n_env), "+s"(hw.time_offset),
                           "+s"(hw.update_interval)
                      : "s"(p.P_out), "s"(p.x_out), "s"(p.x_true_out), "s"(p.obs), "s"(p.metrics), "s"(p.stat_shards), "s"(p.upd), "s"(p.aer_out),
@@ -1291,7 +1302,7 @@
     g = lane >> 4;
     l = lane & 15;
     obj = base + g;
-    e = (valid && p.n_env > 1) ? (int)((uint32_t)obj / (uint32_t)p.n_obj) : 0;
+    e = (valid && SSA_NENV > 1) ? (int)((uint32_t)obj / (uint32_t)p.n_obj) : 0;
     if constexpr (ENVS) e = asrc.env;
     if constexpr (FCAST && LENVS) e = asrc.env;
     if (TILE == 1 && !ISSUE_LAST) tile_issue(pf, p, lane, next_base, next_cnt);
@@ -1340,7 +1351,7 @@
         if (chol_fail) st_new = SSA_ST_PREDICT_LINALG;
         else if (nan_x) st_new = SSA_ST_PREDICT_NAN;
     }
-    if (C.flags & SSA_FLAG_RESAMPLE) {
+    if (!PLAIN && (C.flags & SSA_FLAG_RESAMPLE)) {
         const int rg = robust_chol_row_lds(t, C.scale, g, l);
         wave_lds_sync();
         if (active && st_new == SSA_ST_OK && rg == 16) st_new = SSA_ST_PREDICT_LINALG;
@@ -1380,7 +1391,7 @@
                 sf[c] = o[c];
                 xb[c] = t.X[g * 6 + c];
             }
-            if ((C.flags & SSA_FLAG_RESAMPLE) && (!LSENS || look_s == 0)) {
+            if (!PLAIN && (C.flags & SSA_FLAG_RESAMPLE) && (!LSENS || look_s == 0)) {
                 const int krow = is_pm ? (l - 1) % 6 : 0;
                 const double sgn = (l >= 1 && l <= 6) ? 1.0 : ((l >= 7 && l <= 12) ? -1.0 : 0.0);
 #pragma unroll
@@ -1422,7 +1433,7 @@
                     lim = SP->obs_limit[look_s];
                 } else hx_aer_enu(sf, Mm, C.enu, C.obs_itrs, aer, enu_vec);
                 el_mine = aer[1];
-                if (C.obs_type == SSA_OBS_AER) { z[0] = aer[0]; z[1] = aer[1]; z[2] = aer[2]; }
+                if (PLAIN || C.obs_type == SSA_OBS_AER) { z[0] = aer[0]; z[1] = aer[1]; z[2] = aer[2]; }
                 else { z[0] = sf[0]; z[1] = sf[1]; z[2] = sf[2]; }
             }
             if constexpr (SENS || LSENS) visible = row_bcast<13>(el_mine) >= lim;
@@ -1434,7 +1445,7 @@
             if (visible) {
                 double zp[3];
                 const double wl = (l == 0) ? C.Wc0 : (is_pm ? C.Wi : 0.0);
-                if (C.obs_type == SSA_OBS_AER) {
+                if (PLAIN || C.obs_type == SSA_OBS_AER) {
                     double um[3];
 #pragma unroll
                     for (int c = 0; c < 3; ++c) {
@@ -1462,7 +1473,7 @@
 #pragma unroll
                         for (int c = 0; c < 3; ++c) zin[c] = z[c];
                     }
-                    if (C.obs_type == SSA_OBS_AER) residual_z_aer_wrapped(zin, zp, rz);
+                    if (PLAIN || C.obs_type == SSA_OBS_AER) residual_z_aer_wrapped(zin, zp, rz);
                     else {
 #pragma unroll
                         for (int c = 0; c < 3; ++c) rz[c] = zin[c] - zp[c];
@@ -1585,7 +1596,7 @@
         rec[SSA_UPD_VISIBLE] = visible ? 1.0 : 0.0;
         if constexpr (ENVS) rec[SSA_UPD_ACTION] = attempted ? (double)(p.obj_ids ? (int64_t)t.Oid[g] : obj - (int64_t)asrc.env * p.n_obj) : -1.0;
         else if constexpr (SENS) rec[SSA_UPD_ACTION] = attempted ? (double)(p.obj_ids ? (int64_t)t.Oid[g] : obj) : -1.0;
-        else rec[SSA_UPD_ACTION] = attempted ? (double)(ACT::late ? act : env_action<INL, SEG>(p, e)) : -1.0;
+        else rec[SSA_UPD_ACTION] = attempted ? (double)(ACT::late ? act : PLAIN ? *(ConstPtr<int32_t>)p.actions : env_action<INL, SEG>(p, e)) : -1.0;
     }
     if constexpr (ALL) {
         look_vis = visible;
@@ -1595,13 +1606,13 @@
     g = lane >> 4;
     l = lane & 15;
     obj = base + g;
-    e = (valid && p.n_env > 1) ? (int)((uint32_t)obj / (uint32_t)p.n_obj) : 0;
+    e = (valid && SSA_NENV > 1) ? (int)((uint32_t)obj / (uint32_t)p.n_obj) : 0;
     if constexpr (ENVS) e = asrc.env;
     if constexpr (FCAST && LENVS) e = asrc.env;
     if (TILE == 1 && !ISSUE_LAST) tile_issue(pf, p, lane, next_base, next_cnt);
     }
     if (!ALL && valid && p.upd && obj == (int64_t)e * p.n_obj && l == 0) {
-      const int a_env = ACT::late ? act : env_action<INL, SEG>(p, e);
+      const int a_env = ACT::late ? act : PLAIN ? *(ConstPtr<int32_t>)p.actions : env_action<INL, SEG>(p, e);
       if (!(a_env >= 0 && interval_ok && (int64_t)a_env < p.n_obj)) {
         double* rec = p.upd + (int64_t)e * SSA_UPD_STRIDE;
         rec[SSA_UPD_OBS_TAKEN] = 0.0;
@@ -1661,7 +1672,7 @@
                 rec[SSA_FAIL_ENV] = (double)e;
                 rec[SSA_FAIL_OBJ] = p.obj_ids ? (double)t.Oid[g] : (double)(obj - (int64_t)e * p.n_obj);
                 rec[SSA_FAIL_STATUS] = (double)st_new;
-                rec[SSA_FAIL_TIME] = (double)((ACT::late ? p.env_time[0] : env_time_of<INL, SEG>(p, e)) + p.time_offset);
+                rec[SSA_FAIL_TIME] = (double)((ACT::late ? p.env_time[0] : PLAIN ? *(ConstPtr<int32_t>)p.env_time : env_time_of<INL, SEG>(p, e)) + p.time_offset);
                 rec[SSA_FAIL_ERR + 0] = sqrt(a0 * a0 + a1 * a1 + a2 * a2);
                 rec[SSA_FAIL_ERR + 1] = sqrt(b0 * b0 + b1 * b1 + b2 * b2);
                 rec[SSA_FAIL_ERR + 2] = sqrt(Pd[0] + Pd[7] + Pd[14]);
@@ -1713,21 +1724,21 @@
         return;
     }
     observe_rows(t, g, l, cnt != OBJ_PER_WAVE);
-    if (p.aer_out && p.stat_shards) {
+    if (!PLAIN && p.aer_out && p.stat_shards) {
         if (l < 4 && valid) aer_obs_tile<INL, SEG>(t, p, C, g, l, e, p.obj_ids ? (int64_t)e * p.n_obj + t.Oid[g] : obj);
     }
     wave_lds_sync();
     if (!ACT::late) {
-        if (p.spos_tiles && p.stat_shards && lane == 0) {
+        if (!PLAIN && p.spos_tiles && p.stat_shards && lane == 0) {
             unsigned long long key, idx;
             spos_tile_best(t, cnt, obj - (int64_t)e * p.n_obj, key, idx, p.obj_ids != nullptr);
             unsigned long long* slot = (unsigned long long*)p.spos_tiles + 2 * (int64_t)tile;
             __hip_atomic_store(slot, key, __ATOMIC_RELAXED, __HIP_MEMORY_SCOPE_AGENT);
             __hip_atomic_store(slot + 1, idx, __ATOMIC_RELAXED, __HIP_MEMORY_SCOPE_AGENT);
         }
-        store_tile<TILE != 1>(t, p, lane, base, cnt);
-        const bool one_env = p.n_env == 1 || ((uint32_t)base / (uint32_t)p.n_obj == (uint32_t)(base + cnt - 1) / (uint32_t)p.n_obj);
-        if (FROM_METRICS && (p.launch_mask & SSA_LAUNCH_STATS_FROM_METRICS)) {
+        store_tile<TILE != 1, PLAIN>(t, p, lane, base, cnt);
+        const bool one_env = SSA_NENV == 1 || ((uint32_t)base / (uint32_t)p.n_obj == (uint32_t)(base + cnt - 1) / (uint32_t)p.n_obj);
+        if (FROM_METRICS && (PLAIN || (p.launch_mask & SSA_LAUNCH_STATS_FROM_METRICS))) {
             const unsigned long long failed = __ballot(valid && st_new != 0) & 0x0001000100010001ull;
             if (failed && lane == 63) {
                 unsigned long long* sh = (unsigned long long*)p.stat_shards + (int64_t)(tile & (SSA_STAT_SHARDS - 1)) * SSA_STAT_SHARD_WORDS;
@@ -1813,13 +1824,14 @@
                                               p.stats + (e_first + i) * SSA_STAT_STRIDE, lane);
           }
         }
-        if (tile == 0) {
+        if (!PLAIN && tile == 0) {
             if (p.stat_shards_clear) {
                 unsigned long long* z = (unsigned long long*)p.stat_shards_clear;
                 for (int i = lane; i < p.n_env * SSA_STAT_SHARDS * 4; i += 64) z[(i >> 2) * SSA_STAT_SHARD_WORDS + (i & 3)] = 0ull;
             }
         }
     }
+#undef SSA_NENV
 }
 
 SSA_DEV void fold_stat_shards(unsigned long long* __restrict__ shards, double* __restrict__ stats, int e, int lane,
@@ -1914,6 +1926,9 @@
     LookK k;
     ssa_sensor_params s;
 };
+struct PlainK {
+    StepK k;
+};
 struct VecSensK {
     StepK k;
     ssa_sensor_params s;
@@ -1921,6 +1936,7 @@
 };
 SSA_DEV const StepK& step_of(const StepK& k) { return k; }
 SSA_DEV const StepK& step_of(const LookK& k) { return k.k; }
+SSA_DEV const StepK& step_of(const PlainK& k) { return k.k; }
 SSA_DEV const StepK& step_of(const SensK& k) { return k.k; }
 SSA_DEV const StepK& step_of(const LookSensK& k) { return k.k.k; }
 SSA_DEV const StepK& step_of(const VecLookSensK& k) { return k.k.k; }
@@ -1931,6 +1947,7 @@
 }
 SSA_DEV const StepK& step_of(const VecSensK& k) { return k.k; }
 SSA_DEV ActEarly act_of(const StepK&) { return ActEarly(); }
+SSA_DEV ActPlain act_of(const PlainK&) { return ActPlain(); }
 SSA_DEV ActAll act_of(const LookK& k) { return ActAll{{}, &k.o}; }
 SSA_DEV ActSensors act_of(const SensK& k) { return ActSensors{{}, &k.s}; }
 SSA_DEV ActLookSensors act_of(const LookSensK& k) { return ActLookSensors{{}, &k.k.o, &k.s}; }
@@ -1940,7 +1957,8 @@
     WALK_STEP = 1,
     WALK_ONE_ENV = 2,
     WALK_ACT_SEGMENT = 4,
-    WALK_BASE_PER_TILE = 8
+    WALK_BASE_PER_TILE = 8,
+    WALK_PLAIN = 16
 };
 #define SSA_TILE_KERNEL(NAME, K, WALK)                                                                                                        \
     template <int PROP, bool MULTI>                                                                                                           \
@@ -1952,7 +1970,7 @@
         const int unit = (int)blockIdx.x;                                                                                                     \
         if (((WALK) & WALK_STEP) && unit >= nwork) {                                                                                          \
             const ssa_step_params& p = step_of(k_arg).p;                                                                                      \
-            if (!MULTI && !((WALK) & WALK_ONE_ENV) && (p.launch_mask & SSA_LAUNCH_STATS_FROM_METRICS))                                        \
+            if (!MULTI && !((WALK) & WALK_ONE_ENV) && (((WALK) & WALK_PLAIN) || (p.launch_mask & SSA_LAUNCH_STATS_FROM_METRICS)))             \
                 stats_service_wave(p.metrics_prev, (unsigned long long*)p.stat_shards_prev, p.stats_prev,                                     \
                                    (const unsigned long long*)p.spos_tiles_prev, p.n_obj, unit - nwork, (int)gridDim.x - nwork, lane);        \
             else                                                                                                                              \
@@ -1968,10 +1986,10 @@
             const bool whole = tile < ntiles;                                  \
                    \
             tile_dma_issue(t, pf, pre_P_in, pre_x_in, pre_x_true_in, pre_status, lane, base, whole, step_of(k_arg).p,                         \
-                           ((WALK) & WALK_ONE_ENV) != 0);                                                                                     \
+                           ((WALK) & (WALK_ONE_ENV | WALK_PLAIN)) != 0);                                                                      \
             int cnt = OBJ_PER_WAVE;                                                                                                           \
             asm volatile("" : "+s"(cnt));                                                                                                     \
-            if (!whole) cnt = (int)(tile_total(step_of(k_arg).p, ((WALK) & WALK_ONE_ENV) != 0) - base);                                       \
+            if (!whole) cnt = (int)(tile_total(step_of(k_arg).p, ((WALK) & (WALK_ONE_ENV | WALK_PLAIN)) != 0) - base);                        \
             const K& ka = ((WALK) & WALK_ACT_SEGMENT)                                                                                         \
                               ? *(const K*)(KernargPtr<K>)((const char*)__builtin_amdgcn_kernarg_segment_ptr() + offsetof(TileArgs<K>, k))    \
                               : k_arg;                                                                                                        \
@@ -2006,6 +2024,7 @@
     }
 
 SSA_TILE_KERNEL(step_fast_kernel, StepK, WALK_STEP | WALK_BASE_PER_TILE)
+SSA_TILE_KERNEL(step_plain_kernel, PlainK, WALK_STEP | WALK_PLAIN)
 SSA_TILE_KERNEL(lookahead_kernel, LookK, 0)
 SSA_TILE_KERNEL(lookahead_sensors_kernel, LookSensK, WALK_ONE_ENV | WALK_ACT_SEGMENT)
 SSA_TILE_KERNEL(step_sensors_kernel, SensK, WALK_STEP | WALK_ONE_ENV)
@@ -3715,8 +3734,7 @@
     return s;
 }
 
-static int step_launch(const ssa_consts* c, const ssa_step_params* p, void* stream, hipEvent_t ev0, hipEvent_t ev1,
-                       const ssa_sensor_params* sens = nullptr, const ssa_sensor_envs_params* envs = nullptr)
+static int step_args(const ssa_consts* c, const ssa_step_params* p, bool sens, TileGrid& g)
 {
     if (!c || !p || p->n_obj <= 0 || p->n_env <= 0) return SSA_E_INVALID;
     if (!p->x_true_in || !p->x_true_out || !p->x_in || !p->x_out || !p->P_in || !p->P_out || !p->status ||
@@ -3737,20 +3755,39 @@
     if ((p->spos_tiles || p->spos_tiles_prev) && ragged_envs(p)) return SSA_E_UNSUPPORTED;
     if (!consts_ok(c)) return SSA_E_INVALID;
     if (p->aer_cols != 0 && p->aer_cols != 1 && p->aer_cols != 4) return SSA_E_INVALID;
+    if (!rows_fit(p->n_env, p->n_obj)) return SSA_E_INVALID;
+    g = tile_grid((int64_t)p->n_env * p->n_obj);
+    const bool fast_stats = p->stat_shards != nullptr;
+    const bool defer = fast_stats && (p->launch_mask & SSA_LAUNCH_DEFER_FOLD);
+    if (defer && p->stat_shards_prev && (!p->stats_prev || p->stat_shards_prev == p->stat_shards)) return SSA_E_INVALID;
+    if (p->launch_mask & SSA_LAUNCH_STATS_FROM_METRICS) {
+        if (!defer || sens || p->n_env != 1 || g.per_wave != 1 || (p->launch_mask & SSA_LAUNCH_FOLD_INSIDE) || p->stat_shards_clear)
+            return SSA_E_UNSUPPORTED;
+        if (p->stat_shards_prev && !p->metrics_prev) return SSA_E_INVALID;
+    }
+    return SSA_OK;
+}
+static bool step_plain_form(const ssa_consts* c, const ssa_step_params* p, bool sens, const TileGrid& g)
+{
+    const uint32_t need = SSA_LAUNCH_DEFER_FOLD | SSA_LAUNCH_STATS_FROM_METRICS;
+    const uint32_t none = SSA_LAUNCH_INLINE_ACTION | SSA_LAUNCH_INLINE_ENVS | SSA_LAUNCH_FOLD_INSIDE | SSA_LAUNCH_MIRROR_F32 | SSA_LAUNCH_GENERIC | 7u;
+    return !sens && p->n_env == 1 && g.per_wave == 1 && (p->launch_mask & need) == need && !(p->launch_mask & none) && p->actions &&
+           !p->aer_out && !p->obs_mirror && !p->spos_tiles && !p->spos_tiles_prev && !p->stat_shards_clear && c->update_interval <= 1 &&
+           !(c->flags & SSA_FLAG_RESAMPLE) && c->obs_type == SSA_OBS_AER;
+}
+
+static int step_launch(const ssa_consts* c, const ssa_step_params* p, void* stream, hipEvent_t ev0, hipEvent_t ev1,
+                       const ssa_sensor_params* sens = nullptr, const ssa_sensor_envs_params* envs = nullptr)
+{
+    TileGrid g;
+    const int rc = step_args(c, p, sens != nullptr, g);
+    if (rc != SSA_OK) return rc;
     StepK k;
     k.c = *c;
     k.p = *p;
-    if (!rows_fit(p->n_env, p->n_obj)) return SSA_E_INVALID;
-    const TileGrid g = tile_grid((int64_t)p->n_env * p->n_obj);
     const bool fast_stats = p->stat_shards != nullptr;
     const bool defer = fast_stats && (p->launch_mask & SSA_LAUNCH_DEFER_FOLD);
-    if (defer && p->stat_shards_prev && (!p->stats_prev || p->stat_shards_prev == p->stat_shards)) return SSA_E_INVALID;
     const bool from_metrics = (p->launch_mask & SSA_LAUNCH_STATS_FROM_METRICS) != 0;
-    if (from_metrics) {
-        if (!defer || sens || p->n_env != 1 || g.per_wave != 1 || (p->launch_mask & SSA_LAUNCH_FOLD_INSIDE) || p->stat_shards_clear)
-            return SSA_E_UNSUPPORTED;
-        if (p->stat_shards_prev && !p->metrics_prev) return SSA_E_INVALID;
-    }
     const int nfold = (defer && p->stat_shards_prev) ? (from_metrics ? STAT_SERVICE_WAVES : p->n_env) : 0;
     dim3 grid((unsigned)(g.nwork + nfold)), block(64);
     const int nparts = post_parts(p->n_obj, p->n_env);
@@ -3778,6 +3815,12 @@
         with_prop(prop, g.per_wave != 1, [&](auto P, auto M) {
             hipExtLaunchKernelGGL((step_sensors_kernel<P, M>), grid, block, 0, s, ev0, ev1, 0, g.arg, g.nwork, p->P_in, p->x_in, p->x_true_in, p->status, ks);
         });
+    } else if ((mask & 1u) && step_plain_form(c, p, false, g)) {
+        PlainK kp;
+        kp.k = k;
+        with_prop(prop, [&](auto P) {
+            hipExtLaunchKernelGGL((step_plain_kernel<P, false>), grid, block, 0, s, ev0, ev1, 0, g.arg, g.nwork, p->P_in, p->x_in, p->x_true_in, p->status, kp);
+        });
     } else if (mask & 1u) {
         with_prop(prop, g.per_wave != 1, [&](auto P, auto M) {
             hipExtLaunchKernelGGL((step_fast_kernel<P, M>), grid, block, 0, s, ev0, ev1, 0, g.arg, g.nwork, p->P_in, p->x_in, p->x_true_in, p->status, k);
@@ -3812,6 +3855,12 @@
 int ssa_env_step_f64(const ssa_consts* c, const ssa_step_params* p, void* stream)
 {
     return step_launch(c, p, stream, nullptr, nullptr);
+}
+int ssa_env_step_instance(const ssa_consts* c, const ssa_step_params* p)
+{
+    TileGrid g;
+    const int rc = step_args(c, p, false, g);
+    return rc != SSA_OK ? rc : (step_plain_form(c, p, false, g) ? 1 : 0);
 }
 int ssa_env_step_sensors_f64(const ssa_consts* c, const ssa_step_params* p, const ssa_sensor_params* sp, void* stream)
 {
diff --git a/ssa-gym_amd/engine.py b/ssa-gym_amd/engine.py
--- a/ssa-gym_amd/engine.py
+++ b/ssa-gym_amd/engine.py
@@ -69,6 +69,7 @@
         self._shard_sets = torch.zeros((2, self.E, _lib.STAT_SHARDS, _lib.STAT_SHARD_WORDS), dtype=torch.int64, device=d)
         self.stat_shards = self._shard_sets[0]
         self._shard_cur = 0
+        self.force_generic = False
         self._fold_pending = None
         self.stats_from_metrics = int(self._lib.ssa_stats_from_metrics_waves(self.m, self.E)) > 0
         self._shard_ptr = [self._shard_sets[0].data_ptr(), self._shard_sets[1].data_ptr()]
@@ -291,6 +292,8 @@
             inline |= _lib.LAUNCH_FOLD_INSIDE
         if from_metrics:
             inline |= _lib.LAUNCH_STATS_FROM_METRICS
+        if self.force_generic:
+            inline |= _lib.LAUNCH_GENERIC
         if defer and self._fold_pending is not None:
             p.launch_mask = _lib.LAUNCH_DEFER_FOLD | inline
             p.stat_shards_prev = self._shard_ptr[self._fold_pending[0]]
```

Measured after the change: 77810 (median of 6 runs). 4.5% higher.
